# hbdat/cvpr22_cross_modal_pseudo_labeling

Measured on AMD Instinct MI355X. Metric: images/sec student-teacher train step (COCO 800x1333), higher is better.
Workload: dtype f32 (bf16x3 split MFMA, fp32 accum); 1 GPU; student_teacher_mask_rcnn_uncertainty.yaml R-50-C4, 2 img/GPU 3x800x1333, fwd+bwd+allreduce+SGD; global_batch=2, parallelism=dp1, losses_finite=True, pipelined=True

## Files before the change

### cvpr22_cross_modal_pseudo_labeling_amd/_C.py

```python
import contextlib
import functools
import ctypes
import threading

import torch

from . import _cpu, _lib

_L = _lib.load()


def _stream():
    return torch._C._cuda_getCurrentRawStream(torch.cuda.current_device())


class _Same:

    def __enter__(self):
        return None

    def __exit__(self, *exc):
        return False


# ... 494 lines not shown
    out = torch.empty((r * h * w, 3 * kh * kw * c), dtype=torch.bfloat16, device=x.device)
    if out.numel() == 0:
        return out
    with _on(x.device):
        rc = _L.ovis_im2col_split_bf16x3_f32(x.data_ptr(), out.data_ptr(), r, h, w, c, kh, kw, int(bool(flip)), _stream())
    _lib.check(rc, "im2col_split_bf16x3")
    return out


def match_encode(gt_boxes, gt_labels, proposals, high, low, weights=None, between_keeps_label=False):
    gt_boxes, proposals = _dev(gt_boxes, "gt_boxes"), _dev(proposals, "proposals")
    gt_labels = gt_labels.to(torch.int64).contiguous()
    g, p = gt_boxes.shape[0], proposals.shape[0]
    if g == 0:
        raise ValueError("No ground-truth boxes available for one of the images during training")
    idx = torch.empty((p,), dtype=torch.int64, device=proposals.device)
    lab = torch.empty((p,), dtype=torch.int64, device=proposals.device)
    reg = torch.empty((p, 4), dtype=torch.float32, device=proposals.device) if weights is not None else None
    if p:
        wx, wy, ww, wh = weights if weights is not None else (1.0, 1.0, 1.0, 1.0)
        with _on(proposals.device):
            rc = _L.ovis_match_encode_f32(gt_boxes.data_ptr(), gt_labels.data_ptr(), proposals.data_ptr(), g, p, high, low,
                                          int(bool(between_keeps_label)), wx, wy, ww, wh, idx.data_ptr(), lab.data_ptr(),
                                          0 if reg is None else reg.data_ptr(), _stream())
        _lib.check(rc, "match_encode")
    return idx, lab, reg


def rpn_match_encode(gt_boxes, anchors, visibility, high_threshold, low_threshold, allow_low_quality_matches, weights):
    gt_boxes, anchors = _dev(gt_boxes, "gt_boxes"), _dev(anchors, "anchors")
    if not (visibility.is_cuda and visibility.dtype == torch.bool and visibility.shape == (anchors.shape[0],)):
        raise RuntimeError("rpn_match_encode: visibility must be a bool HIP tensor [A]")
    visibility = visibility.contiguous()
    g, a = gt_boxes.shape[0], anchors.shape[0]
    if g == 0:
        raise ValueError("No ground-truth boxes available for one of the images during training")
    labels = torch.empty((a,), dtype=torch.int64, device=anchors.device)
    reg = torch.empty((a, 4), dtype=torch.float32, device=anchors.device)
    scratch = torch.empty((g,), dtype=torch.int32, device=anchors.device)
    wx, wy, ww, wh = weights
    with _on(anchors.device):
        rc = _L.ovis_rpn_match_encode_f32(gt_boxes.data_ptr(), anchors.data_ptr(), visibility.data_ptr(), g, a, high_threshold,
                                          low_threshold, int(bool(allow_low_quality_matches)), wx, wy, ww, wh, scratch.data_ptr(),
                                          labels.data_ptr(), reg.data_ptr(), _stream())
    _lib.check(rc, "rpn_match_encode")
    return labels, reg


def project_masks(masks, gt_index, boxes, resolution):
    if not (masks.is_cuda and masks.dim() == 3 and masks.dtype in (torch.bool, torch.uint8)):
        raise RuntimeError("project_masks: [G,H,W] bool / uint8 HIP tensor expected")
    masks = masks.contiguous()
    boxes = _dev(boxes, "boxes")
    gt_index = gt_index.to(torch.int64).contiguous()
    p = boxes.shape[0]
    out = torch.empty((p, resolution, resolution), dtype=torch.float32, device=boxes.device)
    if p:
        with _on(boxes.device):
            rc = _L.ovis_project_masks_f32(masks.data_ptr(), gt_index.data_ptr(), boxes.data_ptr(), p, masks.shape[1],
                                           masks.shape[2], resolution, int(masks.dtype == torch.bool), out.data_ptr(),
                                           _stream())
        _lib.check(rc, "project_masks")
    return out


def sample_fg_bg(labels, batch_size, max_positives, seed):
    if not labels.is_cuda or labels.dtype != torch.int64 or labels.dim() != 1:
        raise RuntimeError("sample_fg_bg: 1-D int64 HIP tensor expected (the product path has no CPU fallback)")
    labels = labels.contiguous()
    sel = torch.empty((batch_size,), dtype=torch.int64, device=labels.device)
    slots = torch.empty((batch_size,), dtype=torch.int64, device=labels.device)
    counts = torch.empty((2,), dtype=torch.int32, device=labels.device)
    with _on(labels.device):
        rc = _L.ovis_sample_fg_bg(labels.data_ptr(), labels.numel(), int(batch_size), int(max_positives),
                                  int(seed) & 0xFFFFFFFFFFFFFFFF, sel.data_ptr(), slots.data_ptr(), counts.data_ptr(), _stream())
    _lib.check(rc, "sample_fg_bg")
    return sel, slots, counts


def gather_rows(index, boxes_a=None, boxes_b=None, ints_a=None, ints_b=None):
    index = _dev(index, "index", torch.int64)
    n = index.numel()
    srcs = [None if t is None else _dev(t, "boxes", torch.float32) for t in (boxes_a, boxes_b)] + \
           [None if t is None else _dev(t, "ints", torch.int64) for t in (ints_a, ints_b)]
    for t in srcs[:2]:
        if t is not None and (t.dim() != 2 or t.shape[1] != 4):
            raise RuntimeError("gather_rows: float sources must be [P, 4]")
    for t in srcs[2:]:
        if t is not None and t.dim() != 1:
            raise RuntimeError("gather_rows: int64 sources must be [P]")
    outs = [None if t is None else torch.empty((n,) + tuple(t.shape[1:]), dtype=t.dtype, device=t.device) for t in srcs]
    if n:
        ptr = lambda t: 0 if t is None else t.data_ptr()
        with _on(index.device):
            rc = _L.ovis_gather_rows(index.data_ptr(), n, ptr(srcs[0]), ptr(outs[0]), ptr(srcs[1]), ptr(outs[1]), ptr(srcs[2]),
                                     ptr(outs[2]), ptr(srcs[3]), ptr(outs[3]), _stream())
        _lib.check(rc, "gather_rows")
    return tuple(outs)


def project_pasted_masks(mask_probs, gt_boxes, gt_index, boxes, image_size, resolution, threshold=0.5):
    mask_probs, gt_boxes, boxes = _dev(mask_probs, "mask_probs"), _dev(gt_boxes, "gt_boxes"), _dev(boxes, "boxes")
    gt_index = _dev(gt_index, "gt_index", torch.int64)
    p = boxes.shape[0]
    out = torch.empty((p, resolution, resolution), dtype=torch.float32, device=boxes.device)
    if p == 0:
        return out
    if mask_probs.dim() != 3 or mask_probs.shape[1] != mask_probs.shape[2] or gt_boxes.shape != (mask_probs.shape[0], 4):
        raise RuntimeError("project_pasted_masks: expected mask_probs [G,M,M] and gt_boxes [G,4]")
    with _on(boxes.device):
        rc = _L.ovis_project_pasted_masks_f32(mask_probs.data_ptr(), gt_boxes.data_ptr(), gt_index.data_ptr(),
                                              boxes.data_ptr(), p, int(image_size[0]), int(image_size[1]),
                                              mask_probs.shape[1], int(resolution), float(threshold), out.data_ptr(), _stream())
    _lib.check(rc, "project_pasted_masks")
    return out


def split_pair(x):
    if not x.is_cuda or x.dtype != torch.float32 or x.dim() != 2:
        raise RuntimeError("split_pair: 2-D float32 HIP tensor expected")
    if x.stride(1) != 1 or x.stride(0) % 4 or x.data_ptr() % 16:
        x = x.contiguous()
    rows, cols = x.shape
    out = torch.empty((rows, 2 * cols), dtype=torch.bfloat16, device=x.device)
    if out.numel() == 0:
        return out
    with _on(x.device):
        rc = _L.ovis_split_pair_f32(x.data_ptr(), x.stride(0), out.data_ptr(), rows, cols, _stream())
    _lib.check(rc, "split_pair")
    return out


def gate_split_pair(dy, gate=None, want_f32=False, pooled=None, pool_rows=0, selected=None, group_slot=None):
    if dy is None and pooled is None:
        raise RuntimeError("gate_split_pair: dy or pooled must be given")
    if (selected is None) != (group_slot is None):
        raise RuntimeError("gate_split_pair: selected and group_slot are given together")
    if pooled is not None:
        if not (pooled.is_cuda and pooled.dtype == torch.float32 and pooled.dim() == 2):
            raise RuntimeError("gate_split_pair: pooled must be a 2-D float32 HIP tensor")
        pooled = pooled.contiguous()
    if dy is not None:
        if not (dy.is_cuda and dy.dtype == torch.float32 and dy.dim() == 2):
            raise RuntimeError("gate_split_pair: 2-D float32 HIP tensor expected")
        if dy.stride(1) != 1 or dy.stride(0) % 4 or dy.data_ptr() % 16:
            dy = dy.contiguous()
        rows, cols = dy.shape
    else:
        rows, cols = pooled.shape[0] * pool_rows, pooled.shape[1]
    if pooled is not None and (pool_rows <= 0 or pooled.shape != (rows // max(pool_rows, 1), cols) or rows % pool_rows):
        raise RuntimeError("gate_split_pair: pooled must be [rows / pool_rows, cols]")
    dev = dy.device if dy is not None else pooled.device
    is_pair = 0
    if gate is not None:
        is_pair = int(gate.dtype == torch.bfloat16)
        if not (gate.is_cuda and gate.is_contiguous() and gate.shape == (rows, cols * (2 if is_pair else 1))
                and gate.dtype in (torch.bfloat16, torch.float32)):
            raise RuntimeError("gate_split_pair: gate must be the contiguous fp32 or pair form of the forward output")
    out = torch.empty((rows, 2 * cols), dtype=torch.bfloat16, device=dev)
    g32 = torch.empty((rows, cols), dtype=torch.float32, device=dev) if want_f32 else None
    if out.numel() == 0:
        return out, g32
    if selected is not None:
        selected, group_slot = _dev(selected, "selected"), _dev(group_slot, "group_slot", torch.int32)
        if pool_rows <= 0 or rows % pool_rows or selected.dim() != 2 or selected.shape[1] != cols or \
                selected.shape[0] % pool_rows or group_slot.numel() != rows // pool_rows:
            raise RuntimeError("gate_split_pair: selected must be [S * pool_rows, cols] and group_slot [rows / pool_rows]")
    with _on(dev):
        rc = _L.ovis_gate_split_pair_rows_f32(0 if dy is None else dy.data_ptr(), 0 if dy is None else dy.stride(0),
                                              0 if gate is None else gate.data_ptr(), is_pair, out.data_ptr(),
                                              0 if g32 is None else g32.data_ptr(), rows, cols,
                                              0 if pooled is None else pooled.data_ptr(), pool_rows,
                                              0 if selected is None else selected.data_ptr(),
                                              0 if group_slot is None else group_slot.data_ptr(), _stream())
    _lib.check(rc, "gate_split_pair")
    return out, g32


def im2col_pair(xp, h, w, kh, kw):
    if not (xp.is_cuda and xp.dtype == torch.bfloat16 and xp.dim() == 2 and xp.is_contiguous()):
        raise RuntimeError("im2col_pair: contiguous 2-D bfloat16 HIP tensor (pair layout) expected")
    m, c2 = xp.shape
    if m % (h * w):
        raise RuntimeError("im2col_pair: rows must be a multiple of h*w")
    out = torch.empty((m, kh * kw * c2), dtype=torch.bfloat16, device=xp.device)
    if out.numel() == 0:
        return out
    with _on(xp.device):
        rc = _L.ovis_im2col_pair(xp.data_ptr(), out.data_ptr(), m // (h * w), h, w, c2 // 2, kh, kw, _stream())
    _lib.check(rc, "im2col_pair")
    return out


def im2col_nchw_pair(x, kh, kw, stride, pad):
    if not (x.is_cuda and x.dtype == torch.float32 and x.dim() == 4 and x.is_contiguous()):
        raise RuntimeError("im2col_nchw_pair: contiguous [N,C,H,W] float32 HIP tensor expected")
    n, c, h, w = x.shape
    ho, wo = (h + 2 * pad - kh) // stride + 1, (w + 2 * pad - kw) // stride + 1
    kp = -(-(kh * kw * c) // 32) * 32
    out = torch.empty((n * ho * wo, 2 * kp), dtype=torch.bfloat16, device=x.device)
    if out.numel():
        with _on(x.device):
            rc = _L.ovis_im2col_nchw_pair_f32(x.data_ptr(), out.data_ptr(), n, c, h, w, kh, kw, stride, pad, kp, _stream())
        _lib.check(rc, "im2col_nchw_pair")
    return out, (ho, wo)


_GEMM_TLS = threading.local()


@contextlib.contextmanager
def co_scheduled(on=True):
    prev = getattr(_GEMM_TLS, "co", False)
    _GEMM_TLS.co = bool(on)
    try:
        yield
    finally:
        _GEMM_TLS.co = prev


@functools.lru_cache(maxsize=None)
def _gemm_ws_bytes(m, n, ch, ch2, kh, kw, w, config):
    return int(_L.ovis_split_gemm_pair_workspace_bytes_ex(m, n, ch, ch2, kh, kw, w, config))


@functools.lru_cache(maxsize=None)
def _tn_slices(m, n, ch, taps):
    return int(_L.ovis_split_gemm_tn_slices(m, n, ch, taps))


@functools.lru_cache(maxsize=None)
def _gemm_f32_ws_bytes(m, n, k):
    return int(_L.ovis_gemm_f32_workspace_bytes(m, n, k))


@functools.lru_cache(maxsize=None)
def _nms_presorted_ws_bytes(n, k):
    return int(_L.ovis_nms_presorted_workspace_bytes(n, k))


@functools.lru_cache(maxsize=None)
def _topk_ws_bytes(n, a):
    return int(_L.ovis_topk_sorted_workspace_bytes(n, a))


def _gemm_cfg(config):
    return config | (0x10000 if getattr(_GEMM_TLS, "co", False) else 0)


def split_gemm_pair(a_pair, b_pair, bias=None, residual=None, relu=False, out_f32=True, out_pair=False, conv=None,
                    config=0, a2_pair=None, residual_pair=None):
    for t, name in ((a_pair, "a_pair"), (b_pair, "b_pair")) + (((a2_pair, "a2_pair"),) if a2_pair is not None else ()):
        if not (t.is_cuda and t.dtype == torch.bfloat16 and t.dim() == 2 and t.stride(1) == 1):
            raise RuntimeError(f"split_gemm_pair: {name} must be a 2-D bfloat16 HIP tensor in pair layout")
    m, ch = a_pair.shape[0], a_pair.shape[1] // 2
    n, k = b_pair.shape[0], b_pair.shape[1] // 2
    ch2 = 0
    if a2_pair is not None:
        if conv is not None or a2_pair.shape[0] != m:
            raise RuntimeError("split_gemm_pair: a2_pair needs a plain product and as many rows as a_pair")
        ch2 = a2_pair.shape[1] // 2
    h = w = 0
    kh = kw = 1
    flip = False
    if conv is not None:
        h, w, kh, kw, flip = conv
        if m % (h * w):
            raise RuntimeError("split_gemm_pair: rows must be a multiple of h*w")
    if k != kh * kw * ch + ch2:
        raise RuntimeError(f"split_gemm_pair: contraction mismatch (A has {ch} channels x {kh * kw} taps + {ch2}, B has {k})")
    dev = a_pair.device
    c = torch.empty((m, n), dtype=torch.float32, device=dev) if out_f32 else None
    cp = torch.empty((m, 2 * n), dtype=torch.bfloat16, device=dev) if out_pair else None
    if m == 0 or n == 0:
        return c, cp
    if bias is not None:
        bias = _dev(bias, "bias")
    if residual_pair is not None:
        if residual is not None or conv is not None or a2_pair is not None or n % 32 or not (
                residual_pair.is_cuda and residual_pair.dtype == torch.bfloat16 and residual_pair.dim() == 2
                and residual_pair.stride(1) == 1 and residual_pair.shape == (m, 2 * n)):
            raise RuntimeError("split_gemm_pair: residual_pair must be [M, 2N] bfloat16 pair rows of a plain product")
        with _on(dev):
            config = _gemm_cfg(config)
            nbytes = _gemm_ws_bytes(m, n, ch, 0, 1, 1, 0, config) if not (config & 8) else 0
            ws = torch.empty((nbytes,), dtype=torch.uint8, device=dev) if nbytes else None
            rc = _L.ovis_split_gemm_pair_rp(a_pair.data_ptr(), 2 * a_pair.stride(0), b_pair.data_ptr(), 2 * b_pair.stride(0),
                                            0 if c is None else c.data_ptr(), n, 0 if cp is None else cp.data_ptr(), 4 * n,
                                            0 if bias is None else bias.data_ptr(), residual_pair.data_ptr(),
                                            2 * residual_pair.stride(0), m, n, ch, int(bool(relu)),
                                            0 if ws is None else ws.data_ptr(), nbytes, config, _stream())
        _lib.check(rc, "split_gemm_pair_rp")
        return c, cp
    if residual is not None and not (residual.is_cuda and residual.dtype == torch.float32 and residual.dim() == 2
                                     and residual.stride(1) == 1 and residual.shape == (m, n)):
        raise RuntimeError("split_gemm_pair: residual must be a float32 [M, N] HIP tensor with unit column stride")
    with _on(dev):
        config = _gemm_cfg(config)
        nbytes = _gemm_ws_bytes(m, n, ch, ch2, kh, kw, w, config) if not (config & 8) else 0
        ws = torch.empty((nbytes,), dtype=torch.uint8, device=dev) if nbytes else None
        rc = _L.ovis_split_gemm_pair(a_pair.data_ptr(), 2 * a_pair.stride(0),
                                     0 if a2_pair is None else a2_pair.data_ptr(),
                                     0 if a2_pair is None else 2 * a2_pair.stride(0),
                                     b_pair.data_ptr(), 2 * b_pair.stride(0),
                                     0 if c is None else c.data_ptr(), n, 0 if cp is None else cp.data_ptr(), 4 * n,
                                     0 if bias is None else bias.data_ptr(),
                                     0 if residual is None else residual.data_ptr(),
                                     0 if residual is None else residual.stride(0), m, n, ch, ch2, kh, kw, h, w,
                                     int(bool(flip)), int(bool(relu)), 0 if ws is None else ws.data_ptr(), nbytes,
                                     config, _stream())
    _lib.check(rc, "split_gemm_pair")
    return c, cp


def split_gemm_pair_pool_supported(m, n, ch, pool_rows):
    return bool(_L.ovis_split_gemm_pair_pool_supported(int(m), int(n), int(ch), int(pool_rows)))


def split_gemm_pair_rp_pool(a_pair, b_pair, bias, residual_pair, relu, out_f32, out_pair, pool_rows):
    for t, name in ((a_pair, "a_pair"), (b_pair, "b_pair")) + (((residual_pair, "residual_pair"),) if residual_pair is not None else ()):
        if not (t.is_cuda and t.dtype == torch.bfloat16 and t.dim() == 2 and t.stride(1) == 1):
            raise RuntimeError(f"split_gemm_pair_rp_pool: {name} must be a 2-D bfloat16 HIP tensor in pair layout")
    m, ch = a_pair.shape[0], a_pair.shape[1] // 2
    n, k = b_pair.shape[0], b_pair.shape[1] // 2
    if k != ch or m % pool_rows or (residual_pair is not None and residual_pair.shape != (m, 2 * n)):
        raise RuntimeError("split_gemm_pair_rp_pool: shape mismatch")
    dev = a_pair.device
    c = torch.empty((m, n), dtype=torch.float32, device=dev) if out_f32 else None
    cp = torch.empty((m, 2 * n), dtype=torch.bfloat16, device=dev) if out_pair else None
    pooled = torch.zeros((m // pool_rows, n), dtype=torch.float32, device=dev)
    if m == 0 or n == 0:
        return c, cp, pooled
    if bias is not None:
        bias = _dev(bias, "bias")
    with _on(dev):
        rc = _L.ovis_split_gemm_pair_rp_pool(a_pair.data_ptr(), 2 * a_pair.stride(0), b_pair.data_ptr(), 2 * b_pair.stride(0),
                                             0 if c is None else c.data_ptr(), n, 0 if cp is None else cp.data_ptr(), 4 * n,
                                             0 if bias is None else bias.data_ptr(),
                                             0 if residual_pair is None else residual_pair.data_ptr(),
                                             0 if residual_pair is None else 2 * residual_pair.stride(0), m, n, ch,
                                             int(bool(relu)), pooled.data_ptr(), int(pool_rows), 1.0 / pool_rows, _stream())
    _lib.check(rc, "split_gemm_pair_rp_pool")
    return c, cp, pooled


def weight_prep_pair(w, scale=None, want_transposed=False):
    if not (w.is_cuda and w.dtype == torch.float32 and w.dim() == 4):
        raise RuntimeError("weight_prep_pair: [N,C,KH,KW] float32 HIP tensor expected")
    w = w.detach().contiguous()
    n, c, kh, kw = w.shape
    t = kh * kw
    fwd = torch.empty((n, 2 * t * c), dtype=torch.bfloat16, device=w.device)
    bwd = torch.empty((c, 2 * t * n), dtype=torch.bfloat16, device=w.device) if want_transposed else None
    if scale is not None:
        scale = _dev(scale.detach(), "scale")
    with _on(w.device):
        rc = _L.ovis_weight_prep_pair_f32(w.data_ptr(), 0 if scale is None else scale.data_ptr(), fwd.data_ptr(),
                                          0 if bwd is None else bwd.data_ptr(), n, c, t, _stream())
    _lib.check(rc, "weight_prep_pair")
    return fwd, bwd


def split_gemm_pair_gated(a_pair, b_pair, gate_pair, conv=None, out_f32=False, out_pair=True, config=0):
    for t, name in ((a_pair, "a_pair"), (b_pair, "b_pair"), (gate_pair, "gate_pair")):
        if not (t.is_cuda and t.dtype == torch.bfloat16 and t.dim() == 2 and t.stride(1) == 1):
            raise RuntimeError(f"split_gemm_pair_gated: {name} must be a 2-D bfloat16 HIP tensor in pair layout")
    m, ch = a_pair.shape[0], a_pair.shape[1] // 2
    n, k = b_pair.shape[0], b_pair.shape[1] // 2
    h = w = 0
    kh = kw = 1
    flip = False
    if conv is not None:
        h, w, kh, kw, flip = conv
    if k != kh * kw * ch or gate_pair.shape != (m, 2 * n):
        raise RuntimeError("split_gemm_pair_gated: shape mismatch")
    dev = a_pair.device
    c = torch.empty((m, n), dtype=torch.float32, device=dev) if out_f32 else None
    cp = torch.empty((m, 2 * n), dtype=torch.bfloat16, device=dev) if out_pair else None
    if m == 0 or n == 0:
        return c, cp
    with _on(dev):
        config = _gemm_cfg(config)
        nbytes = _gemm_ws_bytes(m, n, ch, 0, kh, kw, w, config) if not (config & 8) else 0
        ws = torch.empty((nbytes,), dtype=torch.uint8, device=dev) if nbytes else None
        rc = _L.ovis_split_gemm_pair_gated_ws(a_pair.data_ptr(), 2 * a_pair.stride(0), b_pair.data_ptr(),
                                              2 * b_pair.stride(0), 0 if c is None else c.data_ptr(), n,
                                              0 if cp is None else cp.data_ptr(), 4 * n, gate_pair.data_ptr(),
                                              2 * gate_pair.stride(0), m, n, ch, kh, kw, h, w, int(bool(flip)),
                                              0 if ws is None else ws.data_ptr(), nbytes, config, _stream())
    _lib.check(rc, "split_gemm_pair_gated")
    return c, cp


def split_gemm_pair_rp_gated(a_pair, b_pair, residual_pair, gate_pair, out_f32=False, out_pair=True, config=0):
    for t, name in ((a_pair, "a_pair"), (b_pair, "b_pair"), (residual_pair, "residual_pair"), (gate_pair, "gate_pair")):
        if not (t.is_cuda and t.dtype == torch.bfloat16 and t.dim() == 2 and t.stride(1) == 1):
            raise RuntimeError(f"split_gemm_pair_rp_gated: {name} must be a 2-D bfloat16 HIP tensor in pair layout")
    m, ch = a_pair.shape[0], a_pair.shape[1] // 2
    n, k = b_pair.shape[0], b_pair.shape[1] // 2
    if k != ch or gate_pair.shape != (m, 2 * n) or residual_pair.shape != (m, 2 * n):
        raise RuntimeError("split_gemm_pair_rp_gated: shape mismatch")
    dev = a_pair.device
    c = torch.empty((m, n), dtype=torch.float32, device=dev) if out_f32 else None
    cp = torch.empty((m, 2 * n), dtype=torch.bfloat16, device=dev) if out_pair else None
    if m == 0 or n == 0:
        return c, cp
    with _on(dev):
        rc = _L.ovis_split_gemm_pair_rp_gated(a_pair.data_ptr(), 2 * a_pair.stride(0), b_pair.data_ptr(),
                                              2 * b_pair.stride(0), 0 if c is None else c.data_ptr(), n,
                                              0 if cp is None else cp.data_ptr(), 4 * n, residual_pair.data_ptr(),
                                              2 * residual_pair.stride(0), gate_pair.data_ptr(), 2 * gate_pair.stride(0), m, n,
                                              ch, config, _stream())
    _lib.check(rc, "split_gemm_pair_rp_gated")
    return c, cp


def split_gemm_pair_tn_supported(n, ch, conv=None):
    if n % 128 or ch % 128:
        return False
    if conv is not None:
        h, w, kh, kw = conv
        return kh % 2 == 1 and kw % 2 == 1
    return True


def split_gemm_pair_tn(g_pair, x_pair, conv=None, scale=None, weight_shape=None):
    for t, name in ((g_pair, "g_pair"), (x_pair, "x_pair")):
        if not (t.is_cuda and t.dtype == torch.bfloat16 and t.dim() == 2 and t.stride(1) == 1):
            raise RuntimeError(f"split_gemm_pair_tn: {name} must be a 2-D bfloat16 HIP tensor in pair layout")
    m, n, ch = g_pair.shape[0], g_pair.shape[1] // 2, x_pair.shape[1] // 2
    if x_pair.shape[0] != m:
        raise RuntimeError("split_gemm_pair_tn: row counts differ")
    h = w = 0
    kh = kw = 1
    if conv is not None:
        h, w, kh, kw = conv
        if m % (h * w):
            raise RuntimeError("split_gemm_pair_tn: rows must be a multiple of h*w")
    dev = g_pair.device
    if m == 0:
        z = torch.zeros((n, kh * kw * ch), dtype=torch.float32, device=dev)
        return z if weight_shape is None else z.new_zeros(weight_shape)
    slices = _tn_slices(m, n, ch, kh * kw)
    slabs = torch.empty((slices, n, kh * kw * ch), dtype=torch.float32, device=dev)
    with _on(dev):
        rc = _L.ovis_split_gemm_pair_tn(g_pair.data_ptr(), 2 * g_pair.stride(0), x_pair.data_ptr(), 2 * x_pair.stride(0),
                                        slabs.data_ptr(), slices, m, n, ch, kh, kw, h, w, _stream())
        _lib.check(rc, "split_gemm_pair_tn")
        if weight_shape is None:
            return slabs[0] if slices == 1 else slabs.sum(0)
        if tuple(weight_shape) != (n, ch, kh, kw):
            raise RuntimeError("split_gemm_pair_tn: weight_shape must be (N, ch, kh, kw)")
        dw = torch.empty(weight_shape, dtype=torch.float32, device=dev)
        if scale is not None:
            scale = _dev(scale.detach(), "scale")
        rc = _L.ovis_slab_reduce_f32(slabs.data_ptr(), 0 if scale is None else scale.data_ptr(), dw.data_ptr(), slices, n,
                                     ch, kh * kw, _stream())
    _lib.check(rc, "slab_reduce")
    return dw


def bias_act_(y, bias=None, residual=None, relu=True):
    if not (y.is_cuda and y.dtype == torch.float32 and y.dim() == 2 and y.is_contiguous()):
        raise RuntimeError("bias_act_: contiguous 2-D float32 HIP tensor expected")
    if residual is not None and not (residual.is_contiguous() and residual.shape == y.shape):
        raise RuntimeError("bias_act_: residual must be contiguous with y's shape")
    if y.numel() == 0:
        return y
    with _on(y.device):
        rc = _L.ovis_bias_act_f32(y.data_ptr(), 0 if bias is None else bias.data_ptr(),
                                  0 if residual is None else residual.data_ptr(), y.shape[0], y.shape[1],
                                  int(bool(relu)), _stream())
    _lib.check(rc, "bias_act")
    return y


def gemm_nt(a, b, bias=None):
    if not a.is_cuda and not b.is_cuda:
        return _cpu.gemm_nt(a, b, bias)
    if not (a.is_cuda and b.is_cuda):
        raise RuntimeError("gemm_nt: HIP device tensors only")
    if a.dtype != torch.float32 or b.dtype != torch.float32:
        raise RuntimeError("gemm_nt: float32 only")
    m, k = a.shape
    n, k2 = b.shape
    if k != k2:
        raise RuntimeError(f"gemm_nt: inner dimensions differ ({k} vs {k2})")
    out = torch.empty((m, n), dtype=torch.float32, device=a.device)
    if m == 0 or n == 0:
        return out
    if k == 0:
        return out.zero_() if bias is None else out.copy_(bias.expand(m, n))
    if bias is not None:
        bias = _dev(bias, "bias")
    with _on(a.device):
        _gemm_raw(a.data_ptr(), a.stride(0), a.stride(1), b.data_ptr(), b.stride(0), b.stride(1), out.data_ptr(), n, m, n, k,
                  bias_ptr=0 if bias is None else bias.data_ptr(), device=a.device)
    return out


def region_noun_align(region_emb, noun_emb):
    if not region_emb.is_cuda:
        return _cpu.region_noun_align(region_emb, noun_emb)
    region_emb, noun_emb = _dev(region_emb, "region_emb"), _dev(noun_emb, "noun_emb")
    p, d = region_emb.shape
    w = noun_emb.shape[0]
    raw = torch.empty((w,), dtype=torch.float32, device=region_emb.device)
    prob = torch.empty_like(raw)
    idx = torch.empty((w,), dtype=torch.int64, device=region_emb.device)
    if w == 0:
        return raw, prob, idx
    with _on(region_emb.device):
        rc = _L.ovis_region_noun_align_f32(region_emb.data_ptr(), noun_emb.data_ptr(), raw.data_ptr(),
                                           prob.data_ptr(), idx.data_ptr(), p, w, d, _stream())
    _lib.check(rc, "region_noun_align")
    return raw, prob, idx


def text_embed(table, input_ids, special_tokens_mask):
    if not table.is_cuda:
        return _cpu.text_embed(table.detach(), input_ids.to(torch.int64), special_tokens_mask.to(torch.int64))
    table = _dev(table, "table")
    if table.dim() != 2 or input_ids.dim() != 2 or input_ids.shape != special_tokens_mask.shape:
        raise RuntimeError("text_embed: expected table [V, D] and input_ids / special_tokens_mask [N, L]")
    if table.requires_grad:
        raise RuntimeError("text_embed: the embedding table is frozen on this path (MODEL.LANGUAGE_BACKBONE.FT_EMB False)")
    ids = input_ids.to(device=table.device, dtype=torch.int32).contiguous()
    sp = special_tokens_mask.to(device=table.device, dtype=torch.int32).contiguous()
    n, l = ids.shape
    out = torch.empty((n, table.shape[1]), dtype=torch.float32, device=table.device)
    if n:
        with _on(table.device):
            rc = _L.ovis_text_embed_f32(table.data_ptr(), table.shape[0], table.shape[1], ids.data_ptr(), sp.data_ptr(), n, l,
                                        out.data_ptr(), _stream())
        _lib.check(rc, "text_embed")
    return out


def project_polygon_masks(coords, polygon_start, instance_start, gt_index, boxes, image_size, resolution):
    if not boxes.is_cuda:
        return _cpu.project_polygon_masks(coords, polygon_start, instance_start, gt_index, boxes, image_size, resolution)
    boxes = _dev(boxes, "boxes")
    coords = _dev(coords, "coords") if coords.numel() else coords
    polygon_start = _dev(polygon_start, "polygon_start", torch.int32)
    instance_start = _dev(instance_start, "instance_start", torch.int32)
    gt_index = _dev(gt_index, "gt_index", torch.int64)
    p = boxes.shape[0]
    out = torch.empty((p, resolution, resolution), dtype=torch.float32, device=boxes.device)
    if p:
        with _on(boxes.device):
            rc = _L.ovis_project_polygon_masks_f32(coords.data_ptr() if coords.numel() else 0, polygon_start.data_ptr(),
                                                   instance_start.data_ptr(), gt_index.data_ptr(), boxes.data_ptr(), p,
                                                   int(image_size[0]), int(image_size[1]), int(resolution), out.data_ptr(),
                                                   _stream())
        _lib.check(rc, "project_polygon_masks")
    return out


def weighted_ce_fwd_bwd(logits, labels, bg_weight, need_grad=True):
    if not logits.is_cuda:
        return _cpu.weighted_ce_fwd_bwd(logits, labels, bg_weight, need_grad)
    logits, labels = _dev(logits, "logits"), _dev(labels, "labels", torch.int64)
    p, c = logits.shape
    loss = torch.empty((1,), dtype=torch.float32, device=logits.device)
    dlogits = torch.empty_like(logits) if need_grad else None
    scratch = torch.empty((max(p, 1),), dtype=torch.float32, device=logits.device)
# ... 305 lines not shown
```

### cvpr22_cross_modal_pseudo_labeling_amd/_lib.py

```python
import ctypes
import os

_HERE = os.path.dirname(os.path.abspath(__file__))
LIB_PATH = os.path.join(_HERE, "libovis_hip.so")

OVIS_OK = 0
_ERRORS = {-1: "OVIS_EINVAL (bad size or null pointer)",
           -2: "OVIS_ENOSPC (workspace too small)",
           -3: "OVIS_ERANGE (problem size not supported by the kernel)"}

_vp, _i, _f, _sz, _l = ctypes.c_void_p, ctypes.c_int, ctypes.c_float, ctypes.c_size_t, ctypes.c_long

SIGNATURES = {
    "ovis_version": (ctypes.c_char_p, []),
    "ovis_roi_align_forward_f32": (_i, [_vp, _vp, _vp, _i, _i, _i, _i, _i, _i, _i, _f, _i, _vp]),
    "ovis_roi_align_forward_workspace_bytes": (_sz, [_i, _i, _i]),
    "ovis_roi_align_forward_mfma_supported": (_i, [_i, _i, _i, _i]),
    "ovis_roi_align_forward_ws_f32": (_i, [_vp, _vp, _vp, _i, _i, _i, _i, _i, _i, _i, _f, _i, _vp, _sz, _vp]),
    "ovis_roi_align_forward_strided_from_nhwc_f32": (_i, [_vp, _vp, _vp, _i, _i, _i, _i, _i, _i, _i, _i, _f, _i, _i, _vp]),
    "ovis_roi_align_backward_f32": (_i, [_vp, _vp, _vp, _i, _i, _i, _i, _i, _i, _i, _f, _i, _vp]),
    "ovis_roi_align_backward_workspace_bytes": (_sz, [_i, _i, _i, _i]),
    "ovis_roi_align_backward_plane_supported": (_i, [_i, _i, _i, _i]),
    "ovis_roi_align_backward_ws_f32": (_i, [_vp, _vp, _vp, _i, _i, _i, _i, _i, _i, _i, _f, _i, _vp, _sz, _vp]),
    "ovis_roi_align_backward_strided_ws_f32": (_i, [_vp, _vp, _vp, _i, _i, _i, _i, _i, _i, _i, _i, _f, _i, _vp, _sz, _vp]),
    "ovis_roi_align_backward_strided_nhwc_workspace_bytes": (_sz, [_i, _i, _i, _i, _i]),
    "ovis_roi_align_backward_strided_nhwc_ws_f32": (_i, [_vp, _vp, _vp, _i, _i, _i, _i, _i, _i, _i, _i, _f, _i, _vp, _sz, _vp]),
    "ovis_roi_pool_forward_f32": (_i, [_vp, _vp, _vp, _vp, _i, _i, _i, _i, _i, _i, _i, _f, _vp]),
    "ovis_roi_pool_backward_f32": (_i, [_vp, _vp, _vp, _vp, _i, _i, _i, _i, _i, _i, _i, _vp]),
    "ovis_deform_psroi_pool_forward_f32": (_i, [_vp] * 5 + [_i] * 7 + [_f] + [_i] * 5 + [_f, _vp]),
    "ovis_deform_psroi_pool_backward_f32": (_i, [_vp] * 7 + [_i] * 7 + [_f] + [_i] * 5 + [_f, _vp]),
    "ovis_nms_workspace_bytes": (_sz, [_i]),
    "ovis_nms_f32": (_i, [_vp, _vp, _i, _f, _i, _vp, _sz, _vp, _vp, _vp]),
    "ovis_nms_grouped_f32": (_i, [_vp, _vp, _vp, _i, _f, _i, _vp, _sz, _vp, _vp, _vp]),
    "ovis_sample_fg_bg": (_i, [_vp, _i, _i, _i, ctypes.c_uint64, _vp, _vp, _vp, _vp]),
    "ovis_project_pasted_masks_f32": (_i, [_vp, _vp, _vp, _vp, _i, _i, _i, _i, _i, _f, _vp, _vp]),
    "ovis_nms_presorted_workspace_bytes": (_sz, [_i, _i]),
    "ovis_nms_presorted_batched_f32": (_i, [_vp, _vp, _i, _i, _f, _i, _i, _vp, _sz, _vp, _vp, _vp]),
    "ovis_box_decode_f32": (_i, [_vp, _l, _vp, _l, _l, _i, _f, _f, _f, _f, _f, _i, _vp, _vp, _vp, _vp]),
    "ovis_smooth_l1_picked_fwd_bwd_f32": (_i, [_vp, _l, _i, _i, _vp, _l, _vp, _vp, _i, _i, _f, _f, _vp, _vp, _vp]),
    "ovis_gather_rows": (_i, [_vp, _i, _vp, _vp, _vp, _vp, _vp, _vp, _vp, _vp, _vp]),
    "ovis_rois_from_boxes_f32": (_i, [_vp, _vp, _vp, _i, _vp, _vp]),
    "ovis_deform_conv_implicit_f32": (_i, [_vp, _vp, _vp, _vp, _l, _vp, _vp, _l] + [_i] * 16 + [_vp]),
    "ovis_topk_sorted_workspace_bytes": (_sz, [_i, _i]),
    "ovis_topk_sorted_f32": (_i, [_vp, _l, _i, _i, _i, _vp, _vp, _vp, _sz, _vp]),
    "ovis_rpn_decode_f32": (_i, [_vp, _l, _l, _l, _vp, _vp, _vp, _i, _i, _i, _i, _f, _f, _f, _f, _f, _f, _f, _vp, _vp, _vp]),
    "ovis_sigmoid_focal_loss_forward_f32": (_i, [_vp, _vp, _vp, _i, _i, _f, _f, _vp]),
    "ovis_sigmoid_focal_loss_backward_f32": (_i, [_vp, _vp, _vp, _vp, _i, _i, _f, _f, _vp]),
    "ovis_split_bf16x3_f32": (_i, [_vp, _l, _vp, _l, _i, _i, _vp]),
    "ovis_im2col_split_bf16x3_f32": (_i, [_vp, _vp, _l, _i, _i, _i, _i, _i, _i, _vp]),
    "ovis_bias_act_f32": (_i, [_vp, _vp, _vp, _l, _i, _i, _vp]),
    "ovis_split_pair_f32": (_i, [_vp, _l, _vp, _l, _i, _vp]),
    "ovis_gate_split_pair_rows_f32": (_i, [_vp, _l, _vp, _i, _vp, _vp, _l, _i, _vp, _i, _vp, _vp, _vp]),
    "ovis_gate_split_pair_f32": (_i, [_vp, _l, _vp, _i, _vp, _vp, _l, _i, _vp, _i, _vp]),
    "ovis_im2col_nchw_pair_f32": (_i, [_vp, _vp] + [_i] * 9 + [_vp]),
    "ovis_weight_prep_pair_f32": (_i, [_vp, _vp, _vp, _vp, _i, _i, _i, _vp]),
    "ovis_slab_reduce_f32": (_i, [_vp, _vp, _vp, _i, _i, _i, _i, _vp]),
    "ovis_im2col_pair": (_i, [_vp, _vp, _l, _i, _i, _i, _i, _i, _vp]),
    "ovis_split_gemm_tn_slices": (_i, [_l, _i, _i, _i]),
    "ovis_split_gemm_pair_tn": (_i, [_vp, _l, _vp, _l, _vp, _i, _l, _i, _i, _i, _i, _i, _i, _vp]),
    "ovis_split_gemm_pair_gated": (_i, [_vp, _l, _vp, _l, _vp, _l, _vp, _l, _vp, _l, _l] + [_i] * 8 + [_vp]),
    "ovis_split_gemm_pair_gated_ws": (_i, [_vp, _l, _vp, _l, _vp, _l, _vp, _l, _vp, _l, _l] + [_i] * 7 + [_vp, _sz, _i, _vp]),
    "ovis_split_gemm_pair_workspace_bytes": (_sz, [_l, _i, _i, _i, _i, _i, _i]),
    "ovis_split_gemm_pair_workspace_bytes_ex": (_sz, [_l, _i, _i, _i, _i, _i, _i, _i]),
    "ovis_split_gemm_pair_rp_gated": (_i, [_vp, _l, _vp, _l, _vp, _l, _vp, _l, _vp, _l, _vp, _l, _l, _i, _i, _i, _vp]),
    "ovis_split_gemm_pair_pool_supported": (_i, [_l, _i, _i, _i]),
    "ovis_split_gemm_pair_rp_pool": (_i, [_vp, _l, _vp, _l, _vp, _l, _vp, _l, _vp, _vp, _l, _l, _i, _i, _i, _vp, _i, _f, _vp]),
    "ovis_split_gemm_pair_rp": (_i, [_vp, _l, _vp, _l, _vp, _l, _vp, _l, _vp, _vp, _l, _l, _i, _i, _i, _vp, _sz, _i, _vp]),
    "ovis_split_gemm_pair": (_i, [_vp, _l, _vp, _l, _vp, _l, _vp, _l, _vp, _l, _vp, _vp, _l, _l] + [_i] * 9
                             + [_vp, _sz, _i, _vp]),
    "ovis_match_encode_f32": (_i, [_vp, _vp, _vp, _i, _i, _f, _f, _i, _f, _f, _f, _f, _vp, _vp, _vp, _vp]),
    "ovis_rpn_match_encode_f32": (_i, [_vp, _vp, _vp, _i, _i, _f, _f, _i, _f, _f, _f, _f, _vp, _vp, _vp, _vp]),
    "ovis_project_masks_f32": (_i, [_vp, _vp, _vp, _i, _i, _i, _i, _i, _vp, _vp]),
    "ovis_gemm_f32": (_i, [_vp, _l, _l, _vp, _l, _l, _vp, _vp, _l, _i, _i, _i, _vp]),
    "ovis_gemm_ex_f32": (_i, [_vp, _l, _l, _vp, _l, _l, _vp, _i, _f, _i, _vp, _l, _i, _i, _i, _vp]),
    "ovis_gemm_f32_workspace_bytes": (_sz, [_i, _i, _i]),
    "ovis_gemm_ex_ws_f32": (_i, [_vp, _l, _l, _vp, _l, _l, _vp, _i, _f, _i, _vp, _l, _i, _i, _i, _vp, _sz, _vp]),
    "ovis_deform_im2col_f32": (_i, [_vp, _vp, _vp, _vp] + [_i] * 13 + [_vp]),
    "ovis_deform_col2im_f32": (_i, [_vp, _vp, _vp, _vp] + [_i] * 13 + [_vp]),
    "ovis_deform_col2im_coord_f32": (_i, [_vp, _vp, _vp, _vp, _vp, _vp] + [_i] * 13 + [_vp]),
    "ovis_deform_im2col_pair_rows_f32": (_i, [_vp, _vp, _vp, _vp, _l] + [_i] * 15 + [_vp]),
    "ovis_deform_col2im_rows_f32": (_i, [_vp, _l, _vp, _vp, _vp, _vp, _vp, _vp] + [_i] * 15 + [_vp]),
    "ovis_region_noun_align_f32": (_i, [_vp, _vp, _vp, _vp, _vp, _i, _i, _i, _vp]),
    "ovis_text_embed_f32": (_i, [_vp, _l, _i, _vp, _vp, _i, _i, _vp, _vp]),
    "ovis_project_polygon_masks_f32": (_i, [_vp, _vp, _vp, _vp, _vp, _i, _i, _i, _i, _vp, _vp]),
    "ovis_sgd_momentum_multi_f32": (_i, [_vp, _vp, _i, _f, _f, _f, _i, _vp]),
    "ovis_bottleneck_identity_backward_workspace_bytes": (_sz, [_l, _i, _i, _i, _i, _i, _i]),
    "ovis_bottleneck_identity_backward": (_i, [_vp, _l] * 7 + [_vp] * 3 + [_l, _i, _i, _i, _i, _i, _i] + [_vp] * 7 + [_sz, _i, _vp, _vp]),
    "ovis_weight_prep_pair_multi_f32": (_i, [_vp, _vp, _i, _i, _vp]),
    "ovis_weight_prep_tile": (_i, []),
    "ovis_sgd_chunk_elements": (_i, []),
    "ovis_weighted_ce_fwd_bwd_f32": (_i, [_vp, _vp, _f, _vp, _vp, _vp, _i, _i, _vp]),
    "ovis_mask_bce_stochastic_fwd_bwd_f32": (_i, [_vp, _vp, _vp, _vp, _vp, _vp, _vp, _vp, _vp, _i, _i, _i, _i, _i, _vp]),
    "ovis_mask_bce_stochastic_classes_fwd_bwd_f32": (_i, [_vp, _vp, _vp, _vp, _vp, _vp, _vp, _vp, _vp, _vp, _i, _i, _i, _i, _vp]),
}

_lib = None


def load():
    global _lib
    if _lib is None:
        if not os.path.exists(LIB_PATH):
            raise ImportError(
                f"{LIB_PATH} is missing: build the HIP extension first "
                "(make -C cvpr22_cross_modal_pseudo_labeling_amd/csrc). There is no CPU fallback.")
        lib = ctypes.CDLL(LIB_PATH)
        for name, (res, args) in SIGNATURES.items():
            fn = getattr(lib, name)
            fn.restype = res
            fn.argtypes = args
        _lib = lib
    return _lib


def check(rc, what):
    if rc == OVIS_OK:
        return
    if rc < 0:
        raise RuntimeError(f"{what}: {_ERRORS.get(rc, rc)}")
    raise RuntimeError(f"{what}: HIP error {rc}")
```

### cvpr22_cross_modal_pseudo_labeling_amd/csrc/split_gemm.hip

```cpp
#include <stdlib.h>

#include "ovis_common.h"
constexpr int kGroupWidth = 4;

namespace {
typedef short bf16x8 __attribute__((ext_vector_type(8)));
typedef float f32x4 __attribute__((ext_vector_type(4)));
typedef __bf16 b2 __attribute__((ext_vector_type(2)));
typedef float f2 __attribute__((ext_vector_type(2)));

__device__ char g_zero_line[128];

enum { PLAIN = 0, SHIFTED = 1, HALO = 2, DEFORM = 3 };
constexpr int kHalo = 8;

struct SplitGemmArgs {
  const char* A; long a_rs;
  const char* A2; long a2_rs;
  const char* B; long b_rs;
  float* C; long ldc;
  char* Cp; long cp_rs;
  const float* bias; const float* res; long ldr;
  const char* resp; long resp_rs;
  const char* gate; long gate_rs;
  float* pool; int pool_rows; float pool_scale;
  float* slab;
  long M; int N; int ch; int ch2; int T; int H; int W; int KH; int KW; int flip; int relu; int gw;
  int kslices; int steps_per_slice;
  const float* dimg; const float* doff; const float* dmask;
  int Ho; int Wo; int sh; int sw; int ph; int pw; int dlh; int dlw; int dg;
};

__device__ __forceinline__ void glds16(const char* gsrc, char* lds_wave_base) {
  __builtin_amdgcn_global_load_lds((const __attribute__((address_space(1))) void*)gsrc,
                                   (__attribute__((address_space(3))) void*)lds_wave_base, 16, 0, 0);
}

__device__ __forceinline__ unsigned pack_bf16(float a, float b) {
  f2 v = {a, b};
  return __builtin_bit_cast(unsigned, __builtin_convertvector(v, b2));
}

struct EpilogueOperands {
  uint2 a, b;
};

struct EpilogueSource {
  const char* base;
  long row_bytes;
  int second;
};

__device__ __forceinline__ EpilogueSource epilogue_source(const SplitGemmArgs& p) {
  EpilogueSource s;
  s.base = p.res ? (const char*)p.res : (p.resp ? p.resp : p.gate);
  s.row_bytes = p.res ? p.ldr * 4 : (p.resp ? p.resp_rs : p.gate_rs);
  s.second = p.res ? 8 : (p.resp ? 64 : 0);
  return s;
}

__device__ __forceinline__ long epilogue_column_bytes(const SplitGemmArgs& p, int n, long poff) { return p.res ? (long)n * 4 : poff; }

__device__ __forceinline__ void epilogue_fetch4(const EpilogueSource& s, long m, long column_bytes, EpilogueOperands& o) {
  const char* q = s.base + m * s.row_bytes + column_bytes;
  o.a = *(const uint2*)q;
  o.b = *(const uint2*)(q + s.second);
}

template <bool DUAL = false>
__device__ __forceinline__ f32x4 epilogue_apply4(const SplitGemmArgs& p, long m, int n, long poff, f32x4 v, const f32x4& bias4,
                                                 const EpilogueOperands& o, uint2 gate2 = make_uint2(0u, 0u)) {
  if (p.bias) v += bias4;
  if (p.res) {
    v.x += __uint_as_float(o.a.x); v.y += __uint_as_float(o.a.y); v.z += __uint_as_float(o.b.x); v.w += __uint_as_float(o.b.y);
  } else if (p.resp) {
    const unsigned hx = o.a.x, hy = o.a.y, lx = o.b.x, ly = o.b.y;
    v.x += __uint_as_float(hx << 16) + __uint_as_float(lx << 16);
    v.y += __uint_as_float(hx & 0xffff0000u) + __uint_as_float(lx & 0xffff0000u);
    v.z += __uint_as_float(hy << 16) + __uint_as_float(ly << 16);
    v.w += __uint_as_float(hy & 0xffff0000u) + __uint_as_float(ly & 0xffff0000u);
  }
  if (p.relu) {
    v.x = fmaxf(v.x, 0.f); v.y = fmaxf(v.y, 0.f); v.z = fmaxf(v.z, 0.f); v.w = fmaxf(v.w, 0.f);
  }
  if (p.gate) {
    const unsigned gx = DUAL ? gate2.x : o.a.x, gy = DUAL ? gate2.y : o.a.y;
    const unsigned a0 = gx & 0xffffu, a1 = gx >> 16, a2 = gy & 0xffffu, a3 = gy >> 16;
    if (a0 == 0u || a0 >= 0x8000u) v.x = 0.f;
    if (a1 == 0u || a1 >= 0x8000u) v.y = 0.f;
    if (a2 == 0u || a2 >= 0x8000u) v.z = 0.f;
    if (a3 == 0u || a3 >= 0x8000u) v.w = 0.f;
  }
  if (p.C) *(f32x4*)(p.C + m * p.ldc + n) = v;
  if (p.Cp) {
    const unsigned h01 = pack_bf16(v.x, v.y), h23 = pack_bf16(v.z, v.w);
    const unsigned l01 = pack_bf16(v.x - __uint_as_float(h01 << 16), v.y - __uint_as_float(h01 & 0xffff0000u));
    const unsigned l23 = pack_bf16(v.z - __uint_as_float(h23 << 16), v.w - __uint_as_float(h23 & 0xffff0000u));
    char* d = p.Cp + m * p.cp_rs + poff;
    *(uint2*)d = make_uint2(h01, h23);
    *(uint2*)(d + 64) = make_uint2(l01, l23);
  }
  return v;
}

__device__ __forceinline__ void epilogue_store4(const SplitGemmArgs& p, long m, int n, f32x4 v) {
  const long poff = (long)(n >> 5) * 128 + (n & 31) * 2;
  f32x4 bias4 = {0.f, 0.f, 0.f, 0.f};
  if (p.bias) bias4 = *(const f32x4*)(p.bias + n);
  const EpilogueSource src = epilogue_source(p);
  EpilogueOperands o;
  if (src.base) epilogue_fetch4(src, m, epilogue_column_bytes(p, n, poff), o);
  epilogue_apply4(p, m, n, poff, v, bias4, o);
}

template <int WM, int WN, int MODE, int NS, int OCC, bool DUAL = false, bool POOL = false>
__global__ __launch_bounds__(WM * WN * 64, OCC) void split_gemm_kernel(SplitGemmArgs p, int tiles_n, int ntiles) {
  constexpr int BM = WM * 64, BN = WN * 64, NW = WM * WN;
  constexpr int A_ROWS = MODE == HALO ? BM + 2 * kHalo + 2 : BM;
  constexpr int ZROW = BM + 2 * kHalo;
  constexpr int A_BYTES = A_ROWS * 128, B_BYTES = BN * 128, STAGE = A_BYTES + B_BYTES;
  constexpr int A_PIECES = (MODE == HALO ? BM + 2 * kHalo : BM) / 8;
  constexpr int AI = (A_PIECES + NW - 1) / NW;
  constexpr int BI = BN / 8 / NW;
  static_assert(MODE != HALO || NS == 1, "the halo tile is single-staged");
  static_assert(NW * 4096 <= STAGE * NS, "epilogue staging fits the k-loop's LDS");
  extern __shared__ __attribute__((aligned(16))) char smem[];

  const int lane = threadIdx.x & 63, wave = __builtin_amdgcn_readfirstlane(threadIdx.x >> 6);
  int id;
  {
    const int nblocks = gridDim.x;
    const int b = blockIdx.x, q = nblocks >> 3, r = nblocks & 7, xcd = b & 7, loc = b >> 3;
    id = (xcd < r ? xcd * (q + 1) : r * (q + 1) + (xcd - r) * q) + loc;
  }
  const int slice = id / ntiles;
  const int tile = id - slice * ntiles;
  const int gw = p.gw, tiles_m = ntiles / tiles_n;
  const int per_group = tiles_m * gw;
  const int grp = tile / per_group;
  const int in_grp = tile - grp * per_group;
  const int tile_m = in_grp / gw, tile_n = grp * gw + (in_grp - tile_m * gw);
  const long m0 = (long)tile_m * BM;
  const int n0 = tile_n * BN;
  const int Mi = (int)p.M;

  const int cpb = p.ch >> 5;
  const int nk = p.T * cpb + (p.ch2 >> 5);
  int dy = 0, dx = 0;
  auto set_tap = [&](int t) {
    dy = t / p.KW - p.KH / 2;
    dx = t % p.KW - p.KW / 2;
    if (p.flip) { dy = -dy; dx = -dx; }
  };

  struct LaneGeom { int lr, s0, s1; };
  auto lane_geom = [&](int ln) {
    const int lr = ln >> 3, lc = ln & 7;
    return LaneGeom{lr, (lc ^ lr) * 16, (lc ^ lr) * 16};
  };
  auto clamp_row = [&](int gm) { return gm < 0 ? 0 : (gm > Mi - 1 ? Mi - 1 : gm); };
  int a_yx[MODE == SHIFTED ? AI : 1];
  if (MODE == SHIFTED) {
#pragma unroll
    for (int i = 0; i < AI; ++i) {
      const int gm = clamp_row((int)m0 + (wave * AI + i) * 8 + (lane >> 3));
      a_yx[i] = (((gm / p.W) % p.H) << 16) | (gm % p.W);
    }
  }

  auto issue_b = [&](int stage, int kb, const LaneGeom& g) {
#pragma unroll
    for (int i = 0; i < BI; ++i) {
      const int piece = wave * BI + i;
      int gn = n0 + piece * 8 + g.lr;
      if (gn > p.N - 1) gn = p.N - 1;
      glds16(p.B + (long)gn * p.b_rs + (long)kb * 128 + ((piece & 1) ? g.s1 : g.s0),
             smem + stage * STAGE + A_BYTES + piece * 1024);
    }
  };
  auto issue_a_plain = [&](int stage, int kb, const LaneGeom& g) {
    const bool first = kb < cpb;
    const char* base = first ? p.A : p.A2;
    const long rs = first ? p.a_rs : p.a2_rs;
    const long koff = (long)(first ? kb : kb - cpb) * 128;
#pragma unroll
    for (int i = 0; i < AI; ++i) {
      const int piece = wave * AI + i;
      glds16(base + (long)clamp_row((int)m0 + piece * 8 + g.lr) * rs + koff + ((piece & 1) ? g.s1 : g.s0),
             smem + stage * STAGE + piece * 1024);
    }
  };
  const char* zero_line = g_zero_line;
  auto issue_a_shifted = [&](int stage, int cb, const LaneGeom& g) {
    const long shift = ((long)dy * p.W + dx) * p.a_rs + (long)cb * 128;
#pragma unroll
    for (int i = 0; i < AI; ++i) {
      const int piece = wave * AI + i;
      const char* src = p.A + (long)clamp_row((int)m0 + piece * 8 + g.lr) * p.a_rs + shift + ((piece & 1) ? g.s1 : g.s0);
      const int y = (a_yx[MODE == SHIFTED ? i : 0] >> 16) + dy, x = (a_yx[MODE == SHIFTED ? i : 0] & 0xffff) + dx;
      if ((unsigned)y >= (unsigned)p.H || (unsigned)x >= (unsigned)p.W) src = zero_line + (g.s0 & 0x70);
      glds16(src, smem + stage * STAGE + piece * 1024);
    }
  };
  auto issue_a_halo = [&](int cb, const LaneGeom& g) {
#pragma unroll
    for (int i = 0; i < AI; ++i) {
      const int piece = wave + NW * i;
      if (piece < A_PIECES)
        glds16(p.A + (long)clamp_row((int)m0 + piece * 8 + g.lr - kHalo) * p.a_rs + (long)cb * 128 + ((piece & 1) ? g.s1 : g.s0),
               smem + piece * 1024);
    }
  };

  constexpr int DR = MODE == DEFORM ? 4 : 1;
  float d_w[DR][4], d_mask[DR];
  int d_o[DR][4];
  int d_tap = -1, d_grp = -1;
  f32x4 d_v[DR][4];
  auto deform_fetch = [&](int tap, int cb) {
    if constexpr (MODE == DEFORM) {
      const int prow0 = threadIdx.x >> 3, pch = (threadIdx.x & 7) * 4;
      const int grp = (cb * 32) / (p.ch / p.dg);
      if (tap != d_tap || grp != d_grp) {
        d_tap = tap;
        d_grp = grp;
        const long plane_o = (long)p.Ho * p.Wo;
        const int ky = tap / p.KW, kx = tap - ky * p.KW;
#pragma unroll
        for (int j = 0; j < 4; ++j) {
          const int gm = clamp_row((int)m0 + prow0 + 32 * j);
          const int wo = gm % p.Wo, t1 = gm / p.Wo;
          const int ho = t1 % p.Ho, bimg = t1 / p.Ho;
          const long pix = (long)ho * p.Wo + wo;
          const float* off = p.doff + (((long)bimg * p.dg + grp) * 2 * p.T + 2 * tap) * plane_o + pix;
          const float h = (float)(ho * p.sh - p.ph + ky * p.dlh) + off[0];
          const float w = (float)(wo * p.sw - p.pw + kx * p.dlw) + off[plane_o];
          d_o[j][0] = d_o[j][1] = d_o[j][2] = d_o[j][3] = -1;
          d_w[j][0] = d_w[j][1] = d_w[j][2] = d_w[j][3] = 0.f;
          if (h > -1.f && w > -1.f && h < (float)p.H && w < (float)p.W) {
            const int hl = (int)floorf(h), wl = (int)floorf(w);
            const int hh = hl + 1, wh = wl + 1;
            const float lh = h - hl, lw = w - wl, uh = 1.f - lh, uw = 1.f - lw;
            d_w[j][0] = uh * uw; d_w[j][1] = uh * lw; d_w[j][2] = lh * uw; d_w[j][3] = lh * lw;
            const int img = bimg * p.H * p.W;
            if (hl >= 0 && wl >= 0) d_o[j][0] = (img + hl * p.W + wl) * p.ch;
            if (hl >= 0 && wh <= p.W - 1) d_o[j][1] = (img + hl * p.W + wh) * p.ch;
            if (hh <= p.H - 1 && wl >= 0) d_o[j][2] = (img + hh * p.W + wl) * p.ch;
            if (hh <= p.H - 1 && wh <= p.W - 1) d_o[j][3] = (img + hh * p.W + wh) * p.ch;
          }
          d_mask[j] = p.dmask ? p.dmask[(((long)bimg * p.dg + grp) * p.T + tap) * plane_o + pix] : 1.f;
        }
      }
      const float* base = p.dimg + cb * 32 + pch;
      const f32x4 z = f32x4{0.f, 0.f, 0.f, 0.f};
#pragma unroll
      for (int j = 0; j < 4; ++j)
#pragma unroll
        for (int c = 0; c < 4; ++c) d_v[j][c] = d_o[j][c] >= 0 ? *(const f32x4*)(base + d_o[j][c]) : z;
    }
  };
  auto deform_commit = [&]() {
    if constexpr (MODE == DEFORM) {
      const int prow0 = threadIdx.x >> 3, chunk = (threadIdx.x & 7) >> 1, sub = (threadIdx.x & 1) * 8;
#pragma unroll
      for (int j = 0; j < 4; ++j) {
        f32x4 v = d_w[j][0] * d_v[j][0] + d_w[j][1] * d_v[j][1] + d_w[j][2] * d_v[j][2] + d_w[j][3] * d_v[j][3];
        if (p.dmask) v *= d_mask[j];
        const unsigned h0 = pack_bf16(v.x, v.y), h1 = pack_bf16(v.z, v.w);
// ... 14 lines not shown
  if (MODE == HALO) {
#pragma unroll
    for (int f = 0; f < 4; ++f) {
      const int gm = clamp_row((int)m0 + wm * 64 + f * 16 + frow);
      const int x = gm % p.W, y = (gm / p.W) % p.H;
      unsigned mask = 0u;
      for (int t = 0; t < p.T; ++t) {
        set_tap(t);
        if ((unsigned)(y + dy) < (unsigned)p.H && (unsigned)(x + dx) < (unsigned)p.W) mask |= 1u << t;
      }
      h_ok[f >> 1] |= mask << ((f & 1) * 16);
    }
    if (threadIdx.x < 16) *(uint4*)(smem + ZROW * 128 + threadIdx.x * 16) = make_uint4(0u, 0u, 0u, 0u);
  }

  f32x4 acc[4][4];
#pragma unroll
  for (int f = 0; f < 4; ++f)
#pragma unroll
    for (int g = 0; g < 4; ++g) acc[f][g] = f32x4{0.f, 0.f, 0.f, 0.f};

  auto compute = [&](const char* base, int b0, int a0, int a1, int a2, int a3) {
    const int ard[4] = {a0, a1, a2, a3};
    bf16x8 ah[4], al[4], bh[4], bl[4];
#pragma unroll
    for (int f = 0; f < 4; ++f) {
      bh[f] = *(const bf16x8*)(base + b0 + f * 2048);
      ah[f] = *(const bf16x8*)(base + ard[f]);
    }
#pragma unroll
    for (int f = 0; f < 4; ++f) {
      bl[f] = *(const bf16x8*)(base + ((b0 + f * 2048) ^ 64));
      al[f] = *(const bf16x8*)(base + (ard[f] ^ 64));
    }
#pragma unroll
    for (int f = 0; f < 4; ++f)
#pragma unroll
      for (int g = 0; g < 4; ++g)
        acc[f][g] = __builtin_amdgcn_mfma_f32_16x16x32_bf16(bh[g], ah[f], acc[f][g], 0, 0, 0);
#pragma unroll
    for (int f = 0; f < 4; ++f)
#pragma unroll
      for (int g = 0; g < 4; ++g)
        acc[f][g] = __builtin_amdgcn_mfma_f32_16x16x32_bf16(bh[g], al[f], acc[f][g], 0, 0, 0);
#pragma unroll
    for (int f = 0; f < 4; ++f)
#pragma unroll
      for (int g = 0; g < 4; ++g)
        acc[f][g] = __builtin_amdgcn_mfma_f32_16x16x32_bf16(bl[g], ah[f], acc[f][g], 0, 0, 0);
  };
  auto compute_static = [&](const char* base) { compute(base, b_rd0, a_rd0, a_rd0 + 2048, a_rd0 + 4096, a_rd0 + 6144); };

  if (MODE == HALO) {
    const int cb0 = slice * p.steps_per_slice;
    int cb1 = cb0 + p.steps_per_slice;
    if (cb1 > cpb) cb1 = cpb;
    int t = 0, cb = cb0;
    for (int it = (cb1 - cb0) * p.T; it > 0; --it) {
      int ln = lane;
      asm volatile("" : "+v"(ln));
      const LaneGeom g = lane_geom(ln);
      const int fr = ln & 15, fq = ln >> 4;
      if (t == 0) issue_a_halo(cb, g);
      issue_b(0, t * cpb + cb, g);
      set_tap(t);
      const int L0 = wm * 64 + fr + kHalo + dy * p.W + dx;
      const int ard0 = L0 * 128 + ((fq ^ (L0 & 7)) << 4), zrd = ZROW * 128 + (ard0 & 255);
      const int b0 = A_BYTES + (wn * 64 + fr) * 128 + ((fq ^ (fr & 7)) << 4);
      int ard[4];
#pragma unroll
      for (int f = 0; f < 4; ++f) ard[f] = ((h_ok[f >> 1] >> ((f & 1) * 16 + t)) & 1u) ? ard0 + f * 2048 : zrd;
      __syncthreads();
      compute(smem, b0, ard[0], ard[1], ard[2], ard[3]);
      __syncthreads();
      if (++t == p.T) {
        t = 0;
        ++cb;
      }
    }
  } else {
    const int kb0 = slice * p.steps_per_slice;
    int kb1 = kb0 + p.steps_per_slice;
    if (kb1 > nk) kb1 = nk;
    int ld_tap = 0, ld_cb = kb0;
    if (MODE == SHIFTED || MODE == DEFORM) {
      ld_tap = kb0 / cpb;
      ld_cb = kb0 - ld_tap * cpb;
      set_tap(ld_tap);
    }
    auto issue = [&](int stage, int kb, const LaneGeom& g) {
      if (MODE == DEFORM) {
      } else if (MODE == SHIFTED) {
        issue_a_shifted(stage, ld_cb, g);
        if (++ld_cb == cpb) {
          ld_cb = 0;
          set_tap(++ld_tap);
        }
      } else {
        issue_a_plain(stage, kb, g);
      }
      issue_b(stage, kb, g);
    };
    if (MODE == DEFORM) {
      auto advance = [&]() {
        if (++ld_cb == cpb) {
          ld_cb = 0;
          ++ld_tap;
        }
      };
      if (kb0 < kb1) deform_fetch(ld_tap, ld_cb);
      for (int kb = kb0; kb < kb1; ++kb) {
        issue(0, kb, lane_geom(lane));
        deform_commit();
        __syncthreads();
        advance();
        if (kb + 1 < kb1) deform_fetch(ld_tap, ld_cb);
        compute_static(smem);
        __syncthreads();
      }
    } else if (NS == 1) {
      for (int kb = kb0; kb < kb1; ++kb) {
        int ln = lane;
        asm volatile("" : "+v"(ln));
        issue(0, kb, lane_geom(ln));
        __syncthreads();
        compute_static(smem);
        __syncthreads();
      }
    } else {
      const LaneGeom g = lane_geom(lane);
      if (kb0 < kb1) issue(0, kb0, g);
      for (int kb = kb0; kb < kb1; ++kb) {
        __syncthreads();
        if (kb + 1 < kb1) issue((kb + 1 - kb0) & 1, kb + 1, g);
        compute_static(smem + ((kb - kb0) & 1) * STAGE);
      }
      __syncthreads();
    }
  }

  char* stg = smem + wave * 4096;
  const int er = lane >> 4, es = lane & 15;
  const int n = n0 + wn * 64 + es * 4;
  float* slab = p.slab ? p.slab + (long)slice * p.M * p.N : nullptr;
  const bool col_ok = n < p.N;
  const long poff = (long)(n >> 5) * 128 + (n & 31) * 2;
  f32x4 bias4 = {0.f, 0.f, 0.f, 0.f};
  if (!slab && p.bias && col_ok) bias4 = *(const f32x4*)(p.bias + n);
  constexpr int NBUF = DUAL ? 2 : ((MODE == SHIFTED && NS == 1) ? 2 : 3);
  EpilogueOperands ops[NBUF][2];
  uint2 gates[NBUF][2];
  EpilogueSource src = epilogue_source(p);
  long src_col = epilogue_column_bytes(p, col_ok ? n : 0, col_ok ? poff : 0);
  if (slab || !src.base) {
    src.base = p.B;
    src.row_bytes = 0;
    src.second = 8;
    src_col = 0;
  }
  const long m_last = p.M - 1;
  const char* gate_col = DUAL ? p.gate + (col_ok ? poff : 0) : nullptr;
  auto fetch = [&](int piece, EpilogueOperands (&o)[2], uint2 (&g)[2]) {
#pragma unroll
    for (int j = 0; j < 2; ++j) {
      const long m = m0 + wm * 64 + (piece >> 1) * 16 + ((piece & 1) * 2 + j) * 4 + er;
      const long mc = m < m_last ? m : m_last;
      epilogue_fetch4(src, mc, src_col, o[j]);
      if constexpr (DUAL) g[j] = *(const uint2*)(gate_col + mc * p.gate_rs);
    }
  };
  f32x4 ps0 = {0.f, 0.f, 0.f, 0.f}, ps1 = ps0, ps2 = ps0;
  int pool_b1 = 0, pool_b2 = 0;
  long pool_map0 = 0;
  if constexpr (POOL) {
    const long mw = m0 + wm * 64;
    pool_map0 = mw / p.pool_rows;
    pool_b1 = (int)((pool_map0 + 1) * p.pool_rows - mw);
    pool_b2 = pool_b1 + p.pool_rows;
  }
#pragma unroll
  for (int i = 0; i < NBUF - 1; ++i) fetch(i, ops[i], gates[i]);
#pragma unroll
  for (int f = 0; f < 4; ++f) {
#pragma unroll
    for (int g = 0; g < 4; ++g) *(f32x4*)(stg + frow * 256 + (((g * 4 + fc) ^ frow) << 4)) = acc[f][g];
#pragma unroll
    for (int h = 0; h < 2; ++h) {
      const int piece = f * 2 + h;
      if (piece + NBUF - 1 < 8) fetch(piece + NBUF - 1, ops[(piece + NBUF - 1) % NBUF], gates[(piece + NBUF - 1) % NBUF]);
#pragma unroll
      for (int j = 0; j < 2; ++j) {
        const int r = (h * 2 + j) * 4 + er;
        const f32x4 v = *(const f32x4*)(stg + r * 256 + ((es ^ r) << 4));
        const long m = m0 + wm * 64 + f * 16 + r;
        if (m < p.M && col_ok) {
          if (slab) *(f32x4*)(slab + m * p.N + n) = v;
          else {
            const f32x4 fin = epilogue_apply4<DUAL>(p, m, n, poff, v, bias4, ops[piece % NBUF][j], gates[piece % NBUF][j]);
            if constexpr (POOL) {
              const int rr = f * 16 + r;
              const f32x4 z = {0.f, 0.f, 0.f, 0.f};
              ps0 += rr < pool_b1 ? fin : z;
              ps1 += (rr >= pool_b1 && rr < pool_b2) ? fin : z;
              ps2 += rr >= pool_b2 ? fin : z;
            }
          }
        }
      }
    }
  }
  if constexpr (POOL) {
    f32x4* ps[3] = {&ps0, &ps1, &ps2};
#pragma unroll
    for (int sgm = 0; sgm < 3; ++sgm) {
      f32x4 v = *ps[sgm];
#pragma unroll
      for (int e = 0; e < 4; ++e) {
        v[e] += __shfl_xor(v[e], 16, 64);
        v[e] += __shfl_xor(v[e], 32, 64);
      }
      const long first = (m0 + wm * 64) + (sgm == 0 ? 0 : (sgm == 1 ? pool_b1 : pool_b2));
      if (er == 0 && col_ok && first < p.M && (sgm == 0 || (sgm == 1 ? pool_b1 : pool_b2) < 64)) {
        float* d = p.pool + (pool_map0 + sgm) * p.N + n;
#pragma unroll
        for (int e = 0; e < 4; ++e) atomicAdd(d + e, v[e] * p.pool_scale);
      }
    }
  }
}

__global__ __launch_bounds__(256) void split_gemm_finish_kernel(SplitGemmArgs p) {
  const int n4 = p.N >> 2;
  const long total = p.M * n4;
  const long slab = p.M * p.N;
  for (long i = (long)blockIdx.x * 256 + threadIdx.x; i < total; i += (long)gridDim.x * 256) {
    const long m = i / n4;
    const int n = (int)(i - m * n4) * 4;
    const float* s = p.slab + m * p.N + n;
    f32x4 v = *(const f32x4*)s;
    for (int k = 1; k < p.kslices; ++k) v += *(const f32x4*)(s + k * slab);
    epilogue_store4(p, m, n, v);
  }
}

typedef short bf16x4 __attribute__((ext_vector_type(4)));

struct SplitGemmTnArgs {
  const char* G; long g_rs;
  const char* X; long x_rs;
  float* C;
  long M; int N; int ch; int T; int H; int W; int KH; int KW; int slices; int steps_per_slice;
  int g_major;
};

#define OVIS_TR_READ(dst, addr, off) \
  asm volatile("ds_read_b64_tr_b16 %0, %1 offset:%2" : "=v"(dst) : "v"(addr), "n"(off) : "memory")
#define OVIS_LGKM_WAIT8(N, a, b, c, d, e, f, g, h)                                                                \
  asm volatile("s_waitcnt lgkmcnt(%8)"                                                                             \
               : "+v"(a), "+v"(b), "+v"(c), "+v"(d), "+v"(e), "+v"(f), "+v"(g), "+v"(h)                            \
               : "n"(N)                                                                                            \
               : "memory")

template <bool CONV, bool SMALL = false>
__global__ __launch_bounds__(256, 2) void split_gemm_tn_kernel(SplitGemmTnArgs p, int tiles_i, int tiles_j,
                                                              int nblocks) {
  constexpr int TILE_BYTES = 32 * 512, STAGE = 2 * TILE_BYTES;
  extern __shared__ __attribute__((aligned(16))) char smem[];
  const int lane = threadIdx.x & 63, wave = threadIdx.x >> 6;
  int id;
  {
    constexpr int kChunk = 2 * OVIS_NUM_CU;
    const int b = blockIdx.x, base = b / kChunk * kChunk;
    const int nb = min(nblocks - base, kChunk), bl = b - base;
    const int q = nb >> 3, r = nb & 7, xcd = bl & 7, loc = bl >> 3;
    id = base + (xcd < r ? xcd * (q + 1) : r * (q + 1) + (xcd - r) * q) + loc;
  }
  const int per_slice = tiles_i * tiles_j;
  const int slice = id / per_slice;
  const int rem = id - slice * per_slice;
  const int tile_j = p.g_major ? rem % tiles_j : rem / tiles_i;
  const int tile_i = p.g_major ? rem / tiles_j : rem - tile_j * tiles_i;
  const int i0 = tile_i * 128, j0 = tile_j * 128;
  const int tap = CONV ? j0 / p.ch : 0, c0 = CONV ? j0 - tap * p.ch : j0;
  int off_rows = 0, tdy = 0, tdx = 0;
  if (CONV) {
    tdy = tap / p.KW - p.KH / 2;
    tdx = tap % p.KW - p.KW / 2;
    off_rows = tdy * p.W + tdx;
  }
  const long step0 = (long)slice * p.steps_per_slice;
  const long steps_total = (p.M + 31) >> 5;
  long step1 = step0 + p.steps_per_slice;
  if (step1 > steps_total) step1 = steps_total;
  const int nk = step1 > step0 ? (int)(step1 - step0) : 0;

  const int prow = lane >> 5, pseg = (lane & 31) >> 1, phalf = lane & 1;
  int rows[4];
  long g_off[4], x_off[4];
  int x_y[4], x_x[4];
  int m_row[4];
  const int HW = CONV ? p.H * p.W : 1;
  unsigned long long tap_mask = 0;
  if (CONV && SMALL) {
    const int qy = lane / p.W, qx = lane - qy * p.W;
    tap_mask = __ballot(lane < HW && (unsigned)(qy + tdy) < (unsigned)p.H && (unsigned)(qx + tdx) < (unsigned)p.W);
  }
#pragma unroll
  for (int i = 0; i < 4; ++i) {
    const int piece = wave * 4 + i;
    const int row = piece * 2 + prow;
    rows[i] = row;
    const int fr = (((row >> 3) & 1) << 2) | (row & 3);
    const int seg = pseg ^ fr;
    const int m = (int)(step0 << 5) + row;
    m_row[i] = m;
    g_off[i] = (long)m * p.g_rs + (long)i0 * 4 + seg * 32 + phalf * 16;
    x_off[i] = ((long)m + off_rows) * p.x_rs + (long)c0 * 4 + seg * 32 + phalf * 16;
    x_x[i] = CONV ? (SMALL ? m % HW : m % p.W) : 0;
    x_y[i] = (CONV && !SMALL) ? (m / p.W) % p.H : 0;
  }
  const int step_q = (CONV && SMALL) ? 32 % HW : 0;
  const int step_dx = CONV ? 32 % p.W : 0, step_dy = CONV ? 32 / p.W : 0;
  const bool y_single = step_dy + 1 <= p.H;
  const char* zero_src = g_zero_line + (lane & 7) * 16;
  const int Mi = (int)p.M;

  auto issue = [&](int stage) {
    char* base = smem + stage * STAGE;
    bool x_ok[4];
#pragma unroll
    for (int i = 0; i < 4; ++i) {
      x_ok[i] = m_row[i] < Mi;
      if (CONV && SMALL) {
        x_ok[i] = x_ok[i] && ((tap_mask >> x_x[i]) & 1ull) != 0ull;
        int q = x_x[i] + step_q;
        if (q >= HW) q -= HW;
        x_x[i] = q;
      } else if (CONV) {
        x_ok[i] = x_ok[i] && (unsigned)(x_y[i] + tdy) < (unsigned)p.H && (unsigned)(x_x[i] + tdx) < (unsigned)p.W;
        int x = x_x[i] + step_dx, y = x_y[i] + step_dy;
        if (x >= p.W) { x -= p.W; ++y; }
        if (y_single) { if (y >= p.H) y -= p.H; } else { y %= p.H; }
        x_x[i] = x;
        x_y[i] = y;
      }
    }
#pragma unroll
    for (int i = 0; i < 4; ++i) {
      const char* src = p.G + g_off[i];
      if (m_row[i] >= Mi) src = zero_src;
      glds16(src, base + (wave * 4 + i) * 1024);
      g_off[i] += 32 * p.g_rs;
    }
#pragma unroll
    for (int i = 0; i < 4; ++i) {
      const char* src = p.X + x_off[i];
      if (!x_ok[i]) src = zero_src;
      glds16(src, base + TILE_BYTES + (wave * 4 + i) * 1024);
      x_off[i] += 32 * p.x_rs;
      m_row[i] += 32;
    }
  };

  const int wi = wave >> 1, wj = wave & 1;
  const int gq = lane >> 4, pp = lane & 15;
  const int rrow = 8 * gq + (pp >> 2);
  const int rfr = ((gq & 1) << 2) | (pp >> 2);
  int g_rd[4], x_rd[4];
#pragma unroll
  for (int f = 0; f < 4; ++f) {
    const int seg_g = (2 * wi + (f >> 1)) * 4 + (f & 1);
    g_rd[f] = rrow * 512 + ((seg_g ^ rfr) << 5) + (pp & 3) * 8;
    const int seg_x = (2 * wj + (f >> 1)) * 4 + (f & 1);
    x_rd[f] = TILE_BYTES + rrow * 512 + ((seg_x ^ rfr) << 5) + (pp & 3) * 8;
  }

  f32x4 acc[4][4];
#pragma unroll
  for (int f = 0; f < 4; ++f)
#pragma unroll
    for (int g = 0; g < 4; ++g) acc[f][g] = f32x4{0.f, 0.f, 0.f, 0.f};

  if (nk > 0) issue(0);
  for (int kb = 0; kb < nk; ++kb) {
    __syncthreads();
    if (kb + 1 < nk) issue((kb + 1) & 1);
    const int so = (kb & 1) * STAGE;
    bf16x4 xa[4][2], xb[4][2], ga[4][2], gb[4][2];
#pragma unroll
    for (int f = 0; f < 4; ++f) {
      const int ax = so + x_rd[f], ag = so + g_rd[f];
      OVIS_TR_READ(xa[f][0], ax, 0);
      OVIS_TR_READ(xb[f][0], ax, 2048);
      OVIS_TR_READ(ga[f][0], ag, 0);
      OVIS_TR_READ(gb[f][0], ag, 2048);
    }
#pragma unroll
    for (int f = 0; f < 4; ++f) {
      const int ax = so + (x_rd[f] ^ 64), ag = so + (g_rd[f] ^ 64);
      OVIS_TR_READ(xa[f][1], ax, 0);
      OVIS_TR_READ(xb[f][1], ax, 2048);
      OVIS_TR_READ(ga[f][1], ag, 0);
      OVIS_TR_READ(gb[f][1], ag, 2048);
    }
    OVIS_LGKM_WAIT8(15, xa[0][0], xb[0][0], ga[0][0], gb[0][0], xa[1][0], xb[1][0], ga[1][0], gb[1][0]);
    OVIS_LGKM_WAIT8(15, xa[2][0], xb[2][0], ga[2][0], gb[2][0], xa[3][0], xb[3][0], ga[3][0], gb[3][0]);
    bf16x8 gh[4], gl[4], xh[4], xl[4];
#pragma unroll
    for (int f = 0; f < 4; ++f) {
      xh[f] = __builtin_shufflevector(xa[f][0], xb[f][0], 0, 1, 2, 3, 4, 5, 6, 7);
      gh[f] = __builtin_shufflevector(ga[f][0], gb[f][0], 0, 1, 2, 3, 4, 5, 6, 7);
    }
#pragma unroll
    for (int f = 0; f < 4; ++f)
#pragma unroll
      for (int g = 0; g < 4; ++g)
        acc[f][g] = __builtin_amdgcn_mfma_f32_16x16x32_bf16(xh[g], gh[f], acc[f][g], 0, 0, 0);
    OVIS_LGKM_WAIT8(0, xa[0][1], xb[0][1], ga[0][1], gb[0][1], xa[1][1], xb[1][1], ga[1][1], gb[1][1]);
    OVIS_LGKM_WAIT8(0, xa[2][1], xb[2][1], ga[2][1], gb[2][1], xa[3][1], xb[3][1], ga[3][1], gb[3][1]);
#pragma unroll
    for (int f = 0; f < 4; ++f) {
      xl[f] = __builtin_shufflevector(xa[f][1], xb[f][1], 0, 1, 2, 3, 4, 5, 6, 7);
      gl[f] = __builtin_shufflevector(ga[f][1], gb[f][1], 0, 1, 2, 3, 4, 5, 6, 7);
    }
#pragma unroll
    for (int f = 0; f < 4; ++f)
#pragma unroll
      for (int g = 0; g < 4; ++g)
        acc[f][g] = __builtin_amdgcn_mfma_f32_16x16x32_bf16(xh[g], gl[f], acc[f][g], 0, 0, 0);
#pragma unroll
    for (int f = 0; f < 4; ++f)
#pragma unroll
      for (int g = 0; g < 4; ++g)
        acc[f][g] = __builtin_amdgcn_mfma_f32_16x16x32_bf16(xl[g], gh[f], acc[f][g], 0, 0, 0);
  }

  const long ld = (long)p.T * p.ch;
  float* out = p.C + (long)slice * p.N * ld;
#pragma unroll
  for (int f = 0; f < 4; ++f) {
    const int i = i0 + wi * 64 + f * 16 + (lane & 15);
#pragma unroll
    for (int g = 0; g < 4; ++g) {
      const int j = j0 + wj * 64 + g * 16 + (lane >> 4) * 4;
      *(f32x4*)(out + (long)i * ld + j) = acc[f][g];
    }
  }
}

__global__ __launch_bounds__(256) void split_pair_kernel(const float* __restrict__ src, long src_rs,
                                                        char* __restrict__ dst, long rows, int cols) {
  const int oc = cols >> 3;
  const long total = rows * oc;
  for (long i = (long)blockIdx.x * 256 + threadIdx.x; i < total; i += (long)gridDim.x * 256) {
    const long r = i / oc;
    const int c = (int)(i - r * oc) * 8;
    const float4 v0 = *(const float4*)(src + r * src_rs + c), v1 = *(const float4*)(src + r * src_rs + c + 4);
    const unsigned h0 = pack_bf16(v0.x, v0.y), h1 = pack_bf16(v0.z, v0.w), h2 = pack_bf16(v1.x, v1.y),
                   h3 = pack_bf16(v1.z, v1.w);
    const unsigned l0 = pack_bf16(v0.x - __uint_as_float(h0 << 16), v0.y - __uint_as_float(h0 & 0xffff0000u));
    const unsigned l1 = pack_bf16(v0.z - __uint_as_float(h1 << 16), v0.w - __uint_as_float(h1 & 0xffff0000u));
    const unsigned l2 = pack_bf16(v1.x - __uint_as_float(h2 << 16), v1.y - __uint_as_float(h2 & 0xffff0000u));
    const unsigned l3 = pack_bf16(v1.z - __uint_as_float(h3 << 16), v1.w - __uint_as_float(h3 & 0xffff0000u));
    char* d = dst + r * 4L * cols + (long)(c >> 5) * 128 + (c & 31) * 2;
    *(uint4*)d = make_uint4(h0, h1, h2, h3);
    *(uint4*)(d + 64) = make_uint4(l0, l1, l2, l3);
  }
}

template <bool GATE_PAIR, bool WRITE_F32>
__global__ __launch_bounds__(256) void gate_split_pair_kernel(const float* __restrict__ dy, long dy_rs,
                                                             const void* __restrict__ gate, char* __restrict__ dst,
                                                             float* __restrict__ g32, long rows, int cols,
                                                             const float* __restrict__ gpool, int pool_rows,
                                                             float pool_scale, const float* __restrict__ gsel,
                                                             const int* __restrict__ group_slot) {
  const int oc = cols >> 3;
  const long total = rows * oc;
  for (long i = (long)blockIdx.x * 256 + threadIdx.x; i < total; i += (long)gridDim.x * 256) {
    const long r = i / oc;
    const int c = (int)(i - r * oc) * 8;
    float v[8];
    if (dy) {
      *(float4*)v = *(const float4*)(dy + r * dy_rs + c);
      *(float4*)(v + 4) = *(const float4*)(dy + r * dy_rs + c + 4);
    } else {
#pragma unroll
      for (int k = 0; k < 8; ++k) v[k] = 0.f;
    }
    if (gpool) {
      const float* gp = gpool + (r / pool_rows) * (long)cols + c;
      float q[8];
      *(float4*)q = *(const float4*)gp;
      *(float4*)(q + 4) = *(const float4*)(gp + 4);
#pragma unroll
      for (int k = 0; k < 8; ++k) v[k] = dy ? v[k] + q[k] * pool_scale : q[k] * pool_scale;
    }
    if (gsel) {
      const long grp = r / pool_rows;
      const int slot = group_slot[grp];
      if (slot >= 0) {
        const float* gs = gsel + ((long)slot * pool_rows + (r - grp * pool_rows)) * cols + c;
        float q[8];
        *(float4*)q = *(const float4*)gs;
        *(float4*)(q + 4) = *(const float4*)(gs + 4);
#pragma unroll
        for (int k = 0; k < 8; ++k) v[k] += q[k];
      }
    }
    const long poff = r * 4L * cols + (long)(c >> 5) * 128 + (c & 31) * 2;
    if (gate) {
      if (GATE_PAIR) {
        const uint4 h = *(const uint4*)((const char*)gate + poff);
        const unsigned w[4] = {h.x, h.y, h.z, h.w};
#pragma unroll
        for (int k = 0; k < 4; ++k) {
          const unsigned a = w[k] & 0xffffu, b = w[k] >> 16;
          if (a == 0u || a >= 0x8000u) v[2 * k] = 0.f;
          if (b == 0u || b >= 0x8000u) v[2 * k + 1] = 0.f;
        }
      } else {
        float y[8];
        *(float4*)y = *(const float4*)((const float*)gate + r * (long)cols + c);
        *(float4*)(y + 4) = *(const float4*)((const float*)gate + r * (long)cols + c + 4);
#pragma unroll
        for (int k = 0; k < 8; ++k)
          if (!(y[k] > 0.f)) v[k] = 0.f;
      }
    }
    unsigned h[4], l[4];
#pragma unroll
    for (int k = 0; k < 4; ++k) {
      h[k] = pack_bf16(v[2 * k], v[2 * k + 1]);
      l[k] = pack_bf16(v[2 * k] - __uint_as_float(h[k] << 16), v[2 * k + 1] - __uint_as_float(h[k] & 0xffff0000u));
    }
    *(uint4*)(dst + poff) = make_uint4(h[0], h[1], h[2], h[3]);
    *(uint4*)(dst + poff + 64) = make_uint4(l[0], l[1], l[2], l[3]);
    if (WRITE_F32) {
      *(float4*)(g32 + r * (long)cols + c) = *(float4*)v;
      *(float4*)(g32 + r * (long)cols + c + 4) = *(float4*)(v + 4);
    }
  }
}

__global__ __launch_bounds__(256) void im2col_nchw_pair_kernel(const float* __restrict__ src, char* __restrict__ dst,
                                                              int N, int C, int H, int W, int KH, int KW, int stride,
                                                              int pad, int Ho, int Wo, int kp) {
  const int groups = kp >> 3;
  const long total = (long)N * Ho * Wo * groups;
  const int K = KH * KW * C;
  for (long i = (long)blockIdx.x * 256 + threadIdx.x; i < total; i += (long)gridDim.x * 256) {
    const int gidx = (int)(i % groups);
    const long m = i / groups;
    const int ox = (int)(m % Wo);
    const int oy = (int)((m / Wo) % Ho);
    const int n = (int)(m / ((long)Wo * Ho));
    float v[8];
#pragma unroll
    for (int j = 0; j < 8; ++j) {
      const int k = gidx * 8 + j;
      float x = 0.f;
      if (k < K) {
        const int c = k % C, t = k / C;
        const int ky = t / KW, kx = t - ky * KW;
        const int iy = oy * stride - pad + ky, ix = ox * stride - pad + kx;
        if ((unsigned)iy < (unsigned)H && (unsigned)ix < (unsigned)W) x = src[(((long)n * C + c) * H + iy) * W + ix];
      }
      v[j] = x;
    }
    unsigned h[4], l[4];
#pragma unroll
    for (int j = 0; j < 4; ++j) {
      h[j] = pack_bf16(v[2 * j], v[2 * j + 1]);
      l[j] = pack_bf16(v[2 * j] - __uint_as_float(h[j] << 16), v[2 * j + 1] - __uint_as_float(h[j] & 0xffff0000u));
    }
    const int c8 = gidx * 8;
    char* d = dst + m * 4L * kp + (long)(c8 >> 5) * 128 + (c8 & 31) * 2;
    *(uint4*)d = make_uint4(h[0], h[1], h[2], h[3]);
    *(uint4*)(d + 64) = make_uint4(l[0], l[1], l[2], l[3]);
  }
}

__global__ __launch_bounds__(256) void weight_prep_pair_kernel(const float* __restrict__ w, const float* __restrict__ scale,
                                                              char* __restrict__ fwd, char* __restrict__ bwd, int N, int C,
                                                              int T) {
  const long nf = (long)N * T * (C >> 3);
  const long nb = bwd ? (long)C * T * (N >> 3) : 0;
  for (long i = (long)blockIdx.x * 256 + threadIdx.x; i < nf + nb; i += (long)gridDim.x * 256) {
    float v[8];
    char* d;
    if (i < nf) {
      const int cg = (int)(i % (C >> 3));
      const long r = i / (C >> 3);
      const int t = (int)(r % T), n = (int)(r / T);
      const float sc = scale ? scale[n] : 1.f;
#pragma unroll
      for (int j = 0; j < 8; ++j) v[j] = w[((long)n * C + cg * 8 + j) * T + t] * sc;
      const int k = t * C + cg * 8;
      d = fwd + (long)n * 4L * T * C + (long)(k >> 5) * 128 + (k & 31) * 2;
    } else {
      const long ib = i - nf;
      const int ng = (int)(ib % (N >> 3));
      const long r = ib / (N >> 3);
      const int t = (int)(r % T), c = (int)(r / T);
#pragma unroll
      for (int j = 0; j < 8; ++j) {
        const int n = ng * 8 + j;
        v[j] = w[((long)n * C + c) * T + t] * (scale ? scale[n] : 1.f);
      }
      const int k = t * N + ng * 8;
      d = bwd + (long)c * 4L * T * N + (long)(k >> 5) * 128 + (k & 31) * 2;
    }
    unsigned h[4], l[4];
#pragma unroll
    for (int j = 0; j < 4; ++j) {
      h[j] = pack_bf16(v[2 * j], v[2 * j + 1]);
      l[j] = pack_bf16(v[2 * j] - __uint_as_float(h[j] << 16), v[2 * j + 1] - __uint_as_float(h[j] & 0xffff0000u));
    }
    *(uint4*)d = make_uint4(h[0], h[1], h[2], h[3]);
    *(uint4*)(d + 64) = make_uint4(l[0], l[1], l[2], l[3]);
  }
}

__global__ __launch_bounds__(256) void slab_reduce_kernel(const float* __restrict__ slabs, const float* __restrict__ scale,
                                                         float* __restrict__ dw, int S, int N, int C, int T) {
  const long total = (long)N * T * (C >> 2);
  const long slab = (long)N * T * C;
  const int part = threadIdx.x & 3;
  for (long i = ((long)blockIdx.x * 256 + threadIdx.x) >> 2; i < total; i += ((long)gridDim.x * 256) >> 2) {
    const int cg = (int)(i % (C >> 2));
    const long r = i / (C >> 2);
    const int t = (int)(r % T), n = (int)(r / T);
    const float* p = slabs + ((long)n * T + t) * C + cg * 4;
    f32x4 a = {0.f, 0.f, 0.f, 0.f};
    for (int s0 = part; s0 < S; s0 += 32) {
      f32x4 v[8];
#pragma unroll
      for (int u = 0; u < 8; ++u) {
        const int s_ = s0 + 4 * u;
        v[u] = s_ < S ? *(const f32x4*)(p + s_ * slab) : f32x4{0.f, 0.f, 0.f, 0.f};
      }
      a += ((v[0] + v[1]) + (v[2] + v[3])) + ((v[4] + v[5]) + (v[6] + v[7]));
    }
#pragma unroll
    for (int e = 0; e < 4; ++e) {
      a[e] += __shfl_xor(a[e], 1, 64);
      a[e] += __shfl_xor(a[e], 2, 64);
    }
    if (part == 0) {
      const float sc = scale ? scale[n] : 1.f;
      float* o = dw + ((long)n * C + cg * 4) * T + t;
      o[0] = a.x * sc; o[T] = a.y * sc; o[2 * T] = a.z * sc; o[3 * T] = a.w * sc;
    }
  }
}

__global__ __launch_bounds__(256) void im2col_pair_kernel(const char* __restrict__ src, char* __restrict__ dst,
                                                         long pixels, int H, int W, int C, int KH, int KW) {
  const int slots = C >> 2;
  const int T = KH * KW;
  const long total = pixels * T * slots;
  for (long i = (long)blockIdx.x * 256 + threadIdx.x; i < total; i += (long)gridDim.x * 256) {
    const int s = (int)(i % slots);
    const long mt = i / slots;
    const int t = (int)(mt % T);
    const long m = mt / T;
    const int x = (int)(m % W), y = (int)((m / W) % H);
    const int yy = y + t / KW - KH / 2, xx = x + t % KW - KW / 2;
    uint4 v = make_uint4(0u, 0u, 0u, 0u);
    if ((unsigned)yy < (unsigned)H && (unsigned)xx < (unsigned)W)
      v = *(const uint4*)(src + (m + (long)(yy - y) * W + (xx - x)) * 4L * C + s * 16L);
    *(uint4*)(dst + (m * T + t) * 4L * C + s * 16L) = v;
  }
}
}

extern "C" int ovis_split_pair_f32(const float* src, long src_row_stride, void* dst_pair, long rows, int cols,
                                   void* stream) {
  if (rows < 0 || cols < 0) return OVIS_EINVAL;
  if (rows == 0 || cols == 0) return OVIS_OK;
  if (!src || !dst_pair) return OVIS_EINVAL;
  if (cols % 32 != 0 || src_row_stride % 4 != 0 || ((uintptr_t)src & 15) || ((uintptr_t)dst_pair & 15))
    return OVIS_ERANGE;
  const long total = rows * (cols / 8);
  const long blocks = (total + 255) / 256;
  const unsigned grid = (unsigned)(blocks < 8L * OVIS_NUM_CU ? blocks : 8L * OVIS_NUM_CU);
  hipLaunchKernelGGL(split_pair_kernel, dim3(grid), dim3(256), 0, (hipStream_t)stream, src, src_row_stride,
                     (char*)dst_pair, rows, cols);
  OVIS_LAUNCH_CHECK();
  return OVIS_OK;
}

extern "C" int ovis_gate_split_pair_f32(const float* dy, long dy_row_stride, const void* gate, int gate_is_pair,
                                        void* dst_pair, float* g_f32, long rows, int cols, const float* g_pooled,
                                        int pool_rows, void* stream) {
  return ovis_gate_split_pair_rows_f32(dy, dy_row_stride, gate, gate_is_pair, dst_pair, g_f32, rows, cols, g_pooled,
                                       pool_rows, nullptr, nullptr, stream);
}

extern "C" int ovis_gate_split_pair_rows_f32(const float* dy, long dy_row_stride, const void* gate, int gate_is_pair,
                                             void* dst_pair, float* g_f32, long rows, int cols, const float* g_pooled,
                                             int pool_rows, const float* g_selected, const int32_t* group_slot,
                                             void* stream) {
  if (rows < 0 || cols < 0) return OVIS_EINVAL;
  if (rows == 0 || cols == 0) return OVIS_OK;
  if ((!dy && !g_pooled && !g_selected) || !dst_pair || ((g_pooled || g_selected) && (pool_rows <= 0 || rows % pool_rows != 0)) ||
      ((g_selected != nullptr) != (group_slot != nullptr)))
    return OVIS_EINVAL;
  if (cols % 32 != 0 || dy_row_stride % 4 != 0 || ((uintptr_t)dy & 15) || ((uintptr_t)dst_pair & 15) ||
      ((uintptr_t)gate & 15) || ((uintptr_t)g_f32 & 15) || ((uintptr_t)g_pooled & 15) || ((uintptr_t)g_selected & 15))
    return OVIS_ERANGE;
  const float pool_scale = g_pooled ? 1.f / (float)pool_rows : 0.f;
  const long total = rows * (cols / 8);
  const long blocks = (total + 255) / 256;
  const unsigned grid = (unsigned)(blocks < 8L * OVIS_NUM_CU ? blocks : 8L * OVIS_NUM_CU);
  hipStream_t s = (hipStream_t)stream;
#define OVIS_GS(GP_, WF_)                                                                                          \
  hipLaunchKernelGGL((gate_split_pair_kernel<GP_, WF_>), dim3(grid), dim3(256), 0, s, dy, dy_row_stride, gate,      \
                     (char*)dst_pair, g_f32, rows, cols, g_pooled, pool_rows, pool_scale, g_selected, group_slot)
  if (gate_is_pair) { if (g_f32) OVIS_GS(true, true); else OVIS_GS(true, false); }
  else { if (g_f32) OVIS_GS(false, true); else OVIS_GS(false, false); }
#undef OVIS_GS
  OVIS_LAUNCH_CHECK();
  return OVIS_OK;
}

extern "C" int ovis_im2col_nchw_pair_f32(const float* src, void* dst_pair, int num, int channels, int height,
                                         int width, int kh, int kw, int stride, int pad, int k_padded, void* stream) {
  if (num < 0 || channels <= 0 || height <= 0 || width <= 0 || kh <= 0 || kw <= 0 || stride <= 0 || pad < 0)
    return OVIS_EINVAL;
  if (num == 0) return OVIS_OK;
  if (!src || !dst_pair) return OVIS_EINVAL;
  if (k_padded % 32 != 0 || k_padded < kh * kw * channels || ((uintptr_t)dst_pair & 15)) return OVIS_ERANGE;
  const int ho = (height + 2 * pad - kh) / stride + 1, wo = (width + 2 * pad - kw) / stride + 1;
  if (ho <= 0 || wo <= 0) return OVIS_EINVAL;
  const long total = (long)num * ho * wo * (k_padded / 8);
  const long blocks = (total + 255) / 256;
  const unsigned grid = (unsigned)(blocks < 16L * OVIS_NUM_CU ? blocks : 16L * OVIS_NUM_CU);
  hipLaunchKernelGGL(im2col_nchw_pair_kernel, dim3(grid), dim3(256), 0, (hipStream_t)stream, src, (char*)dst_pair, num,
                     channels, height, width, kh, kw, stride, pad, ho, wo, k_padded);
  OVIS_LAUNCH_CHECK();
  return OVIS_OK;
}

extern "C" int ovis_weight_prep_pair_f32(const float* weight, const float* scale, void* fwd_pair, void* bwd_pair,
                                        int out_channels, int in_channels, int taps, void* stream) {
  if (out_channels <= 0 || in_channels <= 0 || taps <= 0) return OVIS_EINVAL;
  if (!weight || !fwd_pair) return OVIS_EINVAL;
  if (in_channels % 32 != 0 || (bwd_pair && out_channels % 32 != 0) || ((uintptr_t)fwd_pair & 15) ||
      ((uintptr_t)bwd_pair & 15))
    return OVIS_ERANGE;
  const long total = (long)out_channels * taps * (in_channels / 8) + (bwd_pair ? (long)in_channels * taps * (out_channels / 8) : 0);
  const long blocks = (total + 255) / 256;
  const unsigned grid = (unsigned)(blocks < 8L * OVIS_NUM_CU ? blocks : 8L * OVIS_NUM_CU);
  hipLaunchKernelGGL(weight_prep_pair_kernel, dim3(grid), dim3(256), 0, (hipStream_t)stream, weight, scale, (char*)fwd_pair,
                     (char*)bwd_pair, out_channels, in_channels, taps);
  OVIS_LAUNCH_CHECK();
  return OVIS_OK;
}

extern "C" int ovis_slab_reduce_f32(const float* slabs, const float* scale, float* dweight, int slices, int out_channels,
                                    int in_channels, int taps, void* stream) {
  if (slices <= 0 || out_channels <= 0 || in_channels <= 0 || taps <= 0) return OVIS_EINVAL;
  if (!slabs || !dweight) return OVIS_EINVAL;
  if (in_channels % 4 != 0 || ((uintptr_t)slabs & 15)) return OVIS_ERANGE;
  const long total = 4L * out_channels * taps * (in_channels / 4);
  const long blocks = (total + 255) / 256;
  const unsigned grid = (unsigned)(blocks < 8L * OVIS_NUM_CU ? blocks : 8L * OVIS_NUM_CU);
  hipLaunchKernelGGL(slab_reduce_kernel, dim3(grid), dim3(256), 0, (hipStream_t)stream, slabs, scale, dweight, slices,
                     out_channels, in_channels, taps);
  OVIS_LAUNCH_CHECK();
  return OVIS_OK;
}

extern "C" int ovis_im2col_pair(const void* src_pair, void* dst_pair, long num, int height, int width, int channels,
                                int kh, int kw, void* stream) {
  if (num < 0 || height <= 0 || width <= 0 || channels < 0 || kh <= 0 || kw <= 0 || !(kh & 1) || !(kw & 1))
    return OVIS_EINVAL;
  if (num == 0 || channels == 0) return OVIS_OK;
  if (!src_pair || !dst_pair) return OVIS_EINVAL;
  if (channels % 32 != 0 || ((uintptr_t)src_pair & 15) || ((uintptr_t)dst_pair & 15)) return OVIS_ERANGE;
  const long total = num * height * width * kh * kw * (channels / 4);
  const long blocks = (total + 255) / 256;
  const unsigned grid = (unsigned)(blocks < 16L * OVIS_NUM_CU ? blocks : 16L * OVIS_NUM_CU);
  hipLaunchKernelGGL(im2col_pair_kernel, dim3(grid), dim3(256), 0, (hipStream_t)stream, (const char*)src_pair,
                     (char*)dst_pair, num * height * width, height, width, channels, kh, kw);
  OVIS_LAUNCH_CHECK();
  return OVIS_OK;
}

extern "C" int ovis_split_gemm_tn_slices(long m, int n, int channels, int taps) {
  if (m <= 0 || n <= 0 || channels <= 0 || taps <= 0) return 1;
  const long tiles = (long)(n / 128) * ((long)taps * channels / 128);
  const long steps = (m + 31) / 32;
  if (tiles <= 0) return 1;
  const long slots = 2L * OVIS_NUM_CU;
  if (steps >= 128 && steps <= 1100 && tiles <= 64) {
    long s = slots / tiles;
    if (s > steps / 16) s = steps / 16;
    if (s > 256) s = 256;
    return (int)(s < 1 ? 1 : s);
  }
  long s_max = (4 * slots + tiles - 1) / tiles;
  if (s_max > steps / 8) s_max = steps / 8;
  if (s_max > 256) s_max = 256;
  if (s_max < 1) s_max = 1;
  long best = 1;
  double best_score = -1.0;
  for (long s = 1; s <= s_max; ++s) {
    const long blocks = s * tiles, rounds = (blocks + slots - 1) / slots;
    double score = (double)blocks / (double)(rounds * slots);
    if (rounds == 1) score *= 0.97 * (double)blocks / (double)slots;
    if (rounds > 2) score -= 0.01 * (double)(rounds - 2);
    if (score > best_score + 1e-9) { best_score = score; best = s; }
  }
  return (int)best;
}

extern "C" int ovis_split_gemm_pair_tn(const void* g_pair, long g_row_bytes, const void* x_pair, long x_row_bytes,
                                       float* c_slabs, int slices, long m, int n, int channels, int taps_h,
                                       int taps_w, int height, int width, void* stream) {
  if (m < 0 || n <= 0 || channels <= 0 || taps_h <= 0 || taps_w <= 0 || !(taps_h & 1) || !(taps_w & 1) || slices <= 0)
    return OVIS_EINVAL;
  if (!g_pair || !x_pair || !c_slabs || m > 0x7fffff00L) return OVIS_EINVAL;
  const int T = taps_h * taps_w;
  if (T > 1 && (height <= 0 || width <= 0)) return OVIS_EINVAL;
  if (n % 128 != 0 || channels % 128 != 0 ||
      g_row_bytes % 16 != 0 || x_row_bytes % 16 != 0 || ((uintptr_t)g_pair & 15) || ((uintptr_t)x_pair & 15) ||
      ((uintptr_t)c_slabs & 15))
    return OVIS_ERANGE;
  SplitGemmTnArgs p;
  p.G = (const char*)g_pair; p.g_rs = g_row_bytes; p.X = (const char*)x_pair; p.x_rs = x_row_bytes;
  p.C = c_slabs; p.M = m; p.N = n; p.ch = channels; p.T = T; p.H = height; p.W = width; p.KH = taps_h; p.KW = taps_w;
  p.slices = slices;
  const long steps = (m + 31) / 32;
  p.steps_per_slice = (int)((steps + slices - 1) / slices);
  const int tiles_i = n / 128, tiles_j = (int)((long)T * channels / 128);
  p.g_major = tiles_i >= channels / 128 ? 1 : 0;
  const long nblocks = (long)tiles_i * tiles_j * slices;
  if (nblocks > 0x7fffffffL) return OVIS_ERANGE;
  hipStream_t s = (hipStream_t)stream;
  const int lds = 2 * 2 * 32 * 512;
  if (T > 1 && (long)height * width <= 64) {
    static bool attr_set_s = false;
    if (!attr_set_s) {
      OVIS_HIP_TRY(hipFuncSetAttribute((const void*)split_gemm_tn_kernel<true, true>, hipFuncAttributeMaxDynamicSharedMemorySize, lds));
      attr_set_s = true;
    }
    hipLaunchKernelGGL((split_gemm_tn_kernel<true, true>), dim3((unsigned)nblocks), dim3(256), lds, s, p, tiles_i, tiles_j, (int)nblocks);
  } else if (T > 1) {
    static bool attr_set_c = false;
    if (!attr_set_c) {
      OVIS_HIP_TRY(hipFuncSetAttribute((const void*)split_gemm_tn_kernel<true>, hipFuncAttributeMaxDynamicSharedMemorySize, lds));
      attr_set_c = true;
    }
    hipLaunchKernelGGL(split_gemm_tn_kernel<true>, dim3((unsigned)nblocks), dim3(256), lds, s, p, tiles_i, tiles_j, (int)nblocks);
  } else {
    static bool attr_set = false;
    if (!attr_set) {
      OVIS_HIP_TRY(hipFuncSetAttribute((const void*)split_gemm_tn_kernel<false>, hipFuncAttributeMaxDynamicSharedMemorySize, lds));
      attr_set = true;
    }
    hipLaunchKernelGGL(split_gemm_tn_kernel<false>, dim3((unsigned)nblocks), dim3(256), lds, s, p, tiles_i, tiles_j, (int)nblocks);
  }
  OVIS_LAUNCH_CHECK();
  return OVIS_OK;
}

namespace {
struct SplitGemmPlan {
  int mode, narrow, stages, kslices, steps_per_slice, tiles_m, tiles_n;
};

SplitGemmPlan split_gemm_plan(long m, int n, int channels, int channels2, int taps_h, int taps_w, int width, int config) {
  SplitGemmPlan q;
  const int T = taps_h * taps_w;
  q.narrow = n <= 64;
  const int bn = q.narrow ? 64 : 128;
  q.tiles_m = (int)((m + 127) / 128);
  q.tiles_n = (n + bn - 1) / bn;
  const long nb = (long)q.tiles_m * q.tiles_n;
  q.mode = PLAIN;
  if (T > 1) q.mode = (!q.narrow && !(config & 4) && (taps_h / 2) * width + taps_w / 2 <= kHalo && T <= 16) ? HALO : SHIFTED;
  const int cpb = channels / 32;
  const int units = q.mode == HALO ? cpb : T * cpb + channels2 / 32;
  q.kslices = 1;
  q.steps_per_slice = units;
  bool sliced_two_stage = false;
  if (!(config & 8) && !q.narrow && nb <= OVIS_NUM_CU / 2) {
    const int min_units = q.mode == HALO ? 1 : 8;
    long s = units / min_units;
    const long want = (2L * OVIS_NUM_CU + nb - 1) / nb;
    if (s > want) s = want;
    if (s > 64) s = 64;
    if (s >= 2) {
      q.steps_per_slice = (int)((units + s - 1) / s);
      q.kslices = (units + q.steps_per_slice - 1) / q.steps_per_slice;
    }
  } else if (!(config & 8) && (config & 0x10000) && !q.narrow && q.mode != HALO) {
    int sl = 1;
    if (nb <= OVIS_NUM_CU && units >= 64) sl = 4;
    else if (nb <= OVIS_NUM_CU && units >= 32) sl = 2;
    else if (nb < 3L * OVIS_NUM_CU && units >= 128) sl = 2;
    if (sl > 1) {
      q.steps_per_slice = (units + sl - 1) / sl;
      q.kslices = (units + q.steps_per_slice - 1) / q.steps_per_slice;
    }
  } else if (!(config & 8) && !q.narrow && q.mode != HALO && nb < 3L * OVIS_NUM_CU && units >= 16) {
    const double slab_unit = (double)m * n * 4.0 / 34.4e6;
    double best = 1e30;
    int best_sl = 1;
    for (int sl : {1, 2, 3, 4, 6, 8}) {
      const int steps = (units + sl - 1) / sl;
      if (sl > 1 && steps < 8) break;
      const long items = nb * ((units + steps - 1) / steps);
      const long full = items / (2L * OVIS_NUM_CU), rest = items % (2L * OVIS_NUM_CU);
      const double t2 = 12.8 + 1.0 * steps, t1 = 8.0 + 0.785 * steps;
      const double t = full * t2 + (rest == 0 ? 0.0 : (rest > OVIS_NUM_CU ? t2 : t1)) + (sl > 1 ? 4.0 + 0.9 * sl * slab_unit : 0.0);
      if (t < best) { best = t; best_sl = sl; }
    }
    if (best_sl > 1) {
      q.steps_per_slice = (units + best_sl - 1) / best_sl;
      q.kslices = (units + q.steps_per_slice - 1) / q.steps_per_slice;
      sliced_two_stage = true;
    }
  }
  if (const int forced = (config >> 8) & 0xff; forced > 0 && !q.narrow) {
    const int sl = forced < units ? forced : units;
    q.steps_per_slice = (units + sl - 1) / sl;
    q.kslices = (units + q.steps_per_slice - 1) / q.steps_per_slice;
  }
  const long total = nb * q.kslices;
  q.stages = 2;
  if (q.mode == HALO || q.narrow) q.stages = 1;
  else if (sliced_two_stage) q.stages = 2;
  else if (total >= 8L * OVIS_NUM_CU || (total >= 4L * OVIS_NUM_CU && (T > 1 || q.tiles_n >= 8))) q.stages = 1;
  else {
    const long slots2 = 2L * OVIS_NUM_CU, slots1 = 4L * OVIS_NUM_CU;
    if (total > slots2 && total <= slots2 + slots2 / 4 && total <= slots1) q.stages = 1;
    if (total > slots1 && total <= slots1 + slots1 / 16) q.stages = 1;
  }
  if (config & 1) q.stages = 1;
  if ((config & 2) && q.mode != HALO && !q.narrow) q.stages = 2;
  return q;
}
}

extern "C" size_t ovis_split_gemm_pair_workspace_bytes_ex(long m, int n, int channels, int channels2, int taps_h,
                                                          int taps_w, int width, int config) {
  if (m <= 0 || n <= 0 || channels <= 0 || taps_h <= 0 || taps_w <= 0 || config < 0 || config > 0x1ffff) return 0;
  const SplitGemmPlan q = split_gemm_plan(m, n, channels, channels2, taps_h, taps_w, width, config);
  return q.kslices > 1 ? (size_t)q.kslices * (size_t)m * (size_t)n * sizeof(float) : 0;
}

extern "C" size_t ovis_split_gemm_pair_workspace_bytes(long m, int n, int channels, int channels2, int taps_h,
                                                       int taps_w, int width) {
  return ovis_split_gemm_pair_workspace_bytes_ex(m, n, channels, channels2, taps_h, taps_w, width, 0);
}

static int split_gemm_pair_impl(const void* a_pair, long a_row_bytes, const void* a2_pair, long a2_row_bytes,
                                const void* b_pair, long b_row_bytes, float* c, long ldc, void* c_pair,
                                long c_pair_row_bytes, const float* bias, const float* residual, long ldr,
                                const void* residual_pair, long residual_pair_row_bytes,
                                const void* gate_pair, long gate_row_bytes, long m, int n, int channels, int channels2,
                                int taps_h, int taps_w, int height, int width, int flip, int relu, void* workspace,
                                size_t workspace_bytes, int config, void* stream, float* pool = nullptr, int pool_rows = 0,
                                float pool_scale = 1.f) {
  if (m < 0 || n < 0 || channels < 0 || channels2 < 0 || taps_h <= 0 || taps_w <= 0 || !(taps_h & 1) || !(taps_w & 1))
    return OVIS_EINVAL;
  if (m == 0 || n == 0) return OVIS_OK;
  if (!a_pair || !b_pair || (!c && !c_pair && !pool) || channels == 0 || m > 0x7fffff00L) return OVIS_EINVAL;
  if (pool && (pool_rows < 32 || pool_rows > 64 || ((uintptr_t)pool & 15))) return OVIS_ERANGE;
  const int T = taps_h * taps_w;
  if (T > 1 && (height <= 0 || width <= 0 || height > 32767 || width > 32767 || channels2 != 0)) return OVIS_EINVAL;
  if (channels2 != 0 && !a2_pair) return OVIS_EINVAL;
  const bool dual = residual_pair && gate_pair && !residual;
  if (!dual && (residual != nullptr) + (residual_pair != nullptr) + (gate_pair != nullptr) > 1) return OVIS_EINVAL;
  if (dual && T > 1) return OVIS_ERANGE;
  if (channels % 32 != 0 || channels2 % 32 != 0 || n % 4 != 0 || (c_pair && n % 32 != 0) || a_row_bytes % 16 != 0 ||
      a2_row_bytes % 16 != 0 || b_row_bytes % 16 != 0 || ((uintptr_t)a_pair & 15) || ((uintptr_t)a2_pair & 15) ||
      ((uintptr_t)b_pair & 15) || ((uintptr_t)c & 15) || ((uintptr_t)c_pair & 15) || ((uintptr_t)bias & 15) ||
      ((uintptr_t)residual & 15) || ((uintptr_t)workspace & 15) || ldc % 4 != 0 || ldr % 4 != 0 ||
      c_pair_row_bytes % 16 != 0)
    return OVIS_ERANGE;
  if (config < 0 || config > 0x1ffff) return OVIS_ERANGE;
  SplitGemmPlan q = split_gemm_plan(m, n, channels, channels2, taps_h, taps_w, width, config);
  if (q.kslices > 1 && (!workspace || workspace_bytes < (size_t)q.kslices * (size_t)m * (size_t)n * sizeof(float))) {
    q = split_gemm_plan(m, n, channels, channels2, taps_h, taps_w, width, config | 8);
  }
  SplitGemmArgs p;
  p.A = (const char*)a_pair; p.a_rs = a_row_bytes;
  p.A2 = (const char*)a2_pair; p.a2_rs = a2_row_bytes;
  p.B = (const char*)b_pair; p.b_rs = b_row_bytes;
  p.C = c; p.ldc = ldc; p.Cp = (char*)c_pair; p.cp_rs = c_pair_row_bytes;
  p.bias = bias; p.res = residual; p.ldr = ldr;
  p.resp = (const char*)residual_pair; p.resp_rs = residual_pair_row_bytes;
  p.gate = (const char*)gate_pair; p.gate_rs = gate_row_bytes;
  p.slab = q.kslices > 1 ? (float*)workspace : nullptr;
  p.pool = pool; p.pool_rows = pool_rows; p.pool_scale = pool_scale;
  p.M = m; p.N = n; p.ch = channels; p.ch2 = channels2; p.T = T; p.H = height; p.W = width; p.KH = taps_h; p.KW = taps_w;
  p.flip = flip; p.relu = relu;
  p.kslices = q.kslices; p.steps_per_slice = q.steps_per_slice;
  p.gw = (q.tiles_n % kGroupWidth == 0) ? kGroupWidth : (q.tiles_n % 4 == 0) ? 4 : q.tiles_n;
  const long ntiles = (long)q.tiles_m * q.tiles_n;
  const long nblocks = ntiles * q.kslices;
  if (nblocks > 0x7fffffffL) return OVIS_ERANGE;
  hipStream_t s = (hipStream_t)stream;
#define OVIS_SG_LAUNCH__(WM_, WN_, MODE_, NS_, OCC_, DUAL_, POOL_)                                                   \
  do {                                                                                                              \
    constexpr int a_rows = MODE_ == HALO ? WM_ * 64 + 2 * kHalo + 2 : WM_ * 64;                                      \
    constexpr int lds = NS_ * (a_rows * 128 + WN_ * 64 * 128);                                                       \
    static bool attr_set = false;                                                                                   \
    if (!attr_set) {                                                                                                \
      OVIS_HIP_TRY(hipFuncSetAttribute((const void*)split_gemm_kernel<WM_, WN_, MODE_, NS_, OCC_, DUAL_, POOL_>,    \
                                       hipFuncAttributeMaxDynamicSharedMemorySize, lds));                           \
      attr_set = true;                                                                                              \
    }                                                                                                               \
    hipLaunchKernelGGL((split_gemm_kernel<WM_, WN_, MODE_, NS_, OCC_, DUAL_, POOL_>), dim3((unsigned)nblocks),      \
                       dim3(WM_ * WN_ * 64), lds, s, p, q.tiles_n, (int)ntiles);                                    \
  } while (0)
#define OVIS_SG_LAUNCH_(WM_, WN_, MODE_, NS_, OCC_, DUAL_) OVIS_SG_LAUNCH__(WM_, WN_, MODE_, NS_, OCC_, DUAL_, false)
#define OVIS_SG_LAUNCH(WM_, WN_, MODE_, NS_, OCC_) OVIS_SG_LAUNCH_(WM_, WN_, MODE_, NS_, OCC_, false)
  if (pool) {
    if (dual || q.narrow || q.mode != PLAIN || q.kslices > 1) return OVIS_ERANGE;
    if (q.stages == 1) OVIS_SG_LAUNCH__(2, 2, PLAIN, 1, 4, false, true); else OVIS_SG_LAUNCH__(2, 2, PLAIN, 2, 2, false, true);
  } else if (dual) {
    if (q.narrow || q.mode != PLAIN || q.kslices > 1) return OVIS_ERANGE;
    if (q.stages == 1) OVIS_SG_LAUNCH_(2, 2, PLAIN, 1, 4, true); else OVIS_SG_LAUNCH_(2, 2, PLAIN, 2, 2, true);
  } else if (q.narrow) {
    if (q.mode == PLAIN) OVIS_SG_LAUNCH(2, 1, PLAIN, 1, 2); else OVIS_SG_LAUNCH(2, 1, SHIFTED, 1, 2);
  } else if (q.mode == HALO) {
    OVIS_SG_LAUNCH(2, 2, HALO, 1, 4);
  } else if (q.mode == SHIFTED) {
    if (q.stages == 1) OVIS_SG_LAUNCH(2, 2, SHIFTED, 1, 4); else OVIS_SG_LAUNCH(2, 2, SHIFTED, 2, 2);
  } else {
    if (q.stages == 1) OVIS_SG_LAUNCH(2, 2, PLAIN, 1, 4); else OVIS_SG_LAUNCH(2, 2, PLAIN, 2, 2);
  }
#undef OVIS_SG_LAUNCH__
#undef OVIS_SG_LAUNCH_
#undef OVIS_SG_LAUNCH
  OVIS_LAUNCH_CHECK();
  if (q.kslices > 1) {
    p.slab = (float*)workspace;
    const long total = m * (n / 4);
    const long blocks = (total + 255) / 256;
    const unsigned grid = (unsigned)(blocks < 8L * OVIS_NUM_CU ? blocks : 8L * OVIS_NUM_CU);
    hipLaunchKernelGGL(split_gemm_finish_kernel, dim3(grid), dim3(256), 0, s, p);
    OVIS_LAUNCH_CHECK();
  }
  return OVIS_OK;
}

extern "C" int ovis_split_gemm_pair(const void* a_pair, long a_row_bytes, const void* a2_pair, long a2_row_bytes,
                                    const void* b_pair, long b_row_bytes, float* c, long ldc, void* c_pair,
                                    long c_pair_row_bytes, const float* bias, const float* residual, long ldr, long m,
                                    int n, int channels, int channels2, int taps_h, int taps_w, int height, int width,
                                    int flip, int relu, void* workspace, size_t workspace_bytes, int config,
                                    void* stream) {
  return split_gemm_pair_impl(a_pair, a_row_bytes, a2_pair, a2_row_bytes, b_pair, b_row_bytes, c, ldc, c_pair,
                              c_pair_row_bytes, bias, residual, ldr, nullptr, 0, nullptr, 0, m, n, channels, channels2,
                              taps_h, taps_w, height, width, flip, relu, workspace, workspace_bytes, config, stream);
}

extern "C" int ovis_split_gemm_pair_rp(const void* a_pair, long a_row_bytes, const void* b_pair, long b_row_bytes,
                                       float* c, long ldc, void* c_pair, long c_pair_row_bytes, const float* bias,
                                       const void* residual_pair, long residual_pair_row_bytes, long m, int n,
                                       int channels, int relu, void* workspace, size_t workspace_bytes, int config,
                                       void* stream) {
  if (!residual_pair || n % 32 != 0 || residual_pair_row_bytes % 16 != 0 || ((uintptr_t)residual_pair & 15)) return OVIS_ERANGE;
  return split_gemm_pair_impl(a_pair, a_row_bytes, nullptr, 0, b_pair, b_row_bytes, c, ldc, c_pair, c_pair_row_bytes, bias,
                              nullptr, 0, residual_pair, residual_pair_row_bytes, nullptr, 0, m, n, channels, 0, 1, 1, 0, 0,
                              0, relu, workspace, workspace_bytes, config, stream);
}

extern "C" int ovis_split_gemm_pair_pool_supported(long m, int n, int channels, int pool_rows) {
  if (m <= 0 || n <= 0 || channels <= 0 || channels % 32 || n % 32 || pool_rows < 32 || pool_rows > 64) return 0;
  const SplitGemmPlan q = split_gemm_plan(m, n, channels, 0, 1, 1, 0, 0);
  return !q.narrow && q.mode == PLAIN && q.kslices == 1;
}

extern "C" int ovis_split_gemm_pair_rp_pool(const void* a_pair, long a_row_bytes, const void* b_pair, long b_row_bytes,
                                            float* c, long ldc, void* c_pair, long c_pair_row_bytes, const float* bias,
                                            const void* residual_pair, long residual_pair_row_bytes, long m, int n,
                                            int channels, int relu, float* pooled, int pool_rows, float pool_scale,
                                            void* stream) {
  if (!pooled) return OVIS_EINVAL;
  if (n % 32 != 0 || (residual_pair && (residual_pair_row_bytes % 16 != 0 || ((uintptr_t)residual_pair & 15)))) return OVIS_ERANGE;
  return split_gemm_pair_impl(a_pair, a_row_bytes, nullptr, 0, b_pair, b_row_bytes, c, ldc, c_pair, c_pair_row_bytes, bias,
                              nullptr, 0, residual_pair, residual_pair_row_bytes, nullptr, 0, m, n, channels, 0, 1, 1, 0, 0,
                              0, relu, nullptr, 0, 8, stream, pooled, pool_rows, pool_scale);
}

extern "C" int ovis_split_gemm_pair_gated(const void* a_pair, long a_row_bytes, const void* b_pair, long b_row_bytes,
                                          float* c, long ldc, void* c_pair, long c_pair_row_bytes,
                                          const void* gate_pair, long gate_row_bytes, long m, int n, int channels,
                                          int taps_h, int taps_w, int height, int width, int flip, int config,
                                          void* stream) {
  if (!gate_pair || gate_row_bytes % 16 != 0 || ((uintptr_t)gate_pair & 15) || n % 32 != 0) return OVIS_ERANGE;
  return split_gemm_pair_impl(a_pair, a_row_bytes, nullptr, 0, b_pair, b_row_bytes, c, ldc, c_pair, c_pair_row_bytes,
                              nullptr, nullptr, 0, nullptr, 0, gate_pair, gate_row_bytes, m, n, channels, 0, taps_h, taps_w,
                              height, width, flip, 0, nullptr, 0, config | 8, stream);
}

extern "C" int ovis_split_gemm_pair_gated_ws(const void* a_pair, long a_row_bytes, const void* b_pair, long b_row_bytes,
                                             float* c, long ldc, void* c_pair, long c_pair_row_bytes,
                                             const void* gate_pair, long gate_row_bytes, long m, int n, int channels,
                                             int taps_h, int taps_w, int height, int width, int flip, void* workspace,
                                             size_t workspace_bytes, int config, void* stream) {
  if (!gate_pair || gate_row_bytes % 16 != 0 || ((uintptr_t)gate_pair & 15) || n % 32 != 0) return OVIS_ERANGE;
  return split_gemm_pair_impl(a_pair, a_row_bytes, nullptr, 0, b_pair, b_row_bytes, c, ldc, c_pair, c_pair_row_bytes,
                              nullptr, nullptr, 0, nullptr, 0, gate_pair, gate_row_bytes, m, n, channels, 0, taps_h, taps_w,
                              height, width, flip, 0, workspace, workspace_bytes, config, stream);
}

extern "C" int ovis_split_gemm_pair_rp_gated(const void* a_pair, long a_row_bytes, const void* b_pair, long b_row_bytes,
                                             float* c, long ldc, void* c_pair, long c_pair_row_bytes,
                                             const void* residual_pair, long residual_pair_row_bytes,
                                             const void* gate_pair, long gate_row_bytes, long m, int n, int channels,
                                             int config, void* stream) {
  if (!residual_pair || !gate_pair || n % 32 != 0 || residual_pair_row_bytes % 16 != 0 || gate_row_bytes % 16 != 0 ||
      ((uintptr_t)residual_pair & 15) || ((uintptr_t)gate_pair & 15))
    return OVIS_ERANGE;
  if (n < 128) return OVIS_ERANGE;
  return split_gemm_pair_impl(a_pair, a_row_bytes, nullptr, 0, b_pair, b_row_bytes, c, ldc, c_pair, c_pair_row_bytes,
                              nullptr, nullptr, 0, residual_pair, residual_pair_row_bytes, gate_pair, gate_row_bytes, m, n,
                              channels, 0, 1, 1, 0, 0, 0, 0, nullptr, 0, config | 8, stream);
}

extern "C" int ovis_deform_conv_implicit_f32(const float* input_nhwc, const float* offset, const float* mask,
                                             const void* weight_pair, long weight_row_bytes, const float* bias,
                                             float* output, long ldc, int batch, int channels, int height, int width,
                                             int out_channels, int out_h, int out_w, int kernel_h, int kernel_w,
                                             int stride_h, int stride_w, int pad_h, int pad_w, int dil_h, int dil_w,
                                             int deformable_group, void* stream) {
  if (batch < 0 || channels <= 0 || height <= 0 || width <= 0 || out_channels <= 0 || out_h <= 0 || out_w <= 0 ||
      kernel_h <= 0 || kernel_w <= 0 || stride_h <= 0 || stride_w <= 0 || dil_h <= 0 || dil_w <= 0 || deformable_group <= 0)
    return OVIS_EINVAL;
  const long m = (long)batch * out_h * out_w;
  if (m == 0) return OVIS_OK;
  if (!input_nhwc || !offset || !weight_pair || !output) return OVIS_EINVAL;
  if ((long)batch * height * width * channels > 0x7fffffffL) return OVIS_ERANGE;
  if (channels % deformable_group != 0 || (channels / deformable_group) % 32 != 0 || out_channels % 4 != 0 || ldc % 4 != 0 ||
      weight_row_bytes % 16 != 0 || m > 0x7fffff00L || ((uintptr_t)input_nhwc & 15) || ((uintptr_t)weight_pair & 15) ||
      ((uintptr_t)output & 15) || ((uintptr_t)bias & 15))
    return OVIS_ERANGE;
  SplitGemmArgs p = {};
  p.B = (const char*)weight_pair; p.b_rs = weight_row_bytes;
  p.C = output; p.ldc = ldc; p.bias = bias;
  p.M = m; p.N = out_channels; p.ch = channels; p.ch2 = 0; p.T = kernel_h * kernel_w; p.H = height; p.W = width;
  p.KH = kernel_h; p.KW = kernel_w; p.flip = 0; p.relu = 0;
  p.kslices = 1; p.steps_per_slice = p.T * (channels / 32);
  p.dimg = input_nhwc; p.doff = offset; p.dmask = mask;
  p.Ho = out_h; p.Wo = out_w; p.sh = stride_h; p.sw = stride_w; p.ph = pad_h; p.pw = pad_w; p.dlh = dil_h; p.dlw = dil_w;
  p.dg = deformable_group;
  const int tiles_m = (int)((m + 127) / 128), tiles_n = (out_channels + 127) / 128;
  p.gw = (tiles_n % kGroupWidth == 0) ? kGroupWidth : (tiles_n % 4 == 0) ? 4 : tiles_n;
  const long ntiles = (long)tiles_m * tiles_n;
  if (ntiles > 0x7fffffffL) return OVIS_ERANGE;
  constexpr int lds = 128 * 128 + 128 * 128;
  static bool attr_set = false;
  if (!attr_set) {
    OVIS_HIP_TRY(hipFuncSetAttribute((const void*)split_gemm_kernel<2, 2, DEFORM, 1, 2>,
                                     hipFuncAttributeMaxDynamicSharedMemorySize, lds));
    attr_set = true;
  }
  hipLaunchKernelGGL((split_gemm_kernel<2, 2, DEFORM, 1, 2>), dim3((unsigned)ntiles), dim3(256), lds, (hipStream_t)stream, p,
                     tiles_n, (int)ntiles);
  OVIS_LAUNCH_CHECK();
  return OVIS_OK;
}
```

### cvpr22_cross_modal_pseudo_labeling_amd/layers/pair_bottleneck.py

```python
import torch
from torch.autograd import Function
from torch.autograd.function import once_differentiable

from .. import _C


def pair_weight(w2d):
    return _C.split_pair(w2d.contiguous())


def conv_weight_matrix(w):
    n, c, kh, kw = w.shape
    return w.permute(0, 2, 3, 1).reshape(n, kh * kw * c)


def conv_weight_matrix_t(w):
    n, c, kh, kw = w.shape
    return w.permute(1, 2, 3, 0).reshape(c, kh * kw * n)


def dw_pair(gp, xp, conv=None):
    n, k = gp.shape[1] // 2, xp.shape[1] // 2
    if _C.split_gemm_pair_tn_supported(n, k, conv):
        return _C.split_gemm_pair_tn(gp, xp, conv)
# ... 14 lines not shown

ONE_CALL_BACKWARD_ROWS = 40000

_WEIGHTS_EPOCH = [0]


def note_weights_written():
    _WEIGHTS_EPOCH[0] += 1


class WeightPrepPlan:

    def __init__(self, blocks):
        import numpy as np
        tile = _C.weight_prep_tile()
        self.max_taps = 1
        self.entries = {}
        rows, blk = [], []
        dev = blocks[0][1][0][0].device
        for key, convs in blocks:
            ws = [w for w, _ in convs]
            if not all(w.is_cuda and w.dtype == torch.float32 and w.dim() == 4 and w.is_contiguous() and w.device == dev
                       and w.shape[0] % 32 == 0 and w.shape[1] % 32 == 0 for w in ws):
                raise RuntimeError("WeightPrepPlan: contiguous float32 HIP weights with channel counts divisible by 32 expected")
            if len(convs) == 1:
                (w, sc), = convs
                n, c, t = w.shape[0], w.shape[1], w.shape[2] * w.shape[3]
                f = torch.empty((n, 2 * t * c), dtype=torch.bfloat16, device=dev)
                tb = torch.empty((c, 2 * t * n), dtype=torch.bfloat16, device=dev)
                if sc is not None and not (sc.is_cuda and sc.dtype == torch.float32 and sc.is_contiguous() and sc.numel() == n):
                    raise RuntimeError("WeightPrepPlan: scale must be a contiguous float32 [N] HIP tensor")
                self.max_taps = max(self.max_taps, t)
                rows.append((w.data_ptr(), 0 if sc is None else sc.data_ptr(), f.data_ptr(), tb.data_ptr(), 2 * f.stride(0),
                             2 * tb.stride(0), n | (c << 32), t))
                blk.extend((len(rows) - 1, ti) for ti in range((n // tile) * (c // tile)))
                self.entries[key] = [{"w": f, "wt": tb}, (w,), (sc,), None]
                continue
            (w1, _), (w2, _), (w3, _) = convs[:3]
            wd = convs[3][0] if len(convs) > 3 else None
            k3 = w3.shape[1] * w3.shape[2] * w3.shape[3]
            kd = wd.shape[1] * wd.shape[2] * wd.shape[3] if wd is not None else 0
            f1 = torch.empty((w1.shape[0], 2 * w1[0].numel()), dtype=torch.bfloat16, device=dev)
            f2 = torch.empty((w2.shape[0], 2 * w2[0].numel()), dtype=torch.bfloat16, device=dev)
            f3d = torch.empty((w3.shape[0], 2 * (k3 + kd)), dtype=torch.bfloat16, device=dev)
            fwd = [(f1, f1.data_ptr()), (f2, f2.data_ptr()), (f3d, f3d.data_ptr())] + ([(f3d, f3d.data_ptr() + 4 * k3)] if wd is not None else [])
            bwd = []
            for (w, sc), (fbuf, fptr) in zip(convs, fwd):
                n, c, t = w.shape[0], w.shape[1], w.shape[2] * w.shape[3]
                tb = torch.empty((c, 2 * t * n), dtype=torch.bfloat16, device=dev)
                bwd.append(tb)
                if sc is not None and not (sc.is_cuda and sc.dtype == torch.float32 and sc.is_contiguous() and sc.numel() == n):
                    raise RuntimeError("WeightPrepPlan: scale must be a contiguous float32 [N] HIP tensor")
                self.max_taps = max(self.max_taps, t)
                rows.append((w.data_ptr(), 0 if sc is None else sc.data_ptr(), fptr, tb.data_ptr(), 2 * fbuf.stride(0),
                             2 * tb.stride(0), n | (c << 32), t))
                blk.extend((len(rows) - 1, ti) for ti in range((n // tile) * (c // tile)))
            wp = {"w1": f1, "w2": f2, "w3": f3d[:, :2 * k3], "wd": f3d[:, 2 * k3:] if wd is not None else None,
                  "wts": tuple(bwd) + ((None,) if wd is None else ())}
            if wd is not None:
                wp["w3d"] = f3d
            self.entries[key] = [wp, tuple(w for w, _ in convs), tuple(sc for _, sc in convs), None]
        table = np.zeros((len(rows), 8), dtype=np.int64)
        for i, r in enumerate(rows):
            table[i] = r
        self.items = torch.from_numpy(table.view(np.uint8).reshape(-1)).to(dev)
        self.blocks = torch.tensor(blk, dtype=torch.int32, device=dev).reshape(-1, 2)
        self._weights = [w for e in self.entries.values() for w in e[1]]
        self._pointers = [w.data_ptr() for w in self._weights]
        self.epoch = -1
        self.event = self.stream = None
        self.rebuild = False

    def describes(self):
        return not self.rebuild and self._pointers == [w.data_ptr() for w in self._weights]

    def run(self):
        _C.weight_prep_pair_multi(self.items, self.blocks, self.max_taps)
        self.epoch = _WEIGHTS_EPOCH[0]
        for e in self.entries.values():
            e[3] = [w._version for w in e[1]]
        self.stream = torch.cuda.current_stream()
        self.event = torch.cuda.Event()
        self.event.record(self.stream)

    def lookup(self, key, scales):
        ent = self.entries.get(key)
        if ent is None or self.epoch != _WEIGHTS_EPOCH[0]:
            return None
        wp, ws, scs, versions = ent
        if len(scales) != len(scs) or any(a is not b for a, b in zip(scales, scs)):
            self.rebuild = True
            return None
        if versions != [w._version for w in ws]:
            return None
        cur = torch.cuda.current_stream()
        if cur != self.stream:
            cur.wait_event(self.event)
        return wp


_NAN_CELL = {}


def nan_placeholder(device, rows, cols):
    cell = _NAN_CELL.get(device)
    if cell is None:
        cell = _NAN_CELL[device] = torch.full((1,), float("nan"), dtype=torch.float32, device=device)
    return cell.expand(rows, cols)


def is_placeholder(t):
    return t is not None and t.numel() > 1 and all(st == 0 for st in t.stride())


class GradLink:

    __slots__ = ("grad_pair", "claimed")

    def __init__(self):
        self.grad_pair = None
        self.claimed = False


class _BottleneckPair(Function):
    @staticmethod
    def forward(ctx, x, xp, geom, w1, s1, b1, w2, s2, b2, w3, s3, b3, wd, sd, want_pair, wpairs, pool, want_f32=True,
                link_in=None, link_out=None, select=None, pool_only_ok=False):
        h, w = geom
        if xp is None:
            xp = _C.split_pair(x)
        kh, kw = w2.shape[2], w2.shape[3]
        need_bwd = any(ctx.needs_input_grad)
        wts = None
        if wpairs is None:
            p1, t1 = _C.weight_prep_pair(w1, s1, need_bwd)
            p2, t2 = _C.weight_prep_pair(w2, s2, need_bwd)
            p3, t3 = _C.weight_prep_pair(w3, s3, need_bwd)
            pd, td = _C.weight_prep_pair(wd, sd, need_bwd) if wd is not None else (None, None)
            wpairs = {"w1": p1, "w2": p2, "w3": p3, "wd": pd}
            wts = (t1, t2, t3, td)
        elif need_bwd:
            wts = wpairs.get("wts")
        f32 = bool(want_f32 or pool or not want_pair)
        x_real = x is not None and not is_placeholder(x)
        _, o1p = _C.split_gemm_pair(xp, wpairs["w1"], b1, None, True, False, True)
        _, o2p = _C.split_gemm_pair(o1p, wpairs["w2"], b2, None, True, False, True, conv=(h, w, kh, kw, False))
        if wd is not None:
            w3d = wpairs.get("w3d")
            if w3d is None:
                w3d = torch.cat([wpairs["w3"], wpairs["wd"]], 1)
            out, outp = _C.split_gemm_pair(o2p, w3d, b3, None, True, f32, want_pair, a2_pair=xp)
        elif x_real:
            out, outp = _C.split_gemm_pair(o2p, wpairs["w3"], b3, x, True, f32, want_pair)
        pooled_k = None
        if wd is None and not x_real:
            fused_pool = (pool and 32 <= h * w <= 64
                          and _C.split_gemm_pair_pool_supported(o2p.shape[0], wpairs["w3"].shape[0], o2p.shape[1] // 2, h * w))
            if fused_pool:
                keep = need_bwd or want_pair or select is not None or not pool_only_ok
                out, outp, pooled_k = _C.split_gemm_pair_rp_pool(o2p, wpairs["w3"], b3, xp, True, keep, want_pair, h * w)
                if out is None and outp is None:
                    out = nan_placeholder(pooled_k.device, o2p.shape[0], pooled_k.shape[1])
            else:
                out, outp = _C.split_gemm_pair(o2p, wpairs["w3"], b3, None, True, f32, want_pair, residual_pair=xp)
        if pooled_k is not None:
            pooled = pooled_k
        else:
            pooled = out.view(-1, h * w, out.shape[1]).mean(dim=1) if pool else None
        out_sel = out.view(-1, h * w, out.shape[1]).index_select(0, select) if (select is not None and f32) else None
        gate_src = out if out is not None else outp
        if out is None:
            out = nan_placeholder(outp.device, outp.shape[0], outp.shape[1] // 2)
        ctx.save_for_backward(xp, o1p, o2p, gate_src, w1, w2, w3, wd, s1, s2, s3, sd, select if out_sel is not None else None)
        ctx.wts = wts
        ctx.geom = (h, w, kh, kw)
        ctx.link_in = link_in if (wd is None and not x_real) else None
        ctx.link_out = link_out if not f32 else None
        ctx.set_materialize_grads(False)
        if outp is not None:
            ctx.mark_non_differentiable(outp)
        return out, outp, pooled, out_sel

    @staticmethod
    @once_differentiable
    def backward(ctx, dout, _dpair, dpooled, dsel):
        link_out, link_in = ctx.link_out, ctx.link_in
        linked = link_out.grad_pair if link_out is not None else None
        if link_out is not None:
            link_out.grad_pair = None
        if dout is None and dpooled is None and linked is None and dsel is None:
            return (None,) * 22
        xp, o1p, o2p, out, w1, w2, w3, wd, s1, s2, s3, sd, select = ctx.saved_tensors
        h, w, kh, kw = ctx.geom
        need = ctx.needs_input_grad
        need_x, need_w1, need_w2, need_w3, need_wd = need[0], need[3], need[6], need[9], need[12]
        wts = ctx.wts
        if wts is None:
            wts = tuple(_C.weight_prep_pair(t, sc, True)[1] if t is not None else None
                        for t, sc in ((w1, s1), (w2, s2), (w3, s3), (wd, sd)))
        t1, t2, t3, td = wts
        n3 = w3.shape[0]
        to_link = (need_x and wd is None and link_in is not None and xp.shape[1] // 2 >= 128)
        if linked is not None:
            if dout is not None and not is_placeholder(dout):
                raise RuntimeError("_BottleneckPair: a pair-only output received a real fp32 gradient next to the linked one "
                                   "(a second consumer of the placeholder: hook, retain_grad, slicing ...)")
            g3p, g3 = linked, None
        else:
            sel_grad = slot = None
            if dsel is not None:
                if dout is None and dpooled is None:
                    dpooled = dsel.new_zeros((out.shape[0] // (h * w), n3))
                slot = torch.full((out.shape[0] // (h * w),), -1, dtype=torch.int32, device=dsel.device)
                slot[select] = torch.arange(select.numel(), dtype=torch.int32, device=dsel.device)
                sel_grad = dsel.reshape(-1, n3)
            g3p, g3 = _C.gate_split_pair(None if dout is None else dout.reshape(-1, n3), out,
                                         want_f32=(wd is None and need_x and not to_link), pooled=dpooled, pool_rows=h * w,
                                         selected=sel_grad, group_slot=slot)
        if (ONE_CALL_BACKWARD_ROWS and linked is not None and wd is None and to_link and need_w1 and need_w2 and need_w3
                and 0 < g3p.shape[0] <= ONE_CALL_BACKWARD_ROWS and t1 is not None and t2 is not None and t3 is not None
                and n3 % 128 == 0 and w1.shape[0] % 128 == 0 and kh % 2 == 1 and kw % 2 == 1):
            from ..engine.trainer import branch_stream
            gx, dw1, dw2, dw3 = _C.bottleneck_identity_backward(g3p, xp, o1p, o2p, t1, t2, t3, (s1, s2, s3), (h, w, kh, kw),
                                                               (w1.shape, w2.shape, w3.shape), branch_stream())
            link_in.grad_pair = gx
            dx = nan_placeholder(gx.device, xp.shape[0], xp.shape[1] // 2)
            return (dx, None, None, dw1, None, None, dw2, None, None, dw3, None, None, None, None, None, None, None, None, None,
                    None, None, None)
        dw3 = _dw(g3p, o2p, w3, s3) if need_w3 else None
        _, g2p = _C.split_gemm_pair_gated(g3p, t3, o2p)
        dw2 = _dw(g2p, o1p, w2, s2, (h, w, kh, kw)) if need_w2 else None
        dx = dw1 = dwd = None
        if need_x or need_w1:
            _, g1p = _C.split_gemm_pair_gated(g2p, t2, o1p, conv=(h, w, kh, kw, True))
            if need_w1:
                dw1 = _dw(g1p, xp, w1, s1)
            if need_x:
                if to_link:
                    _, link_in.grad_pair = _C.split_gemm_pair_rp_gated(g1p, t1, g3p, xp)
                    dx = nan_placeholder(g1p.device, xp.shape[0], xp.shape[1] // 2)
                else:
                    if wd is not None:
                        res, _ = _C.split_gemm_pair(g3p, td)
                        dx, _ = _C.split_gemm_pair(g1p, t1, None, res)
                    elif g3 is not None:
                        dx, _ = _C.split_gemm_pair(g1p, t1, None, g3)
                    else:
                        dx, _ = _C.split_gemm_pair(g1p, t1, None, None, False, True, False, residual_pair=g3p)
        if wd is not None and need_wd:
            dwd = _dw(g3p, xp, wd, sd)
        return (dx, None, None, dw1, None, None, dw2, None, None, dw3, None, None, dwd, None, None, None, None, None, None,
                None, None, None)


def bottleneck_pair(x, xp, geom, w1, b1, w2, b2, w3, b3, wd=None, want_pair=False, wpairs=None, pool=False,
                    scales=(None, None, None, None), want_f32=True, select=None, pool_only_ok=False):
    s1, s2, s3, sd = scales
    pair_only = want_pair and not want_f32 and not pool
    link_in = getattr(xp, "_ovis_grad_link", None) if (xp is not None and (x is None or is_placeholder(x))) else None
    if link_in is not None and torch.is_grad_enabled():
        if link_in.claimed:
            raise RuntimeError("bottleneck_pair: a block output kept in pair layout only can feed one block -- its fp32 "
                               "handle is a placeholder, so the gradients of two consumers could not be summed")
        link_in.claimed = True
    link_out = GradLink() if pair_only else None
    out, outp, pooled, out_sel = _BottleneckPair.apply(x, xp, geom, w1, s1, b1, w2, s2, b2, w3, s3, b3, wd, sd, want_pair,
                                                       wpairs, pool, want_f32, link_in, link_out, select, pool_only_ok)
    if out_sel is not None:
        out._ovis_selected = (select, out_sel)
    if link_out is not None and outp is not None:
        outp._ovis_grad_link = link_out
    return (out, outp, pooled) if pool else (out, outp)


class _ConvSamePair(Function):

    @staticmethod
    def forward(ctx, x2d, geom, w, b, relu, prepared=None):
        h, wd_ = geom
        n, c, kh, kw = w.shape
        xp = _C.split_pair(x2d)
        if prepared is not None:
            wp, wt = prepared["w"], prepared["wt"]
        else:
            wp, wt = _C.weight_prep_pair(w, None, ctx.needs_input_grad[0])
        y, _ = _C.split_gemm_pair(xp, wp, b, None, relu, True, False, conv=(h, wd_, kh, kw, False))
        ctx.wt = wt
        ctx.save_for_backward(xp, y if relu else None, w)
        ctx.geom = (h, wd_, kh, kw)
        ctx.has_bias = b is not None
        return y

    @staticmethod
    @once_differentiable
    def backward(ctx, dy):
        xp, y, w = ctx.saved_tensors
        h, wd_, kh, kw = ctx.geom
        n, c = w.shape[0], w.shape[1]
        need_b = ctx.has_bias and ctx.needs_input_grad[3]
        gp, g32 = _C.gate_split_pair(dy.reshape(-1, n), y, want_f32=need_b)
        dx = dw = db = None
        if ctx.needs_input_grad[0]:
            dx, _ = _C.split_gemm_pair(gp, ctx.wt, conv=(h, wd_, kh, kw, True))
        if ctx.needs_input_grad[2]:
            dw = _dw(gp, xp, w, None, (h, wd_, kh, kw))
        if need_b:
            db = g32.sum(0)
        return dx, None, dw, db, None, None


def conv_same_pair(x2d, geom, w, b=None, relu=False, prepared=None):
    return _ConvSamePair.apply(x2d, geom, w, b, relu, prepared)
```

### cvpr22_cross_modal_pseudo_labeling_amd/modeling/roi_heads.py

```python
import torch
import torch.nn.functional as F
from torch import nn

from .. import _C
from ..layers import (Conv2d, ConvTranspose2d, ROIAlign, linear_mfma, smooth_l1_loss, smooth_l1_picked, stochastic_mask_bce,
                      text_logits, weighted_cross_entropy)
from .backbone import ResNetHead
from .box_coder import BoxCoder
from .matcher import BalancedPositiveNegativeSampler, Matcher
from .structures import BoxList, PastedMasks, PolygonMasks, box_iou, boxlist_nms, cat_boxlist


def _cat(tensors, dim=0):
    return tensors[0] if len(tensors) == 1 else torch.cat(tensors, dim)


class Pooler(nn.Module):
    def __init__(self, output_size, scales, sampling_ratio):
        super().__init__()
        if len(scales) != 1:
            raise NotImplementedError("single-level pooler only (C4)")
        self.pooler = ROIAlign(output_size, spatial_scale=scales[0], sampling_ratio=sampling_ratio)
        self.output_size = output_size

# ... 542 lines not shown
        if mask_targets.numel() == 0:
            return mask_logits.sum() * 0
        self.mask_targets, self.positive_inds = mask_targets, pos
        return F.binary_cross_entropy_with_logits(mask_logits[pos, labels_pos], mask_targets, reduction="none").mean()


def paste_mask_in_image(mask, box, im_h, im_w, thresh=0.5, padding=1):
    M = mask.shape[-1]
    scale = float(M + 2 * padding) / M
    padded = mask.new_zeros((M + 2 * padding, M + 2 * padding))
    padded[padding:-padding, padding:-padding] = mask
    w_half = (box[2] - box[0]) * 0.5 * scale
    h_half = (box[3] - box[1]) * 0.5 * scale
    x_c, y_c = (box[2] + box[0]) * 0.5, (box[3] + box[1]) * 0.5
    bx = torch.stack((x_c - w_half, y_c - h_half, x_c + w_half, y_c + h_half)).to(torch.int32).tolist()
    w = max(bx[2] - bx[0] + 1, 1)
    h = max(bx[3] - bx[1] + 1, 1)
    resized = F.interpolate(padded[None, None].float(), size=(h, w), mode="bilinear", align_corners=False)[0, 0]
    resized = resized > thresh
    im_mask = torch.zeros((im_h, im_w), dtype=torch.bool, device=mask.device)
    x0, x1 = max(bx[0], 0), min(bx[2] + 1, im_w)
    y0, y1 = max(bx[1], 0), min(bx[3] + 1, im_h)
    if x1 > x0 and y1 > y0:
        im_mask[y0:y1, x0:x1] = resized[(y0 - bx[1]):(y1 - bx[1]), (x0 - bx[0]):(x1 - bx[0])]
    return im_mask


class Masker:
    def __init__(self, threshold=0.5, padding=1):
        self.threshold, self.padding = threshold, padding

    def __call__(self, masks, boxlist):
        im_w, im_h = boxlist.size
        P = masks.shape[0]
        if P == 0:
            return masks.new_empty((0, 1, im_h, im_w), dtype=torch.bool)
        M, pad = masks.shape[-1], self.padding
        scale = float(M + 2 * pad) / M
        b = boxlist.bbox
        w_half = (b[:, 2] - b[:, 0]) * 0.5 * scale
        h_half = (b[:, 3] - b[:, 1]) * 0.5 * scale
        x_c, y_c = (b[:, 2] + b[:, 0]) * 0.5, (b[:, 3] + b[:, 1]) * 0.5
        boxes = torch.stack((x_c - w_half, y_c - h_half, x_c + w_half, y_c + h_half), 1).to(torch.int32).tolist()
        padded = masks.new_zeros((P, 1, M + 2 * pad, M + 2 * pad), dtype=torch.float32)
        padded[:, 0, pad:-pad, pad:-pad] = masks[:, 0]
        out = torch.zeros((P, 1, im_h, im_w), dtype=torch.bool, device=masks.device)
        for i, bx in enumerate(boxes):
            w = max(bx[2] - bx[0] + 1, 1)
            h = max(bx[3] - bx[1] + 1, 1)
            x0, x1 = max(bx[0], 0), min(bx[2] + 1, im_w)
            y0, y1 = max(bx[1], 0), min(bx[3] + 1, im_h)
            if x1 > x0 and y1 > y0:
                resized = F.interpolate(padded[i:i + 1], size=(h, w), mode="bilinear", align_corners=False)[0, 0]
                out[i, 0, y0:y1, x0:x1] = resized[(y0 - bx[1]):(y1 - bx[1]), (x0 - bx[0]):(x1 - bx[0])] > self.threshold
        return out


class ROIMaskHead(nn.Module):
    def __init__(self, cfg, in_channels):
        super().__init__()
        self.cfg = cfg
        self.share = cfg.MODEL.ROI_MASK_HEAD.SHARE_BOX_FEATURE_EXTRACTOR
        self.feature_extractor = ResNet50Conv5ROIFeatureExtractor(cfg, cfg.MODEL.ROI_MASK_HEAD)
        self.predictor = MaskRCNNC4Predictor(cfg, self.feature_extractor.out_channels)
        self.loss_evaluator = MaskRCNNLossComputation(cfg)
        self.cls_agnostic_mask = cfg.MODEL.CLS_AGNOSTIC_MASK
        mh = cfg.MODEL.ROI_MASK_HEAD
        self.masker = Masker(threshold=mh.POSTPROCESS_MASKS_THRESHOLD, padding=1) if mh.POSTPROCESS_MASKS else None
        if self.masker is not None and self.masker.threshold < 0:
            raise NotImplementedError("POSTPROCESS_MASKS_THRESHOLD < 0 (the reference's un-thresholded debugging paste)")
        self.log = "N/A"
        self.avg_uncertain = "N/A"

    def forward(self, features, proposals, targets=None, compute_uncertain=False, eps=None):
        if self.training:
            sel = positives_index(proposals)
            if sel is not None:
                proposals = [positive_proposals(p) for p in proposals]
            else:
                positive_inds = [p.get_field("labels") > 0 for p in proposals]
                proposals = [p[i] for p, i in zip(proposals, positive_inds)]
                sel = _cat(positive_inds, 0)
        if self.training and self.share:
            fl = features.permute(0, 2, 3, 1) if features.dim() == 4 else None
            if fl is not None and fl.is_contiguous() and not features.is_contiguous():
                x = fl[sel].permute(0, 3, 1, 2)
            else:
                x = features[sel]
        else:
            x = self.feature_extractor(features, proposals)
        if self.training:
            return x, proposals, dict(loss_mask=self.fused_training_loss(x, proposals, targets, compute_uncertain, eps))
        if compute_uncertain:
            mask_logits, scale = self.predictor(x, True, eps=eps)
            self.log, self.avg_uncertain = scale.max(), scale.mean()
        else:
            mask_logits = self.predictor(x)
        if not self.training:
            prob = mask_logits.sigmoid()
            if self.cls_agnostic_mask:
                prob = prob[:, 1][:, None]
            else:
                labels = _cat([b.get_field("labels") for b in proposals], 0)
                prob = prob[torch.arange(prob.shape[0], device=prob.device), labels][:, None]
            results = []
            for p, b in zip(prob.split([len(b) for b in proposals], 0), proposals):
                out = b.copy_with_fields(b.fields())
                out.add_field("mask", p if self.masker is None else self.masker(p, b))
                results.append(out)
            return x, results, {}
        loss_mask = self.loss_evaluator(proposals, mask_logits, targets)
        return x, proposals, dict(loss_mask=loss_mask)


def _mask_fused_training_loss(self, x, proposals, targets, compute_uncertain=False, eps=None):
    mu, sigma = self.predictor.forward_parts(x)
    if compute_uncertain and sigma is not None:
        self.log, self.avg_uncertain = sigma.max(), sigma.mean()
        if eps is None:
            eps = torch.randn((1, *mu.shape), device=mu.device, dtype=mu.dtype)
        else:
            eps = eps[:, : mu.shape[0]].to(mu.device)
        return self.loss_evaluator.fused(proposals, mu, sigma, eps, targets)
    return self.loss_evaluator.fused(proposals, mu, None, None, targets)


ROIMaskHead.fused_training_loss = _mask_fused_training_loss


class CombinedROIHeads(nn.ModuleDict):
    batch_branches = True

    def __init__(self, cfg, in_channels, is_teacher=False):
        heads = [("box", ROIBoxHead(cfg, in_channels, is_teacher))]
        if cfg.MODEL.MASK_ON:
            heads.append(("mask", ROIMaskHead(cfg, in_channels)))
        super().__init__(heads)
        self.cfg = cfg
        self.mask_on = cfg.MODEL.MASK_ON
        if self.mask_on and cfg.MODEL.ROI_MASK_HEAD.SHARE_BOX_FEATURE_EXTRACTOR:
            self.mask.feature_extractor = self.box.feature_extractor

    def branches_batchable(self, feat):
        return (self.training and feat.is_cuda and (not self.mask_on or (self.mask.share and self.mask.cls_agnostic_mask))
                and self.batch_branches)

    def forward_branches(self, feat, branches):
        box = self.box
        with torch.no_grad():
            sampled = box.loss_evaluator.subsample_many([(br["proposals"], br["targets"]) for br in branches])
        rois = _C.rois_from_boxes([p.bbox for props in sampled for p in props],
                                  [img for br in branches for img in br["image_ids"]])
        sel_pos = positives_index([p for props in sampled for p in props]) if self.mask_on else None
        x = box.feature_extractor.forward_rois([feat], rois, select=sel_pos)
        pooled = box.predictor.pooled(x)
        counts = [sum(len(p) for p in props) for props in sampled]
        out, off = [], 0
        for br, props, cnt in zip(branches, sampled, counts):
            box.predictor.set_class_embeddings(br["cls_embs"])
            class_logits, box_regression = box.predictor(pooled[off:off + cnt])
            box.loss_evaluator._proposals = props
            lc, lb = box.loss_evaluator(class_logits, box_regression)
            out.append(dict(loss_classifier=lc, loss_box_reg=lb))
            off += cnt
        if self.mask_on:
            mask = self.mask
            sel = sel_pos
            if sel is not None:
                pos_all = [[positive_proposals(p) for p in props] for props in sampled]
            else:
                pos_masks = [[p.get_field("labels") > 0 for p in props] for props in sampled]
                sel = _cat([m for ms in pos_masks for m in ms], 0)
                pos_all = [[p[m] for p, m in zip(props, ms)] for props, ms in zip(sampled, pos_masks)]
            handed = getattr(x, "_ovis_selected", None)
            fl = x.permute(0, 2, 3, 1)
            if handed is not None and handed[0] is sel:
                xs = handed[1].view(sel.numel(), x.shape[2], x.shape[3], x.shape[1]).permute(0, 3, 1, 2)
            else:
                xs = fl[sel].permute(0, 3, 1, 2) if (fl.is_contiguous() and not x.is_contiguous()) else x[sel]
            off = 0
            for br, pos_props, losses in zip(branches, pos_all, out):
                k = sum(len(p) for p in pos_props)
                losses["loss_mask"] = mask.fused_training_loss(xs[off:off + k], pos_props, br["targets"],
                                                               br.get("compute_uncertain", False), br.get("eps"))
                off += k
        return out

    def forward(self, features, proposals, targets=None, bbox_only=False, compute_uncertain=False, eps=None,
                is_eval_func=False):
        losses, package_x = {}, {}
        gt_boxes = self.cfg.MODEL.GT_BOX_EVAL and is_eval_func and not self.training
        if gt_boxes:
            device = features[0].device if isinstance(features, (list, tuple)) else features.device
            proposals = []
            for t in targets:
                det = t.copy_with_fields(["labels"])
                det.add_field("objectness", t.get_field("labels") * 0.0 + 1.0)
                proposals.append(det.to(device))
        x, detections, loss_box = self.box(features, proposals, targets)
        if gt_boxes:
            for det, tar in zip(detections, targets):
                assert len(det) == len(tar), "GT_BOX_EVAL keeps one detection per ground-truth box"
        package_x["bbox"] = x
        losses.update(loss_box)
        if self.mask_on and not bbox_only:
            mask_features = features
            if self.training and self.cfg.MODEL.ROI_MASK_HEAD.SHARE_BOX_FEATURE_EXTRACTOR:
                mask_features = x
            x, detections, loss_mask = self.mask(mask_features, detections, targets, compute_uncertain, eps=eps)
            package_x["mask"] = x
            losses.update(loss_mask)
        return package_x, detections, losses
```

### include/ovis_hip.h

```cpp
#ifndef OVIS_HIP_H_
#define OVIS_HIP_H_

#include <stddef.h>
#include <stdint.h>

#ifdef __cplusplus
extern "C" {
#endif

#define OVIS_OK 0
#define OVIS_EINVAL (-1)
#define OVIS_ENOSPC (-2)
#define OVIS_ERANGE (-3)

const char* ovis_version(void);

int ovis_roi_align_forward_f32(const float* input, const float* rois, float* output,
                               int num_rois, int batch, int channels, int height,
                               int width, int pooled_h, int pooled_w,
                               float spatial_scale, int sampling_ratio, void* stream);

size_t ovis_roi_align_forward_workspace_bytes(int num_rois, int height, int width);
int ovis_roi_align_forward_mfma_supported(int height, int width, int pooled_h, int pooled_w);
int ovis_roi_align_forward_ws_f32(const float* input, const float* rois, float* output,
                                  int num_rois, int batch, int channels, int height, int width,
                                  int pooled_h, int pooled_w, float spatial_scale,
                                  int sampling_ratio, void* workspace, size_t workspace_bytes,
                                  void* stream);

int ovis_roi_align_forward_strided_from_nhwc_f32(const float* input_nhwc, const float* rois, void* output, int num_rois,
                                                 int batch, int channels, int height, int width, int pooled_h,
                                                 int pooled_w, int bin_stride, float spatial_scale, int sampling_ratio,
                                                 int pair_out, void* stream);

int ovis_roi_align_backward_f32(const float* grad_output, const float* rois,
                                float* grad_input, int num_rois, int batch,
                                int channels, int height, int width, int pooled_h,
                                int pooled_w, float spatial_scale, int sampling_ratio,
                                void* stream);

size_t ovis_roi_align_backward_workspace_bytes(int num_rois, int batch, int height, int width);
int ovis_roi_align_backward_plane_supported(int height, int width, int pooled_h, int pooled_w);
int ovis_roi_align_backward_ws_f32(const float* grad_output, const float* rois,
                                   float* grad_input, int num_rois, int batch, int channels,
                                   int height, int width, int pooled_h, int pooled_w,
                                   float spatial_scale, int sampling_ratio, void* workspace,
                                   size_t workspace_bytes, void* stream);
int ovis_roi_align_backward_strided_ws_f32(const float* grad_output, const float* rois, float* grad_input,
                                           int num_rois, int batch, int channels, int height, int width,
                                           int pooled_h, int pooled_w, int bin_stride, float spatial_scale,
                                           int sampling_ratio, void* workspace, size_t workspace_bytes, void* stream);

size_t ovis_roi_align_backward_strided_nhwc_workspace_bytes(int num_rois, int batch, int channels, int height, int width);
int ovis_roi_align_backward_strided_nhwc_ws_f32(const float* grad_output_nhwc, const float* rois, float* grad_input,
                                                int num_rois, int batch, int channels, int height, int width,
                                                int pooled_h, int pooled_w, int bin_stride, float spatial_scale,
                                                int sampling_ratio, void* workspace, size_t workspace_bytes,
                                                void* stream);

size_t ovis_nms_workspace_bytes(int num_boxes);
int ovis_nms_f32(const float* boxes, const float* scores, int num_boxes, float threshold,
                 int ge_mode, void* workspace, size_t workspace_bytes, int64_t* keep_out,
                 int32_t* num_keep, void* stream);
int ovis_nms_grouped_f32(const float* boxes, const float* scores, const int32_t* groups, int num_boxes,
                         float threshold, int ge_mode, void* workspace, size_t workspace_bytes,
                         int64_t* keep_out, int32_t* num_keep, void* stream);

size_t ovis_nms_presorted_workspace_bytes(int num_images, int num_boxes);
int ovis_nms_presorted_batched_f32(const float* boxes, const int32_t* drop, int num_images, int num_boxes,
                                   float threshold, int ge_mode, int below, void* workspace, size_t workspace_bytes,
                                   int64_t* keep_out, int32_t* num_keep, void* stream);

size_t ovis_topk_sorted_workspace_bytes(int num_rows, int row_len);
int ovis_topk_sorted_f32(const float* scores, long row_stride, int num_rows, int row_len, int k, float* out_scores,
                         int64_t* out_idx, void* workspace, size_t workspace_bytes, void* stream);

int ovis_rpn_decode_f32(const float* box_regression, long reg_stride_image, long reg_stride_position,
                        long reg_stride_channel, const int64_t* topk_idx, const float* cell_anchors,
                        const float* image_wh, int num_images, int num_candidates, int anchors_per_position,
                        int feature_width, float anchor_stride, float weight_x, float weight_y, float weight_w,
                        float weight_h, float xform_clip, float min_size, float* boxes, int32_t* drop, void* stream);

#define OVIS_BOX_DECODE_MAX_IMAGES 16
int ovis_box_decode_f32(const float* rel_codes, long codes_row_stride, const float* boxes, long boxes_row_stride,
                        long num_rows, int boxes_per_row, float weight_x, float weight_y, float weight_w,
                        float weight_h, float xform_clip, int num_images, const int32_t* rows_per_image,
                        const float* image_wh, float* decoded, void* stream);

int ovis_rois_from_boxes_f32(const float* const* boxes, const int32_t* boxes_per_image, const int32_t* image_ids,
                             int num_images, float* rois, void* stream);

int ovis_smooth_l1_picked_fwd_bwd_f32(const float* box_regression, long regression_row_stride, int num_rows,
                                      int num_columns, const float* regression_targets, long targets_row_stride,
                                      const int64_t* positives, const int64_t* labels, int num_positives, int column0,
                                      float beta, float denominator, float* loss, float* grad_regression, void* stream);

int ovis_roi_pool_forward_f32(const float* input, const float* rois, float* output, int32_t* argmax,
                              int num_rois, int batch, int channels, int height, int width,
                              int pooled_h, int pooled_w, float spatial_scale, void* stream);
int ovis_roi_pool_backward_f32(const float* grad_output, const int32_t* argmax, const float* rois,
                               float* grad_input, int num_rois, int batch, int channels, int height,
                               int width, int pooled_h, int pooled_w, void* stream);

int ovis_deform_psroi_pool_forward_f32(const float* data, const float* rois, const float* trans, float* out,
                                       float* out_count, int num_rois, int batch, int channels, int height, int width,
                                       int channels_trans, int no_trans, float spatial_scale, int output_dim,
                                       int group_size, int pooled_size, int part_size, int sample_per_part,
                                       float trans_std, void* stream);
int ovis_deform_psroi_pool_backward_f32(const float* grad_out, const float* out_count, const float* data,
                                        const float* rois, const float* trans, float* grad_data, float* grad_trans,
                                        int num_rois, int batch, int channels, int height, int width,
                                        int channels_trans, int no_trans, float spatial_scale, int output_dim,
                                        int group_size, int pooled_size, int part_size, int sample_per_part,
                                        float trans_std, void* stream);

int ovis_sigmoid_focal_loss_forward_f32(const float* logits, const int32_t* targets,
                                        float* losses, int num, int num_classes,
                                        float gamma, float alpha, void* stream);
int ovis_sigmoid_focal_loss_backward_f32(const float* logits, const int32_t* targets,
                                         const float* d_losses, float* d_logits, int num,
                                         int num_classes, float gamma, float alpha,
                                         void* stream);

int ovis_split_bf16x3_f32(const float* src, long src_row_stride, void* dst_bf16, long rows,
                          int cols, int mode, void* stream);

int ovis_im2col_split_bf16x3_f32(const float* src, void* dst_bf16, long num, int height,
                                 int width, int channels, int kh, int kw, int flip, void* stream);

int ovis_bias_act_f32(float* y, const float* bias, const float* residual, long rows, int cols,
                      int relu, void* stream);

int ovis_split_pair_f32(const float* src, long src_row_stride, void* dst_pair, long rows,
                        int cols, void* stream);

int ovis_gate_split_pair_f32(const float* dy, long dy_row_stride, const void* gate, int gate_is_pair,
                             void* dst_pair, float* g_f32, long rows, int cols, const float* g_pooled,
                             int pool_rows, void* stream);
int ovis_gate_split_pair_rows_f32(const float* dy, long dy_row_stride, const void* gate, int gate_is_pair,
                                  void* dst_pair, float* g_f32, long rows, int cols, const float* g_pooled,
                                  int pool_rows, const float* g_selected, const int32_t* group_slot, void* stream);

int ovis_weight_prep_pair_f32(const float* weight, const float* scale, void* fwd_pair, void* bwd_pair,
                              int out_channels, int in_channels, int taps, void* stream);

int ovis_slab_reduce_f32(const float* slabs, const float* scale, float* dweight, int slices, int out_channels,
                         int in_channels, int taps, void* stream);

int ovis_im2col_pair(const void* src_pair, void* dst_pair, long num, int height, int width,
                     int channels, int kh, int kw, void* stream);

int ovis_split_gemm_pair_gated(const void* a_pair, long a_row_bytes, const void* b_pair, long b_row_bytes,
                               float* c, long ldc, void* c_pair, long c_pair_row_bytes, const void* gate_pair,
                               long gate_row_bytes, long m, int n, int channels, int taps_h, int taps_w,
                               int height, int width, int flip, int config, void* stream);

int ovis_split_gemm_pair_gated_ws(const void* a_pair, long a_row_bytes, const void* b_pair, long b_row_bytes,
                                  float* c, long ldc, void* c_pair, long c_pair_row_bytes, const void* gate_pair,
                                  long gate_row_bytes, long m, int n, int channels, int taps_h, int taps_w,
                                  int height, int width, int flip, void* workspace, size_t workspace_bytes,
                                  int config, void* stream);

int ovis_split_gemm_pair_rp_gated(const void* a_pair, long a_row_bytes, const void* b_pair, long b_row_bytes, float* c,
                                  long ldc, void* c_pair, long c_pair_row_bytes, const void* residual_pair,
                                  long residual_pair_row_bytes, const void* gate_pair, long gate_row_bytes, long m, int n,
                                  int channels, int config, void* stream);

int ovis_im2col_nchw_pair_f32(const float* src, void* dst_pair, int num, int channels, int height, int width,
                              int kh, int kw, int stride, int pad, int k_padded, void* stream);

size_t ovis_split_gemm_pair_workspace_bytes(long m, int n, int channels, int channels2, int taps_h, int taps_w,
                                            int width);
size_t ovis_split_gemm_pair_workspace_bytes_ex(long m, int n, int channels, int channels2, int taps_h, int taps_w,
                                               int width, int config);
int ovis_split_gemm_pair(const void* a_pair, long a_row_bytes, const void* a2_pair, long a2_row_bytes,
                         const void* b_pair, long b_row_bytes, float* c, long ldc, void* c_pair,
                         long c_pair_row_bytes, const float* bias, const float* residual, long ldr, long m,
                         int n, int channels, int channels2, int taps_h, int taps_w, int height, int width,
                         int flip, int relu, void* workspace, size_t workspace_bytes, int config, void* stream);
int ovis_split_gemm_pair_rp(const void* a_pair, long a_row_bytes, const void* b_pair, long b_row_bytes, float* c, long ldc,
                            void* c_pair, long c_pair_row_bytes, const float* bias, const void* residual_pair,
                            long residual_pair_row_bytes, long m, int n, int channels, int relu, void* workspace,
                            size_t workspace_bytes, int config, void* stream);

int ovis_split_gemm_tn_slices(long m, int n, int channels, int taps);
int ovis_split_gemm_pair_tn(const void* g_pair, long g_row_bytes, const void* x_pair, long x_row_bytes,
                            float* c_slabs, int slices, long m, int n, int channels, int taps_h,
                            int taps_w, int height, int width, void* stream);

int ovis_match_encode_f32(const float* gt_boxes, const int64_t* gt_labels, const float* proposals, int num_gt,
                          int num_proposals, float high_threshold, float low_threshold, int between_keeps_label,
                          float wx, float wy, float ww, float wh, int64_t* matched_idx, int64_t* labels,
                          float* regression_targets, void* stream);
int ovis_rpn_match_encode_f32(const float* gt_boxes, const float* anchors, const uint8_t* visibility, int num_gt,
                              int num_anchors, float high_threshold, float low_threshold, int allow_low_quality_matches,
                              float wx, float wy, float ww, float wh, uint32_t* best_per_gt_scratch, int64_t* labels,
                              float* regression_targets, void* stream);
int ovis_project_masks_f32(const uint8_t* masks, const int64_t* gt_index, const float* boxes, int num, int height,
                           int width, int resolution, int masks_are_bool, float* out, void* stream);
int ovis_sample_fg_bg(const int64_t* labels, int num, int batch_size, int max_positives, uint64_t seed,
                      int64_t* selected, int64_t* positive_slots, int32_t* counts, void* stream);
int ovis_project_pasted_masks_f32(const float* mask_probs, const float* gt_boxes, const int64_t* gt_index,
                                  const float* boxes, int num, int image_height, int image_width, int prob_resolution,
                                  int resolution, float threshold, float* out, void* stream);
int ovis_gather_rows(const int64_t* index, int num, const float* boxes_a, float* boxes_a_out, const float* boxes_b,
                     float* boxes_b_out, const int64_t* ints_a, int64_t* ints_a_out, const int64_t* ints_b,
                     int64_t* ints_b_out, void* stream);

int ovis_gemm_f32(const float* A, long a_row_stride, long a_k_stride, const float* B,
                  long b_row_stride, long b_k_stride, const float* bias, float* C,
                  long c_row_stride, int M, int N, int K, void* stream);

int ovis_gemm_ex_f32(const float* A, long a_row_stride, long a_k_stride, const float* B,
                     long b_row_stride, long b_k_stride, const float* bias, int bias_per_row,
                     float alpha, int accumulate, float* C, long c_row_stride, int M, int N, int K,
                     void* stream);

size_t ovis_gemm_f32_workspace_bytes(int M, int N, int K);
int ovis_gemm_ex_ws_f32(const float* A, long a_row_stride, long a_k_stride, const float* B,
                        long b_row_stride, long b_k_stride, const float* bias, int bias_per_row,
                        float alpha, int accumulate, float* C, long c_row_stride, int M, int N, int K,
                        void* workspace, size_t workspace_bytes, void* stream);

int ovis_region_noun_align_f32(const float* region_emb, const float* noun_emb, float* raw_scores,
                               float* sigmoid_scores, int64_t* best_region, int num_regions,
                               int num_nouns, int dim, void* stream);

int ovis_weighted_ce_fwd_bwd_f32(const float* logits, const int64_t* labels, float bg_weight,
                                 float* loss, float* dlogits, float* row_scratch, int num_rows,
                                 int num_classes, void* stream);
int ovis_mask_bce_stochastic_fwd_bwd_f32(const float* mu, const float* sigma, const float* eps,
                                         const int64_t* pos_index, const float* targets, float* loss,
                                         float* dmu, float* dsigma, float* row_scratch, int num_rois,
                                         int num_pos, int num_channels, int mask_pixels, int channel,
                                         void* stream);
int ovis_mask_bce_stochastic_classes_fwd_bwd_f32(const float* mu, const float* sigma, const float* eps,
                                                 const int64_t* pos_index, const int64_t* channels,
                                                 const float* targets, float* loss, float* dmu, float* dsigma,
                                                 float* row_scratch, int num_rois, int num_pos,
                                                 int num_channels, int mask_pixels, void* stream);

int ovis_deform_im2col_f32(const float* input, const float* offset, const float* mask, float* columns,
                           int num_images, int channels, int height, int width, int kernel_h,
                           int kernel_w, int pad_h, int pad_w, int stride_h, int stride_w,
                           int dilation_h, int dilation_w, int deformable_group, void* stream);
int ovis_deform_col2im_f32(const float* columns, const float* offset, const float* mask,
                           float* grad_input, int num_images, int channels, int height, int width,
                           int kernel_h, int kernel_w, int pad_h, int pad_w, int stride_h,
                           int stride_w, int dilation_h, int dilation_w, int deformable_group,
                           void* stream);
int ovis_deform_col2im_coord_f32(const float* columns, const float* input, const float* offset,
                                 const float* mask, float* grad_offset, float* grad_mask,
                                 int num_images, int channels, int height, int width, int kernel_h,
                                 int kernel_w, int pad_h, int pad_w, int stride_h, int stride_w,
                                 int dilation_h, int dilation_w, int deformable_group, void* stream);

int ovis_deform_conv_implicit_f32(const float* input_nhwc, const float* offset, const float* mask,
                                  const void* weight_pair, long weight_row_bytes, const float* bias, float* output,
                                  long ldc, int batch, int channels, int height, int width, int out_channels, int out_h,
                                  int out_w, int kernel_h, int kernel_w, int stride_h, int stride_w, int pad_h,
                                  int pad_w, int dil_h, int dil_w, int deformable_group, void* stream);

int ovis_text_embed_f32(const float* table, long table_rows, int dim, const int32_t* input_ids,
                        const int32_t* special_tokens_mask, int num_words, int max_tokens, float* out, void* stream);

int ovis_project_polygon_masks_f32(const float* coords, const int32_t* polygon_start, const int32_t* instance_start,
                                   const int64_t* gt_index, const float* boxes, int num, int image_width,
                                   int image_height, int resolution, float* out, void* stream);

int ovis_deform_im2col_pair_rows_f32(const float* input_nhwc, const float* offset, const float* mask, void* columns_pair,
                                     long columns_row_bytes, int batch, int channels, int height, int width, int out_h,
                                     int out_w, int kernel_h, int kernel_w, int stride_h, int stride_w, int pad_h, int pad_w,
                                     int dil_h, int dil_w, int deformable_group, void* stream);
int ovis_deform_col2im_rows_f32(const float* dcol_rows, long dcol_ld, const float* input_nhwc, const float* offset,
                                const float* mask, float* grad_input_nhwc, float* grad_offset, float* grad_mask, int batch,
                                int channels, int height, int width, int out_h, int out_w, int kernel_h, int kernel_w,
                                int stride_h, int stride_w, int pad_h, int pad_w, int dil_h, int dil_w, int deformable_group,
                                void* stream);

int ovis_split_gemm_pair_pool_supported(long m, int n, int channels, int pool_rows);
int ovis_split_gemm_pair_rp_pool(const void* a_pair, long a_row_bytes, const void* b_pair, long b_row_bytes, float* c,
                                 long ldc, void* c_pair, long c_pair_row_bytes, const float* bias,
                                 const void* residual_pair, long residual_pair_row_bytes, long m, int n, int channels,
                                 int relu, float* pooled, int pool_rows, float pool_scale, void* stream);

int ovis_sgd_momentum_multi_f32(const void* items, const void* blocks, int num_blocks, float lr, float weight_decay,
                                float momentum, int apply_weight_decay, void* stream);
int ovis_sgd_chunk_elements(void);

size_t ovis_bottleneck_identity_backward_workspace_bytes(long m, int channels, int mid_channels, int taps_h, int taps_w,
                                                         int width, int config);
int ovis_bottleneck_identity_backward(
    const void* g3_pair, long g3_row_bytes, const void* x_pair, long x_row_bytes, const void* o1_pair, long o1_row_bytes,
    const void* o2_pair, long o2_row_bytes, const void* t1_pair, long t1_row_bytes, const void* t2_pair, long t2_row_bytes,
    const void* t3_pair, long t3_row_bytes, const float* scale1, const float* scale2, const float* scale3, long m, int channels,
    int mid_channels, int taps_h, int taps_w, int height, int width, void* g2_pair, void* g1_pair, void* gx_pair, float* dw1,
    float* dw2, float* dw3, void* workspace, size_t workspace_bytes, int config, void* stream, void* side_stream);

int ovis_weight_prep_pair_multi_f32(const void* items, const void* blocks, int num_blocks, int max_taps, void* stream);
int ovis_weight_prep_tile(void);

#ifdef __cplusplus
}
#endif
#endif
```

Measured before the change: 60.64 images/sec.

## Store ROI-head bottleneck ReLU gate as byte mask and fuse selected-row gather into pool GEMM

In the last ROI-head bottleneck, the fused pool GEMM now writes only a one-byte-per-element ReLU mask, the pooled output, and the positive-ROI rows into a compact buffer. It no longer materializes the full fp32 output. Backward gate kernels read the byte mask instead of the fp32 or pair activation, and they reuse the group-slot map built in forward. The aim is to cut activation writes and reads plus a separate index_select pass. The cost is extra template specializations and scattered stores inside the epilogue.

```diff
diff --git a/cvpr22_cross_modal_pseudo_labeling_amd/_C.py b/cvpr22_cross_modal_pseudo_labeling_amd/_C.py
--- a/cvpr22_cross_modal_pseudo_labeling_amd/_C.py
+++ b/cvpr22_cross_modal_pseudo_labeling_amd/_C.py
@@ -670,11 +670,12 @@
         raise RuntimeError("gate_split_pair: pooled must be [rows / pool_rows, cols]")
     dev = dy.device if dy is not None else pooled.device
     is_pair = 0
+    byte_gate = gate is not None and gate.dtype == torch.uint8
     if gate is not None:
         is_pair = int(gate.dtype == torch.bfloat16)
         if not (gate.is_cuda and gate.is_contiguous() and gate.shape == (rows, cols * (2 if is_pair else 1))
-                and gate.dtype in (torch.bfloat16, torch.float32)):
-            raise RuntimeError("gate_split_pair: gate must be the contiguous fp32 or pair form of the forward output")
+                and gate.dtype in (torch.bfloat16, torch.float32, torch.uint8)):
+            raise RuntimeError("gate_split_pair: gate must be the contiguous fp32, pair or byte-mask form of the forward output")
     out = torch.empty((rows, 2 * cols), dtype=torch.bfloat16, device=dev)
     g32 = torch.empty((rows, cols), dtype=torch.float32, device=dev) if want_f32 else None
     if out.numel() == 0:
@@ -684,6 +685,15 @@
         if pool_rows <= 0 or rows % pool_rows or selected.dim() != 2 or selected.shape[1] != cols or \
                 selected.shape[0] % pool_rows or group_slot.numel() != rows // pool_rows:
             raise RuntimeError("gate_split_pair: selected must be [S * pool_rows, cols] and group_slot [rows / pool_rows]")
+    if byte_gate:
+        with _on(dev):
+            rc = _L.ovis_gate_split_pair_rows_bm_f32(0 if dy is None else dy.data_ptr(), 0 if dy is None else dy.stride(0),
+                                                     gate.data_ptr(), out.data_ptr(), 0 if g32 is None else g32.data_ptr(),
+                                                     rows, cols, 0 if pooled is None else pooled.data_ptr(), pool_rows,
+                                                     0 if selected is None else selected.data_ptr(),
+                                                     0 if group_slot is None else group_slot.data_ptr(), _stream())
+        _lib.check(rc, "gate_split_pair")
+        return out, g32
     with _on(dev):
         rc = _L.ovis_gate_split_pair_rows_f32(0 if dy is None else dy.data_ptr(), 0 if dy is None else dy.stride(0),
                                               0 if gate is None else gate.data_ptr(), is_pair, out.data_ptr(),
@@ -862,6 +872,40 @@
     return c, cp, pooled
 
 
+def split_gemm_pair_rp_pool_masked(a_pair, b_pair, bias, residual_pair, relu, pool_rows, group_slot=None, num_selected=0):
+    for t, name in ((a_pair, "a_pair"), (b_pair, "b_pair")) + (((residual_pair, "residual_pair"),) if residual_pair is not None else ()):
+        if not (t.is_cuda and t.dtype == torch.bfloat16 and t.dim() == 2 and t.stride(1) == 1):
+            raise RuntimeError(f"split_gemm_pair_rp_pool_masked: {name} must be a 2-D bfloat16 HIP tensor in pair layout")
+    m, ch = a_pair.shape[0], a_pair.shape[1] // 2
+    n, k = b_pair.shape[0], b_pair.shape[1] // 2
+    if k != ch or m % pool_rows or (residual_pair is not None and residual_pair.shape != (m, 2 * n)):
+        raise RuntimeError("split_gemm_pair_rp_pool_masked: shape mismatch")
+    dev = a_pair.device
+    pooled = torch.zeros((m // pool_rows, n), dtype=torch.float32, device=dev)
+    mask = torch.empty((m, n), dtype=torch.uint8, device=dev)
+    sel = None
+    if group_slot is not None:
+        group_slot = _dev(group_slot, "group_slot", torch.int32)
+        if group_slot.numel() != m // pool_rows or num_selected < 0:
+            raise RuntimeError("split_gemm_pair_rp_pool_masked: group_slot must be [M / pool_rows]")
+        sel = torch.empty((num_selected * pool_rows, n), dtype=torch.float32, device=dev)
+    if m == 0 or n == 0:
+        return pooled, mask, sel
+    no_sel = sel is None or sel.numel() == 0
+    if bias is not None:
+        bias = _dev(bias, "bias")
+    with _on(dev):
+        rc = _L.ovis_split_gemm_pair_rp_pool_masked(a_pair.data_ptr(), 2 * a_pair.stride(0), b_pair.data_ptr(), 2 * b_pair.stride(0),
+                                                    0, n, 0, 4 * n, 0 if bias is None else bias.data_ptr(),
+                                                    0 if residual_pair is None else residual_pair.data_ptr(),
+                                                    0 if residual_pair is None else 2 * residual_pair.stride(0), m, n, ch,
+                                                    int(bool(relu)), pooled.data_ptr(), int(pool_rows), 1.0 / pool_rows,
+                                                    mask.data_ptr(), n, 0 if no_sel else group_slot.data_ptr(),
+                                                    0 if no_sel else sel.data_ptr(), _stream())
+    _lib.check(rc, "split_gemm_pair_rp_pool_masked")
+    return pooled, mask, sel
+
+
 def weight_prep_pair(w, scale=None, want_transposed=False):
     if not (w.is_cuda and w.dtype == torch.float32 and w.dim() == 4):
         raise RuntimeError("weight_prep_pair: [N,C,KH,KW] float32 HIP tensor expected")
@@ -930,6 +974,31 @@
                                               2 * residual_pair.stride(0), gate_pair.data_ptr(), 2 * gate_pair.stride(0), m, n,
                                               ch, config, _stream())
     _lib.check(rc, "split_gemm_pair_rp_gated")
+    return c, cp
+
+
+def split_gemm_pair_rp_gated_bm(a_pair, b_pair, residual_pair, gate_mask, out_f32=False, out_pair=True, config=0):
+    for t, name in ((a_pair, "a_pair"), (b_pair, "b_pair"), (residual_pair, "residual_pair")):
+        if not (t.is_cuda and t.dtype == torch.bfloat16 and t.dim() == 2 and t.stride(1) == 1):
+            raise RuntimeError(f"split_gemm_pair_rp_gated_bm: {name} must be a 2-D bfloat16 HIP tensor in pair layout")
+    m, ch = a_pair.shape[0], a_pair.shape[1] // 2
+    n, k = b_pair.shape[0], b_pair.shape[1] // 2
+    if not (gate_mask.is_cuda and gate_mask.dtype == torch.uint8 and gate_mask.dim() == 2 and gate_mask.stride(1) == 1):
+        raise RuntimeError("split_gemm_pair_rp_gated_bm: gate_mask must be a 2-D uint8 HIP tensor")
+    if k != ch or gate_mask.shape != (m, n) or residual_pair.shape != (m, 2 * n):
+        raise RuntimeError("split_gemm_pair_rp_gated_bm: shape mismatch")
+    dev = a_pair.device
+    c = torch.empty((m, n), dtype=torch.float32, device=dev) if out_f32 else None
+    cp = torch.empty((m, 2 * n), dtype=torch.bfloat16, device=dev) if out_pair else None
+    if m == 0 or n == 0:
+        return c, cp
+    with _on(dev):
+        rc = _L.ovis_split_gemm_pair_rp_gated_bm(a_pair.data_ptr(), 2 * a_pair.stride(0), b_pair.data_ptr(),
+                                                 2 * b_pair.stride(0), 0 if c is None else c.data_ptr(), n,
+                                                 0 if cp is None else cp.data_ptr(), 4 * n, residual_pair.data_ptr(),
+                                                 2 * residual_pair.stride(0), gate_mask.data_ptr(), gate_mask.stride(0), m, n,
+                                                 ch, config, _stream())
+    _lib.check(rc, "split_gemm_pair_rp_gated_bm")
     return c, cp
 
 
diff --git a/cvpr22_cross_modal_pseudo_labeling_amd/_lib.py b/cvpr22_cross_modal_pseudo_labeling_amd/_lib.py
--- a/cvpr22_cross_modal_pseudo_labeling_amd/_lib.py
+++ b/cvpr22_cross_modal_pseudo_labeling_amd/_lib.py
@@ -51,6 +51,7 @@
     "ovis_bias_act_f32": (_i, [_vp, _vp, _vp, _l, _i, _i, _vp]),
     "ovis_split_pair_f32": (_i, [_vp, _l, _vp, _l, _i, _vp]),
     "ovis_gate_split_pair_rows_f32": (_i, [_vp, _l, _vp, _i, _vp, _vp, _l, _i, _vp, _i, _vp, _vp, _vp]),
+    "ovis_gate_split_pair_rows_bm_f32": (_i, [_vp, _l, _vp, _vp, _vp, _l, _i, _vp, _i, _vp, _vp, _vp]),
     "ovis_gate_split_pair_f32": (_i, [_vp, _l, _vp, _i, _vp, _vp, _l, _i, _vp, _i, _vp]),
     "ovis_im2col_nchw_pair_f32": (_i, [_vp, _vp] + [_i] * 9 + [_vp]),
     "ovis_weight_prep_pair_f32": (_i, [_vp, _vp, _vp, _vp, _i, _i, _i, _vp]),
@@ -63,7 +64,10 @@
     "ovis_split_gemm_pair_workspace_bytes": (_sz, [_l, _i, _i, _i, _i, _i, _i]),
     "ovis_split_gemm_pair_workspace_bytes_ex": (_sz, [_l, _i, _i, _i, _i, _i, _i, _i]),
     "ovis_split_gemm_pair_rp_gated": (_i, [_vp, _l, _vp, _l, _vp, _l, _vp, _l, _vp, _l, _vp, _l, _l, _i, _i, _i, _vp]),
+    "ovis_split_gemm_pair_rp_gated_bm": (_i, [_vp, _l, _vp, _l, _vp, _l, _vp, _l, _vp, _l, _vp, _l, _l, _i, _i, _i, _vp]),
     "ovis_split_gemm_pair_pool_supported": (_i, [_l, _i, _i, _i]),
+    "ovis_split_gemm_pair_rp_pool_masked": (_i, [_vp, _l, _vp, _l, _vp, _l, _vp, _l, _vp, _vp, _l, _l, _i, _i, _i, _vp, _i, _f,
+                                                 _vp, _l, _vp, _vp, _vp]),
     "ovis_split_gemm_pair_rp_pool": (_i, [_vp, _l, _vp, _l, _vp, _l, _vp, _l, _vp, _vp, _l, _l, _i, _i, _i, _vp, _i, _f, _vp]),
     "ovis_split_gemm_pair_rp": (_i, [_vp, _l, _vp, _l, _vp, _l, _vp, _l, _vp, _vp, _l, _l, _i, _i, _i, _vp, _sz, _i, _vp]),
     "ovis_split_gemm_pair": (_i, [_vp, _l, _vp, _l, _vp, _l, _vp, _l, _vp, _l, _vp, _vp, _l, _l] + [_i] * 9
diff --git a/cvpr22_cross_modal_pseudo_labeling_amd/csrc/split_gemm.hip b/cvpr22_cross_modal_pseudo_labeling_amd/csrc/split_gemm.hip
--- a/cvpr22_cross_modal_pseudo_labeling_amd/csrc/split_gemm.hip
+++ b/cvpr22_cross_modal_pseudo_labeling_amd/csrc/split_gemm.hip
@@ -12,6 +12,7 @@
 __device__ char g_zero_line[128];
 
 enum { PLAIN = 0, SHIFTED = 1, HALO = 2, DEFORM = 3 };
+enum { EXT_NONE = 0, EXT_BYTE_GATE = 1, EXT_MASK_OUT = 2 };
 constexpr int kHalo = 8;
 
 struct SplitGemmArgs {
@@ -29,6 +30,8 @@
   int kslices; int steps_per_slice;
   const float* dimg; const float* doff; const float* dmask;
   int Ho; int Wo; int sh; int sw; int ph; int pw; int dlh; int dlw; int dg;
+  unsigned char* mask; long mask_rs;
+  const int* group_slot; float* sel_out;
 };
 
 __device__ __forceinline__ void glds16(const char* gsrc, char* lds_wave_base) {
@@ -61,13 +64,19 @@
 
 __device__ __forceinline__ long epilogue_column_bytes(const SplitGemmArgs& p, int n, long poff) { return p.res ? (long)n * 4 : poff; }
 
+template <bool BYTES = false>
 __device__ __forceinline__ void epilogue_fetch4(const EpilogueSource& s, long m, long column_bytes, EpilogueOperands& o) {
   const char* q = s.base + m * s.row_bytes + column_bytes;
-  o.a = *(const uint2*)q;
-  o.b = *(const uint2*)(q + s.second);
-}
-
-template <bool DUAL = false>
+  if constexpr (BYTES) {
+    o.a = make_uint2(*(const unsigned*)q, 0u);
+    o.b = make_uint2(0u, 0u);
+  } else {
+    o.a = *(const uint2*)q;
+    o.b = *(const uint2*)(q + s.second);
+  }
+}
+
+template <bool DUAL = false, int EXT = EXT_NONE>
 __device__ __forceinline__ f32x4 epilogue_apply4(const SplitGemmArgs& p, long m, int n, long poff, f32x4 v, const f32x4& bias4,
                                                  const EpilogueOperands& o, uint2 gate2 = make_uint2(0u, 0u)) {
   if (p.bias) v += bias4;
@@ -83,7 +92,13 @@
   if (p.relu) {
     v.x = fmaxf(v.x, 0.f); v.y = fmaxf(v.y, 0.f); v.z = fmaxf(v.z, 0.f); v.w = fmaxf(v.w, 0.f);
   }
-  if (p.gate) {
+  if (EXT == EXT_BYTE_GATE) {
+    const unsigned g = DUAL ? gate2.x : o.a.x;
+    if (!(g & 0xffu)) v.x = 0.f;
+    if (!(g & 0xff00u)) v.y = 0.f;
+    if (!(g & 0xff0000u)) v.z = 0.f;
+    if (!(g & 0xff000000u)) v.w = 0.f;
+  } else if (p.gate) {
     const unsigned gx = DUAL ? gate2.x : o.a.x, gy = DUAL ? gate2.y : o.a.y;
     const unsigned a0 = gx & 0xffffu, a1 = gx >> 16, a2 = gy & 0xffffu, a3 = gy >> 16;
     if (a0 == 0u || a0 >= 0x8000u) v.x = 0.f;
@@ -100,6 +115,11 @@
     *(uint2*)d = make_uint2(h01, h23);
     *(uint2*)(d + 64) = make_uint2(l01, l23);
   }
+  if constexpr (EXT == EXT_MASK_OUT) {
+    if (p.mask)
+      *(unsigned*)(p.mask + m * p.mask_rs + n) = (v.x > 0.f ? 1u : 0u) | (v.y > 0.f ? 0x100u : 0u) |
+                                                 (v.z > 0.f ? 0x10000u : 0u) | (v.w > 0.f ? 0x1000000u : 0u);
+  }
   return v;
 }
 
@@ -113,7 +133,7 @@
   epilogue_apply4(p, m, n, poff, v, bias4, o);
 }
 
-template <int WM, int WN, int MODE, int NS, int OCC, bool DUAL = false, bool POOL = false>
+template <int WM, int WN, int MODE, int NS, int OCC, bool DUAL = false, bool POOL = false, int EXT = EXT_NONE>
 __global__ __launch_bounds__(WM * WN * 64, OCC) void split_gemm_kernel(SplitGemmArgs p, int tiles_n, int ntiles) {
   constexpr int BM = WM * 64, BN = WN * 64, NW = WM * WN;
   constexpr int A_ROWS = MODE == HALO ? BM + 2 * kHalo + 2 : BM;
@@ -434,6 +454,8 @@
   uint2 gates[NBUF][2];
   EpilogueSource src = epilogue_source(p);
   long src_col = epilogue_column_bytes(p, col_ok ? n : 0, col_ok ? poff : 0);
+  constexpr bool SRC_BYTES = EXT == EXT_BYTE_GATE && !DUAL;
+  if constexpr (SRC_BYTES) src_col = col_ok ? n : 0;
   if (slab || !src.base) {
     src.base = p.B;
     src.row_bytes = 0;
@@ -441,14 +463,15 @@
     src_col = 0;
   }
   const long m_last = p.M - 1;
-  const char* gate_col = DUAL ? p.gate + (col_ok ? poff : 0) : nullptr;
+  const char* gate_col = DUAL ? p.gate + (col_ok ? (EXT == EXT_BYTE_GATE ? (long)n : poff) : 0) : nullptr;
   auto fetch = [&](int piece, EpilogueOperands (&o)[2], uint2 (&g)[2]) {
 #pragma unroll
     for (int j = 0; j < 2; ++j) {
       const long m = m0 + wm * 64 + (piece >> 1) * 16 + ((piece & 1) * 2 + j) * 4 + er;
       const long mc = m < m_last ? m : m_last;
-      epilogue_fetch4(src, mc, src_col, o[j]);
-      if constexpr (DUAL) g[j] = *(const uint2*)(gate_col + mc * p.gate_rs);
+      epilogue_fetch4<SRC_BYTES>(src, mc, src_col, o[j]);
+      if constexpr (DUAL && EXT == EXT_BYTE_GATE) g[j] = make_uint2(*(const unsigned*)(gate_col + mc * p.gate_rs), 0u);
+      else if constexpr (DUAL) g[j] = *(const uint2*)(gate_col + mc * p.gate_rs);
     }
   };
   f32x4 ps0 = {0.f, 0.f, 0.f, 0.f}, ps1 = ps0, ps2 = ps0;
@@ -460,6 +483,15 @@
     pool_b1 = (int)((pool_map0 + 1) * p.pool_rows - mw);
     pool_b2 = pool_b1 + p.pool_rows;
   }
+  int sel_slot[3] = {-1, -1, -1};
+  if constexpr (POOL && EXT == EXT_MASK_OUT) {
+    if (p.sel_out) {
+      const long groups = p.M / p.pool_rows;
+#pragma unroll
+      for (int sgm = 0; sgm < 3; ++sgm)
+        if (pool_map0 + sgm < groups) sel_slot[sgm] = p.group_slot[pool_map0 + sgm];
+    }
+  }
 #pragma unroll
   for (int i = 0; i < NBUF - 1; ++i) fetch(i, ops[i], gates[i]);
 #pragma unroll
@@ -478,13 +510,21 @@
         if (m < p.M && col_ok) {
           if (slab) *(f32x4*)(slab + m * p.N + n) = v;
           else {
-            const f32x4 fin = epilogue_apply4<DUAL>(p, m, n, poff, v, bias4, ops[piece % NBUF][j], gates[piece % NBUF][j]);
+            const f32x4 fin = epilogue_apply4<DUAL, EXT>(p, m, n, poff, v, bias4, ops[piece % NBUF][j], gates[piece % NBUF][j]);
             if constexpr (POOL) {
               const int rr = f * 16 + r;
               const f32x4 z = {0.f, 0.f, 0.f, 0.f};
               ps0 += rr < pool_b1 ? fin : z;
               ps1 += (rr >= pool_b1 && rr < pool_b2) ? fin : z;
               ps2 += rr >= pool_b2 ? fin : z;
+              if constexpr (EXT == EXT_MASK_OUT) {
+                const int sgm = rr < pool_b1 ? 0 : (rr < pool_b2 ? 1 : 2);
+                const int slot = sgm == 0 ? sel_slot[0] : (sgm == 1 ? sel_slot[1] : sel_slot[2]);
+                if (slot >= 0) {
+                  const long in_map = m - (pool_map0 + sgm) * p.pool_rows;
+                  *(f32x4*)(p.sel_out + ((long)slot * p.pool_rows + in_map) * p.N + n) = fin;
+                }
+              }
             }
           }
         }
@@ -750,7 +790,8 @@
   }
 }
 
-template <bool GATE_PAIR, bool WRITE_F32>
+enum { GATE_F32 = 0, GATE_PAIR_HI = 1, GATE_BYTES = 2 };
+template <int GATE, bool WRITE_F32>
 __global__ __launch_bounds__(256) void gate_split_pair_kernel(const float* __restrict__ dy, long dy_rs,
                                                              const void* __restrict__ gate, char* __restrict__ dst,
                                                              float* __restrict__ g32, long rows, int cols,
@@ -792,7 +833,14 @@
     }
     const long poff = r * 4L * cols + (long)(c >> 5) * 128 + (c & 31) * 2;
     if (gate) {
-      if (GATE_PAIR) {
+      if (GATE == GATE_BYTES) {
+        const uint2 b = *(const uint2*)((const unsigned char*)gate + r * (long)cols + c);
+#pragma unroll
+        for (int k = 0; k < 4; ++k) {
+          if (!((b.x >> (8 * k)) & 0xffu)) v[k] = 0.f;
+          if (!((b.y >> (8 * k)) & 0xffu)) v[4 + k] = 0.f;
+        }
+      } else if (GATE == GATE_PAIR_HI) {
         const uint4 h = *(const uint4*)((const char*)gate + poff);
         const unsigned w[4] = {h.x, h.y, h.z, h.w};
 #pragma unroll
@@ -980,10 +1028,9 @@
                                        pool_rows, nullptr, nullptr, stream);
 }
 
-extern "C" int ovis_gate_split_pair_rows_f32(const float* dy, long dy_row_stride, const void* gate, int gate_is_pair,
-                                             void* dst_pair, float* g_f32, long rows, int cols, const float* g_pooled,
-                                             int pool_rows, const float* g_selected, const int32_t* group_slot,
-                                             void* stream) {
+static int gate_split_pair_impl(const float* dy, long dy_row_stride, const void* gate, int gate_kind, void* dst_pair,
+                                float* g_f32, long rows, int cols, const float* g_pooled, int pool_rows,
+                                const float* g_selected, const int32_t* group_slot, void* stream) {
   if (rows < 0 || cols < 0) return OVIS_EINVAL;
   if (rows == 0 || cols == 0) return OVIS_OK;
   if ((!dy && !g_pooled && !g_selected) || !dst_pair || ((g_pooled || g_selected) && (pool_rows <= 0 || rows % pool_rows != 0)) ||
@@ -997,14 +1044,32 @@
   const long blocks = (total + 255) / 256;
   const unsigned grid = (unsigned)(blocks < 8L * OVIS_NUM_CU ? blocks : 8L * OVIS_NUM_CU);
   hipStream_t s = (hipStream_t)stream;
-#define OVIS_GS(GP_, WF_)                                                                                          \
-  hipLaunchKernelGGL((gate_split_pair_kernel<GP_, WF_>), dim3(grid), dim3(256), 0, s, dy, dy_row_stride, gate,      \
+#define OVIS_GS(GK_, WF_)                                                                                          \
+  hipLaunchKernelGGL((gate_split_pair_kernel<GK_, WF_>), dim3(grid), dim3(256), 0, s, dy, dy_row_stride, gate,      \
                      (char*)dst_pair, g_f32, rows, cols, g_pooled, pool_rows, pool_scale, g_selected, group_slot)
-  if (gate_is_pair) { if (g_f32) OVIS_GS(true, true); else OVIS_GS(true, false); }
-  else { if (g_f32) OVIS_GS(false, true); else OVIS_GS(false, false); }
+  if (gate_kind == GATE_BYTES) { if (g_f32) OVIS_GS(GATE_BYTES, true); else OVIS_GS(GATE_BYTES, false); }
+  else if (gate_kind == GATE_PAIR_HI) { if (g_f32) OVIS_GS(GATE_PAIR_HI, true); else OVIS_GS(GATE_PAIR_HI, false); }
+  else { if (g_f32) OVIS_GS(GATE_F32, true); else OVIS_GS(GATE_F32, false); }
 #undef OVIS_GS
   OVIS_LAUNCH_CHECK();
   return OVIS_OK;
+}
+
+extern "C" int ovis_gate_split_pair_rows_f32(const float* dy, long dy_row_stride, const void* gate, int gate_is_pair,
+                                             void* dst_pair, float* g_f32, long rows, int cols, const float* g_pooled,
+                                             int pool_rows, const float* g_selected, const int32_t* group_slot,
+                                             void* stream) {
+  return gate_split_pair_impl(dy, dy_row_stride, gate, gate_is_pair ? GATE_PAIR_HI : GATE_F32, dst_pair, g_f32, rows, cols,
+                              g_pooled, pool_rows, g_selected, group_slot, stream);
+}
+
+extern "C" int ovis_gate_split_pair_rows_bm_f32(const float* dy, long dy_row_stride, const unsigned char* gate_mask,
+                                                void* dst_pair, float* g_f32, long rows, int cols, const float* g_pooled,
+                                                int pool_rows, const float* g_selected, const int32_t* group_slot,
+                                                void* stream) {
+  if (!gate_mask && rows > 0 && cols > 0) return OVIS_EINVAL;
+  return gate_split_pair_impl(dy, dy_row_stride, gate_mask, GATE_BYTES, dst_pair, g_f32, rows, cols, g_pooled, pool_rows,
+                              g_selected, group_slot, stream);
 }
 
 extern "C" int ovis_im2col_nchw_pair_f32(const float* src, void* dst_pair, int num, int channels, int height,
@@ -1247,11 +1312,17 @@
                                 const void* gate_pair, long gate_row_bytes, long m, int n, int channels, int channels2,
                                 int taps_h, int taps_w, int height, int width, int flip, int relu, void* workspace,
                                 size_t workspace_bytes, int config, void* stream, float* pool = nullptr, int pool_rows = 0,
-                                float pool_scale = 1.f) {
+                                float pool_scale = 1.f, int ext = EXT_NONE, unsigned char* mask = nullptr, long mask_rs = 0,
+                                const int32_t* group_slot = nullptr, float* sel_out = nullptr) {
   if (m < 0 || n < 0 || channels < 0 || channels2 < 0 || taps_h <= 0 || taps_w <= 0 || !(taps_h & 1) || !(taps_w & 1))
     return OVIS_EINVAL;
   if (m == 0 || n == 0) return OVIS_OK;
-  if (!a_pair || !b_pair || (!c && !c_pair && !pool) || channels == 0 || m > 0x7fffff00L) return OVIS_EINVAL;
+  if (!a_pair || !b_pair || (!c && !c_pair && !pool && !mask) || channels == 0 || m > 0x7fffff00L) return OVIS_EINVAL;
+  if (ext == EXT_BYTE_GATE && (!gate_pair || residual || gate_row_bytes % 4 != 0 || ((uintptr_t)gate_pair & 3))) return OVIS_EINVAL;
+  if (ext == EXT_MASK_OUT && (gate_pair || ((uintptr_t)mask & 3) || mask_rs % 4 != 0 || (mask && mask_rs < n) ||
+                              (sel_out != nullptr) != (group_slot != nullptr) || ((uintptr_t)sel_out & 15) ||
+                              (sel_out && (!pool || pool_rows <= 0 || m % pool_rows != 0))))
+    return OVIS_EINVAL;
   if (pool && (pool_rows < 32 || pool_rows > 64 || ((uintptr_t)pool & 15))) return OVIS_ERANGE;
   const int T = taps_h * taps_w;
   if (T > 1 && (height <= 0 || width <= 0 || height > 32767 || width > 32767 || channels2 != 0)) return OVIS_EINVAL;
@@ -1280,6 +1351,7 @@
   p.gate = (const char*)gate_pair; p.gate_rs = gate_row_bytes;
   p.slab = q.kslices > 1 ? (float*)workspace : nullptr;
   p.pool = pool; p.pool_rows = pool_rows; p.pool_scale = pool_scale;
+  p.mask = mask; p.mask_rs = mask_rs; p.group_slot = group_slot; p.sel_out = sel_out;
   p.M = m; p.N = n; p.ch = channels; p.ch2 = channels2; p.T = T; p.H = height; p.W = width; p.KH = taps_h; p.KW = taps_w;
   p.flip = flip; p.relu = relu;
   p.kslices = q.kslices; p.steps_per_slice = q.steps_per_slice;
@@ -1288,22 +1360,34 @@
   const long nblocks = ntiles * q.kslices;
   if (nblocks > 0x7fffffffL) return OVIS_ERANGE;
   hipStream_t s = (hipStream_t)stream;
-#define OVIS_SG_LAUNCH__(WM_, WN_, MODE_, NS_, OCC_, DUAL_, POOL_)                                                   \
+#define OVIS_SG_LAUNCH___(WM_, WN_, MODE_, NS_, OCC_, DUAL_, POOL_, EXT_)                                            \
   do {                                                                                                              \
     constexpr int a_rows = MODE_ == HALO ? WM_ * 64 + 2 * kHalo + 2 : WM_ * 64;                                      \
     constexpr int lds = NS_ * (a_rows * 128 + WN_ * 64 * 128);                                                       \
     static bool attr_set = false;                                                                                   \
     if (!attr_set) {                                                                                                \
-      OVIS_HIP_TRY(hipFuncSetAttribute((const void*)split_gemm_kernel<WM_, WN_, MODE_, NS_, OCC_, DUAL_, POOL_>,    \
+      OVIS_HIP_TRY(hipFuncSetAttribute((const void*)split_gemm_kernel<WM_, WN_, MODE_, NS_, OCC_, DUAL_, POOL_, EXT_>, \
                                        hipFuncAttributeMaxDynamicSharedMemorySize, lds));                           \
       attr_set = true;                                                                                              \
     }                                                                                                               \
-    hipLaunchKernelGGL((split_gemm_kernel<WM_, WN_, MODE_, NS_, OCC_, DUAL_, POOL_>), dim3((unsigned)nblocks),      \
+    hipLaunchKernelGGL((split_gemm_kernel<WM_, WN_, MODE_, NS_, OCC_, DUAL_, POOL_, EXT_>), dim3((unsigned)nblocks), \
                        dim3(WM_ * WN_ * 64), lds, s, p, q.tiles_n, (int)ntiles);                                    \
   } while (0)
+#define OVIS_SG_LAUNCH__(WM_, WN_, MODE_, NS_, OCC_, DUAL_, POOL_) OVIS_SG_LAUNCH___(WM_, WN_, MODE_, NS_, OCC_, DUAL_, POOL_, EXT_NONE)
 #define OVIS_SG_LAUNCH_(WM_, WN_, MODE_, NS_, OCC_, DUAL_) OVIS_SG_LAUNCH__(WM_, WN_, MODE_, NS_, OCC_, DUAL_, false)
 #define OVIS_SG_LAUNCH(WM_, WN_, MODE_, NS_, OCC_) OVIS_SG_LAUNCH_(WM_, WN_, MODE_, NS_, OCC_, false)
-  if (pool) {
+  if (ext != EXT_NONE) {
+    if (q.narrow || q.mode != PLAIN || q.kslices > 1) return OVIS_ERANGE;
+    if (ext == EXT_MASK_OUT) {
+      if (!pool || dual) return OVIS_ERANGE;
+      if (q.stages == 1) OVIS_SG_LAUNCH___(2, 2, PLAIN, 1, 4, false, true, EXT_MASK_OUT);
+      else OVIS_SG_LAUNCH___(2, 2, PLAIN, 2, 2, false, true, EXT_MASK_OUT);
+    } else {
+      if (!dual || pool) return OVIS_ERANGE;
+      if (q.stages == 1) OVIS_SG_LAUNCH___(2, 2, PLAIN, 1, 4, true, false, EXT_BYTE_GATE);
+      else OVIS_SG_LAUNCH___(2, 2, PLAIN, 2, 2, true, false, EXT_BYTE_GATE);
+    }
+  } else if (pool) {
     if (dual || q.narrow || q.mode != PLAIN || q.kslices > 1) return OVIS_ERANGE;
     if (q.stages == 1) OVIS_SG_LAUNCH__(2, 2, PLAIN, 1, 4, false, true); else OVIS_SG_LAUNCH__(2, 2, PLAIN, 2, 2, false, true);
   } else if (dual) {
@@ -1318,6 +1402,7 @@
   } else {
     if (q.stages == 1) OVIS_SG_LAUNCH(2, 2, PLAIN, 1, 4); else OVIS_SG_LAUNCH(2, 2, PLAIN, 2, 2);
   }
+#undef OVIS_SG_LAUNCH___
 #undef OVIS_SG_LAUNCH__
 #undef OVIS_SG_LAUNCH_
 #undef OVIS_SG_LAUNCH
@@ -1371,6 +1456,21 @@
   return split_gemm_pair_impl(a_pair, a_row_bytes, nullptr, 0, b_pair, b_row_bytes, c, ldc, c_pair, c_pair_row_bytes, bias,
                               nullptr, 0, residual_pair, residual_pair_row_bytes, nullptr, 0, m, n, channels, 0, 1, 1, 0, 0,
                               0, relu, nullptr, 0, 8, stream, pooled, pool_rows, pool_scale);
+}
+
+extern "C" int ovis_split_gemm_pair_rp_pool_masked(const void* a_pair, long a_row_bytes, const void* b_pair,
+                                                   long b_row_bytes, float* c, long ldc, void* c_pair,
+                                                   long c_pair_row_bytes, const float* bias, const void* residual_pair,
+                                                   long residual_pair_row_bytes, long m, int n, int channels, int relu,
+                                                   float* pooled, int pool_rows, float pool_scale, unsigned char* mask,
+                                                   long mask_row_bytes, const int32_t* group_slot, float* selected,
+                                                   void* stream) {
+  if (!pooled || (!mask && !selected)) return OVIS_EINVAL;
+  if (n % 32 != 0 || (residual_pair && (residual_pair_row_bytes % 16 != 0 || ((uintptr_t)residual_pair & 15)))) return OVIS_ERANGE;
+  return split_gemm_pair_impl(a_pair, a_row_bytes, nullptr, 0, b_pair, b_row_bytes, c, ldc, c_pair, c_pair_row_bytes, bias,
+                              nullptr, 0, residual_pair, residual_pair_row_bytes, nullptr, 0, m, n, channels, 0, 1, 1, 0, 0,
+                              0, relu, nullptr, 0, 8, stream, pooled, pool_rows, pool_scale, EXT_MASK_OUT, mask,
+                              mask_row_bytes, group_slot, selected);
 }
 
 extern "C" int ovis_split_gemm_pair_gated(const void* a_pair, long a_row_bytes, const void* b_pair, long b_row_bytes,
@@ -1407,6 +1507,20 @@
   return split_gemm_pair_impl(a_pair, a_row_bytes, nullptr, 0, b_pair, b_row_bytes, c, ldc, c_pair, c_pair_row_bytes,
                               nullptr, nullptr, 0, residual_pair, residual_pair_row_bytes, gate_pair, gate_row_bytes, m, n,
                               channels, 0, 1, 1, 0, 0, 0, 0, nullptr, 0, config | 8, stream);
+}
+
+extern "C" int ovis_split_gemm_pair_rp_gated_bm(const void* a_pair, long a_row_bytes, const void* b_pair, long b_row_bytes,
+                                                float* c, long ldc, void* c_pair, long c_pair_row_bytes,
+                                                const void* residual_pair, long residual_pair_row_bytes,
+                                                const unsigned char* gate_mask, long gate_row_bytes, long m, int n,
+                                                int channels, int config, void* stream) {
+  if (!residual_pair || !gate_mask || n % 32 != 0 || residual_pair_row_bytes % 16 != 0 || gate_row_bytes % 4 != 0 ||
+      gate_row_bytes < n || ((uintptr_t)residual_pair & 15) || ((uintptr_t)gate_mask & 3))
+    return OVIS_ERANGE;
+  if (n < 128) return OVIS_ERANGE;
+  return split_gemm_pair_impl(a_pair, a_row_bytes, nullptr, 0, b_pair, b_row_bytes, c, ldc, c_pair, c_pair_row_bytes,
+                              nullptr, nullptr, 0, residual_pair, residual_pair_row_bytes, gate_mask, gate_row_bytes, m, n,
+                              channels, 0, 1, 1, 0, 0, 0, 0, nullptr, 0, config | 8, stream, nullptr, 0, 1.f, EXT_BYTE_GATE);
 }
 
 extern "C" int ovis_deform_conv_implicit_f32(const float* input_nhwc, const float* offset, const float* mask,
diff --git a/cvpr22_cross_modal_pseudo_labeling_amd/layers/pair_bottleneck.py b/cvpr22_cross_modal_pseudo_labeling_amd/layers/pair_bottleneck.py
--- a/cvpr22_cross_modal_pseudo_labeling_amd/layers/pair_bottleneck.py
+++ b/cvpr22_cross_modal_pseudo_labeling_amd/layers/pair_bottleneck.py
@@ -190,11 +190,18 @@
             out, outp = _C.split_gemm_pair(o2p, w3d, b3, None, True, f32, want_pair, a2_pair=xp)
         elif x_real:
             out, outp = _C.split_gemm_pair(o2p, wpairs["w3"], b3, x, True, f32, want_pair)
-        pooled_k = None
+        pooled_k = sel_k = slot_k = gate_mask = None
         if wd is None and not x_real:
             fused_pool = (pool and 32 <= h * w <= 64
                           and _C.split_gemm_pair_pool_supported(o2p.shape[0], wpairs["w3"].shape[0], o2p.shape[1] // 2, h * w))
-            if fused_pool:
+            if fused_pool and need_bwd and pool_only_ok and not want_pair:
+                if select is not None:
+                    slot_k = torch.full((o2p.shape[0] // (h * w),), -1, dtype=torch.int32, device=o2p.device)
+                    slot_k[select] = torch.arange(select.numel(), dtype=torch.int32, device=o2p.device)
+                pooled_k, gate_mask, sel_k = _C.split_gemm_pair_rp_pool_masked(o2p, wpairs["w3"], b3, xp, True, h * w, slot_k,
+                                                                               0 if select is None else select.numel())
+                out, outp = nan_placeholder(pooled_k.device, o2p.shape[0], pooled_k.shape[1]), None
+            elif fused_pool:
                 keep = need_bwd or want_pair or select is not None or not pool_only_ok
                 out, outp, pooled_k = _C.split_gemm_pair_rp_pool(o2p, wpairs["w3"], b3, xp, True, keep, want_pair, h * w)
                 if out is None and outp is None:
@@ -205,12 +212,16 @@
             pooled = pooled_k
         else:
             pooled = out.view(-1, h * w, out.shape[1]).mean(dim=1) if pool else None
-        out_sel = out.view(-1, h * w, out.shape[1]).index_select(0, select) if (select is not None and f32) else None
-        gate_src = out if out is not None else outp
+        if sel_k is not None:
+            out_sel = sel_k.view(select.numel(), h * w, sel_k.shape[1])
+        else:
+            out_sel = out.view(-1, h * w, out.shape[1]).index_select(0, select) if (select is not None and f32) else None
+        gate_src = gate_mask if gate_mask is not None else (out if out is not None else outp)
         if out is None:
             out = nan_placeholder(outp.device, outp.shape[0], outp.shape[1] // 2)
         ctx.save_for_backward(xp, o1p, o2p, gate_src, w1, w2, w3, wd, s1, s2, s3, sd, select if out_sel is not None else None)
         ctx.wts = wts
+        ctx.group_slot = slot_k
         ctx.geom = (h, w, kh, kw)
         ctx.link_in = link_in if (wd is None and not x_real) else None
         ctx.link_out = link_out if not f32 else None
@@ -249,8 +260,10 @@
             if dsel is not None:
                 if dout is None and dpooled is None:
                     dpooled = dsel.new_zeros((out.shape[0] // (h * w), n3))
-                slot = torch.full((out.shape[0] // (h * w),), -1, dtype=torch.int32, device=dsel.device)
-                slot[select] = torch.arange(select.numel(), dtype=torch.int32, device=dsel.device)
+                slot = ctx.group_slot
+                if slot is None:
+                    slot = torch.full((out.shape[0] // (h * w),), -1, dtype=torch.int32, device=dsel.device)
+                    slot[select] = torch.arange(select.numel(), dtype=torch.int32, device=dsel.device)
                 sel_grad = dsel.reshape(-1, n3)
             g3p, g3 = _C.gate_split_pair(None if dout is None else dout.reshape(-1, n3), out,
                                          want_f32=(wd is None and need_x and not to_link), pooled=dpooled, pool_rows=h * w,
diff --git a/cvpr22_cross_modal_pseudo_labeling_amd/modeling/roi_heads.py b/cvpr22_cross_modal_pseudo_labeling_amd/modeling/roi_heads.py
--- a/cvpr22_cross_modal_pseudo_labeling_amd/modeling/roi_heads.py
+++ b/cvpr22_cross_modal_pseudo_labeling_amd/modeling/roi_heads.py
@@ -718,7 +718,8 @@
         rois = _C.rois_from_boxes([p.bbox for props in sampled for p in props],
                                   [img for br in branches for img in br["image_ids"]])
         sel_pos = positives_index([p for props in sampled for p in props]) if self.mask_on else None
-        x = box.feature_extractor.forward_rois([feat], rois, select=sel_pos)
+        x = box.feature_extractor.forward_rois([feat], rois, select=sel_pos,
+                                               pooled_only=(not self.mask_on) or sel_pos is not None)
         pooled = box.predictor.pooled(x)
         counts = [sum(len(p) for p in props) for props in sampled]
         out, off = [], 0
diff --git a/include/ovis_hip.h b/include/ovis_hip.h
--- a/include/ovis_hip.h
+++ b/include/ovis_hip.h
@@ -140,6 +140,9 @@
 int ovis_gate_split_pair_rows_f32(const float* dy, long dy_row_stride, const void* gate, int gate_is_pair,
                                   void* dst_pair, float* g_f32, long rows, int cols, const float* g_pooled,
                                   int pool_rows, const float* g_selected, const int32_t* group_slot, void* stream);
+int ovis_gate_split_pair_rows_bm_f32(const float* dy, long dy_row_stride, const unsigned char* gate_mask, void* dst_pair,
+                                     float* g_f32, long rows, int cols, const float* g_pooled, int pool_rows,
+                                     const float* g_selected, const int32_t* group_slot, void* stream);
 
 int ovis_weight_prep_pair_f32(const float* weight, const float* scale, void* fwd_pair, void* bwd_pair,
                               int out_channels, int in_channels, int taps, void* stream);
@@ -165,6 +168,10 @@
                                   long ldc, void* c_pair, long c_pair_row_bytes, const void* residual_pair,
                                   long residual_pair_row_bytes, const void* gate_pair, long gate_row_bytes, long m, int n,
                                   int channels, int config, void* stream);
+int ovis_split_gemm_pair_rp_gated_bm(const void* a_pair, long a_row_bytes, const void* b_pair, long b_row_bytes, float* c,
+                                     long ldc, void* c_pair, long c_pair_row_bytes, const void* residual_pair,
+                                     long residual_pair_row_bytes, const unsigned char* gate_mask, long gate_row_bytes,
+                                     long m, int n, int channels, int config, void* stream);
 
 int ovis_im2col_nchw_pair_f32(const float* src, void* dst_pair, int num, int channels, int height, int width,
                               int kh, int kw, int stride, int pad, int k_padded, void* stream);
@@ -283,6 +290,11 @@
                                  long ldc, void* c_pair, long c_pair_row_bytes, const float* bias,
                                  const void* residual_pair, long residual_pair_row_bytes, long m, int n, int channels,
                                  int relu, float* pooled, int pool_rows, float pool_scale, void* stream);
+int ovis_split_gemm_pair_rp_pool_masked(const void* a_pair, long a_row_bytes, const void* b_pair, long b_row_bytes, float* c,
+                                        long ldc, void* c_pair, long c_pair_row_bytes, const float* bias,
+                                        const void* residual_pair, long residual_pair_row_bytes, long m, int n, int channels,
+                                        int relu, float* pooled, int pool_rows, float pool_scale, unsigned char* mask,
+                                        long mask_row_bytes, const int32_t* group_slot, float* selected, void* stream);
 
 int ovis_sgd_momentum_multi_f32(const void* items, const void* blocks, int num_blocks, float lr, float weight_decay,
                                 float momentum, int apply_weight_decay, void* stream);
```

Result: no change. 60.60 images/sec (-0.1%).
